# ttaoREtw/semi-tts

Measured on AMD Instinct MI355X. Metric: mel-frames/sec (decode+attn), higher is better.
Workload: dtype f32

## Files before the change

### include/semitts.h

```cpp
#ifndef SEMITTS_H
#define SEMITTS_H

#include <stddef.h>
#include <stdint.h>

#ifdef __cplusplus
extern "C" {
#endif

#define ST_ABI_VERSION 1

#define ST_ACT_NONE 0
#define ST_ACT_RELU 1
#define ST_ACT_TANH 2
#define ST_ACT_SIGMOID 3

const char* st_last_error(void);
int st_abi_version(void);
int st_device_info(int* n_cu, int* lds_bytes, char* name, int name_len);

int st_stream_create(void** stream_out);
int st_stream_destroy(void* stream);
int st_stream_sync(void* stream);
int st_graph_begin(void* stream);
// ... 225 lines not shown
    float* run_mean; float* run_var; long long* batches_tracked;
    float momentum, eps;
    float* mean; float* var;
    float* dx; int lddx;
    float* sums;
} st_bn_bank_seg;
size_t st_bn_bank_workspace_floats(int nseg, int max_rows, int N);
int st_bn_bank_fwd(const st_bn_bank_seg* segs, int nseg, int Bn, int N, float* Y, int ldy, int Tout, float* ws, void* stream);
int st_bn_bank_bwd(const st_bn_bank_seg* segs, int nseg, int Bn, int N, const float* dY, int lddy, int Tout, int relu_in, float* ws,
                   void* stream);
int st_bn_bank_stats_record(const st_bn_bank_seg* segs, int nseg, int Bn, int N, float* rec, float* ws, void* stream);
int st_bn_bank_sync_merge(const st_bn_bank_seg* segs, int nseg, int Bn, int N, const float* allrec, int world, float* inv_total, void* stream);
int st_bn_bank_norm(const st_bn_bank_seg* segs, int nseg, int Bn, int N, float* Y, int ldy, int Tout, void* stream);
int st_bn_bank_bwd_reduce(const st_bn_bank_seg* segs, int nseg, int Bn, int N, const float* dY, int lddy, int Tout, float* ws, void* stream);
int st_bn_bank_bwd_apply(const st_bn_bank_seg* segs, int nseg, int Bn, int N, const float* dY, int lddy, int Tout, int relu_in,
                         const float* inv_total, void* stream);
int st_highway_ht_fwd(const float* ht, const float* x, float* y, int M, int C, void* stream);
int st_highway_ht_bwd(const float* dy, const float* ht, const float* x, float* dht, float* dx_direct, int M, int C, void* stream);
int st_highway_bwd(const float* dy, const float* H, const float* x, const float* Tgate,
                   float* dH, float* dT, float* dx_direct, size_t total, void* stream);
int st_pool_prev_fwd(const float* x, float* y, int Bn, int T, int C, void* stream);
int st_pool_prev_bwd(const float* dy_pooled, const float* x, float* dx, int Bn, int T, int C, void* stream);
int st_copy3d(float* dst, long dst_sb, long dst_st, const float* src, long src_sb, long src_st,
              int Bn, int T, int C, int accumulate, void* stream);
int st_scatter_add_rows(const float* dout, const int64_t* idx, float* dtable, int n, int D, int V, void* stream);

int st_lstm_seq_fwd(const float* xproj, const float* w_hh, const float* b_hh, float* out, int ldo, int ocol,
                    float* ws, float* gates_tape, float* c_tape, int B, int T, int H, int reverse, void* stream);
int st_lstm_cell_bwd_pointwise(const float* dh0, int ld0, const float* dh1, int ld1, const float* dh2, int ld2,
                               const float* scale2, const float* mask, const float* gates, const float* c, int ldc,
                               const float* c_prev, int ldcp, float* dc, float* dgates, int ldg,
                               const st_t16_view* dgates_t16, int B, int H, void* stream);
int st_lstm_cell_pair_fwd(const st_seg* segs2, const float* const* b_hh2, const float* const* pre2, int ldpre,
                          const float* const* c_prev2, int ldc_prev, float* const* h_out2, int ldh,
                          float* const* c_out2, int ldc, float* const* gates_out2, int B, int H, void* stream);
int st_lstm_seq2_fwd(const float* const* xproj2, const float* const* w_hh2, const float* const* b_hh2, float* out, int ldo,
                     const int* ocol2, float* ws, float* const* gates_tape2, float* const* c_tape2,
                     int B, int T, int H, void* stream);
int st_lstm_seq2_persist_supported(int B, int T, int H, int ldo, int ocol0, int ocol1);
int st_lstm_seq2_persist_fwd(const float* const* xproj2, const float* const* w_hh2, const float* const* b_hh2, float* out, int ldo,
                             const int* ocol2, float* const* gates_tape2, float* const* c_tape2,
                             int B, int T, int H, unsigned* status, void* stream);
int st_lstm_seq2_bwd(const float* dout, int ldd, const int* dcol2, const float* const* gates_tape2, const float* const* c_tape2,
                     const float* const* w_hh_t2, float* const* dxproj2, float* ws, int B, int T, int H, void* stream);
int st_lstm_seq2_bwd_persist_supported(int B, int T, int H, int ldd, int dcol0, int dcol1);
int st_lstm_seq2_bwd_persist(const float* dout, int ldd, const int* dcol2, const float* const* gates_tape2, const float* const* c_tape2,
                             const float* const* w_hh2, float* const* dxproj2, int B, int T, int H, unsigned* status, void* stream);
int st_skinny_linear_pair_fwd(const st_seg* segs2, float* const* y2, int ldy, int B, int N, void* stream);
int st_lstm_seq2_bwd_packed(const float* dout, int ldd, const int* dcol2, const float* const* gates_tape2, const float* const* c_tape2,
                            const float* const* w_hh_t_p16_2, float* const* dxproj2, float* ws, float* dg_t16_ws,
                            int B, int T, int H, void* stream);
int st_lstm_seq_bwd(const float* dout, int ldd, int dcol, const float* gates_tape, const float* c_tape,
                    const float* w_hh_t, float* dxproj, float* ws, int B, int T, int H, int reverse, void* stream);
int st_gru_seq_fwd(const float* gi_fwd, const float* gi_bwd, const float* w_hh_fwd, const float* w_hh_bwd,
                   const float* b_hh_fwd, const float* b_hh_bwd, float* out, int ldo, float* tape,
                   int B, int T, int H, int ndir, void* stream);
int st_gru_seq_bwd(const float* dout, int ldd, const float* out, int ldo, const float* tape,
                   const float* w_hh_fwd, const float* w_hh_bwd, float* dgi_fwd, float* dgi_bwd,
                   float* dgh_fwd, float* dgh_bwd, int B, int T, int H, int ndir, void* stream);
#define ST_GRU_TRI 0
#define ST_GRU_QUAD 1
#define ST_GRU_REG32 2
#define ST_GRU_GENERAL 3
int st_gru_seq_variant(int H, int backward);

int st_vq_build_table(const float* learnable, int Dl, const float* attr, int n_attr,
                      const float* attr_w, const float* attr_b, int Da, float* table, int V, void* stream);
int st_gather_rows(const float* table, const int64_t* idx, float* out, int n, int D, int V, void* stream);
int st_vq_l2_fwd(const float* x, const float* table, const float* temp, float* p_code,
                 int64_t* idx, float* out, float* workspace, int n, int D, int V, void* stream);
int st_vq_pack_table(const float* table, float* packed, int D, int V, void* stream);
int st_vq_l2_packed_fwd(const float* x, const float* table, const float* packed, const float* temp, float* p_code,
                        int64_t* idx, float* out, int n, int D, int V, void* stream);
size_t st_vq_l2_workspace_floats(int D, int V);
int st_softmax_bwd(const float* p, const float* dp, const float* relu_scale, float scale, float* dz, float* rowsum,
                   int n, int V, void* stream);
int st_rowscale_combine(const float* a, float alpha, const float* x, const float* r, float beta, const float* c,
                        float* out, int M, int D, void* stream);
int st_vq_mean_fwd(const float* p_code, const float* latent, float* out, int* lens, int* frame_seg, float* frame_w,
                   int B, int T, int D, int V, int max_frames_per_phn, void* stream);
int st_vq_mean_bwd(const float* dout, int n_seg_rows, const int* frame_seg, const float* frame_w, float* dlatent,
                   int B, int T, int D, void* stream);
int st_softmax_argmax(const float* logits, float* p, int64_t* idx, int n, int V, void* stream);

typedef struct st_decoder_weights {
    const float* prenet_w0;
    const float* prenet_w1;
    const float* q_w_ih;
    const float* q_w_hh;
    const float* q_b_ih; const float* q_b_hh;
    const float* attn_query_w;
    const float* attn_v;
    const float* attn_loc_conv_w;
    const float* attn_loc_lin_w;
    const float* d_w_ih;
    const float* d_w_hh;
    const float* d_b_ih; const float* d_b_hh;
    const float* projgate_w;
    const float* projgate_b;
    const float* pre_norm_w[2]; const float* pre_norm_b[2];
    float* pre_norm_rm[2]; float* pre_norm_rv[2]; long long* pre_norm_nbt[2];
    float pre_norm_eps, pre_norm_momentum;
} st_decoder_weights;

typedef struct st_decoder_dims {
    int B, L, E, n_mels, r, P, Q, D, A, F, K;
    int fuse_pre0;
    int prenet_norm;
} st_decoder_dims;

typedef struct st_decoder_io {
    const float* memory;
    const float* pm;
    const float* ada_std;
    const float* ada_mean;
    const int* step_src;
    const float* teacher_pre;
    const float* teacher_mean;
    int Bt, Tt;
    const float* prenet_mask;
    const float* q_mask;
    const float* d_mask;
    int steps;
    float* mel_out;
    float* align_out;
    float* stop_out;
    const float* packed;
    float* xq_tape; float* xd_tape; float* xo_tape;
    float* cq_tape; float* cd_tape; float* wcum_tape;
    float* pq_buf;
    float* pre1_t16;
    float* mel_t16;
    float* zero_row;
    float* gates_q_tape;
    float* gates_d_tape;
    float* attn_s_buf;
    int attn_pre_parts;
    int attn_fin_parts;
    int defer_proj;
    int pre1_step_floats;
    int attn_s_step_floats;
    float* attn_loc_tape;
    float* attn_split_ws;
    int attn_split_parts;
    unsigned long long* pq_granules;
    const float* dec_in0;
    float* pre_nat;
    unsigned long long* attn_xchg;
    unsigned* handoff_status;
    int pair_cells;
    float* pre_nat_tape;
    float* gate_part;
    int gate_part_k;
} st_decoder_io;

int st_decoder_gate_split_k(const st_decoder_dims* d);
size_t st_decoder_packed_floats(const st_decoder_dims* d);
size_t st_decoder_tape_floats(const st_decoder_dims* d, int which);
int st_decoder_pack(const st_decoder_weights* w, const st_decoder_dims* d, float* packed, void* stream);
int st_decoder_forward(const st_decoder_weights* w, const st_decoder_dims* d, const st_decoder_io* io,
                       void* stream);
int st_decoder_fwd_forms(const st_decoder_dims* d, const st_decoder_io* io, int cus, int rng_capacity);

typedef struct st_attn_bwd_job {
    const float* pq; const float* pm; const float* memory;
    const float* w_prev; int ld_wprev; const float* w_cum_prev; const float* w; int ld_w;
    const float* loc_conv_w; const float* loc_lin_w; const float* v;
    const float* dctx[3]; int ld_dctx[3]; int n_dctx;
    const float* dw_direct[3]; int ld_dw[3]; int n_dw;
    float* dcum; const float* dcum_add; int ld_dcum_add;
    float* dpq; st_t16_view dpq_t16; float* dhist; float* ds_t; float* loc_t; float* dloc_t; float* hist_t;
    float* dctx_t; float* dv_t; const float* s_in;
    int B, L, A, E, F, K;
    int parts; float* dloc_part;
    const float* dctx_more[3]; int ld_dctx_more[3]; int n_dctx_more;
} st_attn_bwd_job;
int st_attn_step_bwd(const st_attn_bwd_job* job, void* stream);

int st_attn_dmem(const float* align, const float* dctx_tape, float* dmem, int B, int steps, int L, int E, void* stream);

typedef struct st_decoder_bwd_weights {
    const float* q_w_cat_t;
    const float* d_w_cat_t;
    const float* attn_query_w_t;
    const float* q_w_cat_t_p16;
    const float* d_w_cat_t_p16;
    const float* attn_query_w_t_p16;
    const float* attn_v; const float* attn_loc_conv_w; const float* attn_loc_lin_w;
} st_decoder_bwd_weights;

typedef struct st_decoder_bwd_io {
    const float* memory; const float* pm; const float* ada_std;
    const float* align;
    const float* wcum_tape;
    const float* cq_tape; const float* cd_tape;
    const float* gates_q_tape; const float* gates_d_tape;
    const float* q_mask; const float* d_mask;
    const float* pq_all;
    int steps; int Bp;
    const float* dxo;
    const float* dalign;
    float* dgq; float* dgd;
    float* dxq; float* dxd;
    float* dpq;
    float* ds_tape; float* loc_tape; float* dloc_tape;
    float* hist_tape; float* dctx_tape; float* dv_tape;
    float* dcq; float* dcd;
    float* dhist[2];
    float* dcum;
    float* dhq_attn;
    float* dgq_t16; float* dgd_t16;
    const int* step_src; int Bt;
    float* dY;
    float* dxo_rw;
    const float* wpg_t;
    const float* pre_w1_t; const float* pre_w0_t;
    const float* own_mask;
    const float* xq_nat;
    const float* pre1_nat;
    float* d2_tape; float* dp1_tape;
    float* tmp_p; float* tmp_in;
    int fuse_pw;
    float* dgd_t16_b;
    float* dpq_t16;
    int need_dxq0;
    const float* attn_s_tape;
    int overlap_attn;
    int prenet_norm;
    const float* pre_y_tape;
    const float* pre_norm_w[2]; const float* pre_norm_rm[2]; const float* pre_norm_rv[2];
    float pre_norm_eps;
    float* dpre_norm_w[2]; float* dpre_norm_b[2];
    int attn_parts; float* dloc_part;
    float* dxd_part; int dxd_splits;
    float* dxq_part; int dxq_splits;
} st_decoder_bwd_io;
int st_decoder_bwd_fuse_dims(const st_decoder_dims* d);
int st_decoder_bwd_forms(const st_decoder_dims* d, const st_decoder_bwd_io* io);
typedef struct st_attn_hist_job {
    const float* dloc_part; int parts;
    const float* loc_conv_w;
    const float* w_prev; int ld_wprev; const float* w_cum_prev;
    float* dloc_t; float* hist_t; float* dhist; float* dcum;
    int B, L, F, K;
} st_attn_hist_job;
int st_skinny_linear_packed_lstm_bwd_pair_fwd(const float* const* packed_w2, const st_t16_view* x2, int K, float* const* y2, int ldy,
                                              int B, int N, const st_lstm_pw_job* job2, void* stream);
int st_skinny_linear_packed_lstm_bwd_attn_bwd(const float* packed_w, const st_t16_view* x, int K, float* y, int ldy, int B, int N,
                                              const st_lstm_pw_job* job, const st_attn_bwd_job* ab, void* stream);
int st_attn_bwd_wide_fits(int L, int A, int E, int F, int K);
int st_attn_bwd_variant(int L, int A, int E, int F, int K, int has_s, int parts, int hosted, int B, int N, const float* loc_lin_w);
typedef struct st_partial_sum_job {
    const float* part; int S; int N;
    float* y; int ldy;
    const st_lstm_pw_job* pw;
} st_partial_sum_job;
int st_skinny_partial_attn_bwd(const float* packed_w, const st_t16_view* x, int K, float* part, int S, int B, int N,
                               const st_attn_bwd_job* ab, void* stream);
int st_skinny_partial_attn_hist(const float* packed_w, const st_t16_view* x, int K, float* part, int S, int B, int N,
                                const st_attn_hist_job* hist, void* stream);
int st_skinny_linear_packed_lstm_bwd_attn_hist_sum(const float* packed_w, const st_t16_view* x, int K, float* y, int ldy, int B, int N,
                                                   const st_lstm_pw_job* job, const st_attn_hist_job* hist,
                                                   const st_partial_sum_job* sum, void* stream);
int st_skinny_linear_packed_attn_hist(const float* packed_w, const st_t16_view* x, int K, float* y, int ldy, int B, int N,
                                      const st_attn_hist_job* hist, void* stream);
int st_decoder_backward(const st_decoder_bwd_weights* w, const st_decoder_dims* d, const st_decoder_bwd_io* io, void* stream);
void st_loop_graph_stats(long* fwd3, long* bwd3);
int st_loop_graphs_enable(int on);
int st_decoder_pack_dout(const float* dmel, const float* dstop, float* dY, int ld, int B, int Bp, int steps, int r, int n_mels,
                         void* stream);
int st_decoder_unpack_out(const float* Y, float* mel, float* stop, int B, int Bp, int steps, int r, int n_mels, int ld, void* stream);
int st_decoder_dteacher_sum(const float* dxq_part, float* dteacher, int S, int Bp, int XQw, int Bt, int Tt, int P, int steps, void* stream);
int st_adain_bwd(const float* dadapt, long da_step_stride, int da_ld, const float* hq, long hq_step_stride, int hq_ld,
                 const float* ada_std, const float* ada_mean, float* dstd, float* dmean, int B, int Q, int steps, void* stream);

size_t st_ctc_workspace_floats(int B, int T);
int st_ctc_loss(const float* prob, const int64_t* text, float eps, float* loss, float* dprob, float* ws,
                int B, int T, int V, int L, int log_input, void* stream);

int st_ctc_greedy_edit_distance(const float* prob, int B, int T, int V, const int64_t* text, int L,
                                const int32_t* ignore, int n_ignore,
                                int32_t* dist, int32_t* ref_len, int64_t* hyp , int32_t* hyp_len ,
                                void* stream);
int st_ids_edit_distance(const int64_t* pred, int B, int T, const int64_t* text, int L, const int32_t* ignore, int n_ignore,
                         int32_t* dist, int32_t* ref_len, int64_t* hyp, int32_t* hyp_len, void* stream);
int st_hyp_edit_distance(const int64_t* hyp, const int32_t* hyp_len, int B, int Lh, const int64_t* text, int L, const int32_t* ignore,
                         int n_ignore, int32_t* dist, int32_t* ref_len, void* stream);

size_t st_ctc_beam_workspace_bytes(int B, int T, int W);
int st_ctc_beam_search(const float* prob, int B, int T, int V, const int32_t* lengths , int W, int N, int blank,
                       int log_input, float eps, int64_t* hyp , int32_t* hyp_len ,
                       float* score , void* ws, void* stream);
int st_ctc_beam_search_lm(const float* prob, int B, int T, int V, const int32_t* lengths , int W, int N, int blank,
                          int log_input, float eps, const float* bonus , int order, int bos,
                          int64_t* hyp , int32_t* hyp_len , float* score , void* ws,
                          void* stream);

size_t st_ctc_align_workspace_bytes(int B, int T, int L);
int st_ctc_forced_align(const float* prob, int B, int T, int V, const int32_t* lengths ,
                        const int64_t* text , int L, const int32_t* text_lengths ,
                        int blank, int log_input, float eps,
                        float* score , int32_t* path ,
                        int32_t* tok_start , int32_t* tok_end , void* ws, void* stream);

#define ST_SCALAR_MAX 8
int st_scalar_combine(const float* const* xs, int n, const float* W, int m, float* const* outs, void* stream);
int st_scalar_fanout(const float* dout, const float* w, int n, float* out, void* stream);

size_t st_freq_loss_workspace_floats(void);
int st_freq_loss(const float* pred, const float* label, float* loss, float* dpred, float* ws,
                 int B, int T, int D, int n_low, float w_all, float w_low, float w_diff, int l1, void* stream);
typedef struct st_wgrad_job {
    const float* dC; int lddc, dcoff; const float* A; int lda; float* dW; float* db;
    int Bn, Tin, Tout, Cin, N, KT, pad;
} st_wgrad_job;
// ... 64 lines not shown
```

### semi_tts_amd/_lib.py

```python
import ctypes as C
import os

HERE = os.path.dirname(os.path.abspath(__file__))
LIB_PATH = os.environ.get('ST_LIB_PATH') or os.path.join(HERE, 'lib', 'libsemitts_hip.so')

c_float_p = C.c_void_p
c_void_p = C.c_void_p


class StSeg(C.Structure):
    _fields_ = [('x', C.c_void_p), ('w', C.c_void_p), ('ldx', C.c_int), ('ldw', C.c_int), ('k', C.c_int)]


class StT16View(C.Structure):
    _fields_ = [('base', C.c_void_p), ('kb_stride', C.c_int), ('kb0', C.c_int)]


class StGemmEpilogue(C.Structure):
    _fields_ = [('bias', C.c_void_p), ('act_pre', C.c_int),
                ('bn_mean', C.c_void_p), ('bn_var', C.c_void_p), ('bn_w', C.c_void_p), ('bn_b', C.c_void_p),
                ('bn_eps', C.c_float), ('act_post', C.c_int),
                ('res', C.c_void_p), ('ldres', C.c_int),
                ('highway_h', C.c_void_p), ('ldhw', C.c_int),
                ('mask', C.c_void_p), ('ldmask', C.c_int), ('w_tap_major', C.c_int),
                ('splitk_ws', C.c_void_p), ('splitk_slabs', C.c_int)]


class StGemmJob(C.Structure):
    _fields_ = [('A', C.c_void_p), ('lda', C.c_int), ('W', C.c_void_p), ('C', C.c_void_p), ('ldc', C.c_int), ('coff', C.c_int),
                ('Bn', C.c_int), ('Tin', C.c_int), ('Tout', C.c_int), ('Cin', C.c_int), ('N', C.c_int), ('KT', C.c_int),
                ('pad', C.c_int), ('stride', C.c_int), ('pool_prev', C.c_int), ('ep', StGemmEpilogue)]


class StRelayoutDesc(C.Structure):
    _fields_ = [('src', C.c_void_p), ('dst', C.c_void_p), ('N', C.c_int), ('Cin', C.c_int), ('KT', C.c_int), ('mode', C.c_int),
                ('blk0', C.c_int), ('ld_dst', C.c_int)]


class StBnBankSeg(C.Structure):
    _fields_ = [('x', C.c_void_p), ('ldx', C.c_int), ('T', C.c_int), ('w', C.c_void_p), ('b', C.c_void_p), ('run_mean', C.c_void_p),
                ('run_var', C.c_void_p), ('batches_tracked', C.c_void_p), ('momentum', C.c_float), ('eps', C.c_float),
                ('mean', C.c_void_p), ('var', C.c_void_p), ('dx', C.c_void_p), ('lddx', C.c_int), ('sums', C.c_void_p)]


class StDecoderWeights(C.Structure):
    _fields_ = [(n, C.c_void_p) for n in (
        'prenet_w0', 'prenet_w1', 'q_w_ih', 'q_w_hh', 'q_b_ih', 'q_b_hh',
        'attn_query_w', 'attn_v', 'attn_loc_conv_w', 'attn_loc_lin_w',
        'd_w_ih', 'd_w_hh', 'd_b_ih', 'd_b_hh', 'projgate_w', 'projgate_b')] + [
        ('pre_norm_w', C.c_void_p * 2), ('pre_norm_b', C.c_void_p * 2), ('pre_norm_rm', C.c_void_p * 2), ('pre_norm_rv', C.c_void_p * 2),
        ('pre_norm_nbt', C.c_void_p * 2), ('pre_norm_eps', C.c_float), ('pre_norm_momentum', C.c_float)]


class StDecoderDims(C.Structure):
    _fields_ = [(n, C.c_int) for n in ('B', 'L', 'E', 'n_mels', 'r', 'P', 'Q', 'D', 'A', 'F', 'K', 'fuse_pre0', 'prenet_norm')]


class StDecoderIO(C.Structure):
    _fields_ = [('memory', C.c_void_p), ('pm', C.c_void_p), ('ada_std', C.c_void_p), ('ada_mean', C.c_void_p),
                ('step_src', C.POINTER(C.c_int)), ('teacher_pre', C.c_void_p), ('teacher_mean', C.c_void_p),
                ('Bt', C.c_int), ('Tt', C.c_int),
                ('prenet_mask', C.c_void_p), ('q_mask', C.c_void_p), ('d_mask', C.c_void_p),
                ('steps', C.c_int),
                ('mel_out', C.c_void_p), ('align_out', C.c_void_p), ('stop_out', C.c_void_p),
                ('packed', C.c_void_p),
                ('xq_tape', C.c_void_p), ('xd_tape', C.c_void_p), ('xo_tape', C.c_void_p),
                ('cq_tape', C.c_void_p), ('cd_tape', C.c_void_p), ('wcum_tape', C.c_void_p),
                ('pq_buf', C.c_void_p), ('pre1_t16', C.c_void_p), ('mel_t16', C.c_void_p),
                ('zero_row', C.c_void_p),
                ('gates_q_tape', C.c_void_p), ('gates_d_tape', C.c_void_p), ('attn_s_buf', C.c_void_p), ('attn_pre_parts', C.c_int), ('attn_fin_parts', C.c_int), ('defer_proj', C.c_int),
                ('pre1_step_floats', C.c_int), ('attn_s_step_floats', C.c_int), ('attn_loc_tape', C.c_void_p),
                ('attn_split_ws', C.c_void_p), ('attn_split_parts', C.c_int), ('pq_granules', C.c_void_p),
                ('dec_in0', C.c_void_p), ('pre_nat', C.c_void_p), ('attn_xchg', C.c_void_p), ('handoff_status', C.c_void_p),
                ('pair_cells', C.c_int), ('pre_nat_tape', C.c_void_p), ('gate_part', C.c_void_p), ('gate_part_k', C.c_int)]


class StDecoderBwdWeights(C.Structure):
    _fields_ = [(n, C.c_void_p) for n in ('q_w_cat_t', 'd_w_cat_t', 'attn_query_w_t', 'q_w_cat_t_p16', 'd_w_cat_t_p16', 'attn_query_w_t_p16',
                                          'attn_v', 'attn_loc_conv_w', 'attn_loc_lin_w')]


class StDecoderBwdIO(C.Structure):
    _fields_ = ([(n, C.c_void_p) for n in ('memory', 'pm', 'ada_std', 'align', 'wcum_tape', 'cq_tape', 'cd_tape',
                                           'gates_q_tape', 'gates_d_tape', 'q_mask', 'd_mask', 'pq_all')] +
                [('steps', C.c_int), ('Bp', C.c_int)] +
                [(n, C.c_void_p) for n in ('dxo', 'dalign', 'dgq', 'dgd', 'dxq', 'dxd', 'dpq', 'ds_tape', 'loc_tape', 'dloc_tape',
                                           'hist_tape', 'dctx_tape', 'dv_tape', 'dcq', 'dcd')] +
                [('dhist', C.c_void_p * 2), ('dcum', C.c_void_p), ('dhq_attn', C.c_void_p), ('dgq_t16', C.c_void_p),
                 ('dgd_t16', C.c_void_p), ('step_src', C.POINTER(C.c_int)), ('Bt', C.c_int)] +
                [(n, C.c_void_p) for n in ('dY', 'dxo_rw', 'wpg_t', 'pre_w1_t', 'pre_w0_t', 'own_mask', 'xq_nat', 'pre1_nat',
                                           'd2_tape', 'dp1_tape', 'tmp_p', 'tmp_in')] +
                [('fuse_pw', C.c_int), ('dgd_t16_b', C.c_void_p), ('dpq_t16', C.c_void_p), ('need_dxq0', C.c_int), ('attn_s_tape', C.c_void_p),
                 ('overlap_attn', C.c_int), ('prenet_norm', C.c_int), ('pre_y_tape', C.c_void_p), ('pre_norm_w', C.c_void_p * 2),
                 ('pre_norm_rm', C.c_void_p * 2), ('pre_norm_rv', C.c_void_p * 2), ('pre_norm_eps', C.c_float),
                 ('dpre_norm_w', C.c_void_p * 2), ('dpre_norm_b', C.c_void_p * 2), ('attn_parts', C.c_int), ('dloc_part', C.c_void_p),
                 ('dxd_part', C.c_void_p), ('dxd_splits', C.c_int), ('dxq_part', C.c_void_p), ('dxq_splits', C.c_int)])



class StLstmPwJob(C.Structure):
    _fields_ = [('n0', C.c_int), ('H', C.c_int), ('dh1', C.c_void_p), ('ld1', C.c_int), ('dh2', C.c_void_p), ('ld2', C.c_int),
                ('scale2', C.c_void_p), ('mask', C.c_void_p), ('gates', C.c_void_p), ('c', C.c_void_p), ('ldc', C.c_int),
                ('c_prev', C.c_void_p), ('ldcp', C.c_int), ('dc', C.c_void_p), ('dgates', C.c_void_p), ('ldg', C.c_int),
                ('dgates_t16', StT16View), ('dh1_slabs', C.c_int), ('dh1_slab_stride', C.c_long)]


class StLstmCellPackedJob(C.Structure):
    _fields_ = [('packed_w', C.c_void_p), ('x', StT16View), ('K', C.c_int), ('b_ih', C.c_void_p), ('b_hh', C.c_void_p),
                ('c_prev', C.c_void_p), ('ldc_prev', C.c_int), ('mask', C.c_void_p), ('h_dst0', StT16View), ('h_dst1', StT16View),
                ('c_out', C.c_void_p), ('ldc', C.c_int), ('gates_out', C.c_void_p), ('ada_std', C.c_void_p), ('ada_mean', C.c_void_p),
                ('hadapt_dst', StT16View), ('B', C.c_int), ('H', C.c_int), ('part', C.c_void_p), ('w_kbs', C.c_int)]


class StAttnBwdJob(C.Structure):
    _fields_ = [('pq', C.c_void_p), ('pm', C.c_void_p), ('memory', C.c_void_p),
                ('w_prev', C.c_void_p), ('ld_wprev', C.c_int), ('w_cum_prev', C.c_void_p), ('w', C.c_void_p), ('ld_w', C.c_int),
                ('loc_conv_w', C.c_void_p), ('loc_lin_w', C.c_void_p), ('v', C.c_void_p),
                ('dctx', C.c_void_p * 3), ('ld_dctx', C.c_int * 3), ('n_dctx', C.c_int),
                ('dw_direct', C.c_void_p * 3), ('ld_dw', C.c_int * 3), ('n_dw', C.c_int),
                ('dcum', C.c_void_p), ('dcum_add', C.c_void_p), ('ld_dcum_add', C.c_int),
                ('dpq', C.c_void_p), ('dpq_t16', StT16View), ('dhist', C.c_void_p), ('ds_t', C.c_void_p), ('loc_t', C.c_void_p),
                ('dloc_t', C.c_void_p), ('hist_t', C.c_void_p), ('dctx_t', C.c_void_p), ('dv_t', C.c_void_p), ('s_in', C.c_void_p),
                ('B', C.c_int), ('L', C.c_int), ('A', C.c_int), ('E', C.c_int), ('F', C.c_int), ('K', C.c_int),
                ('parts', C.c_int), ('dloc_part', C.c_void_p),
                ('dctx_more', C.c_void_p * 3), ('ld_dctx_more', C.c_int * 3), ('n_dctx_more', C.c_int)]


class StAttnHistJob(C.Structure):
    _fields_ = [('dloc_part', C.c_void_p), ('parts', C.c_int), ('loc_conv_w', C.c_void_p),
                ('w_prev', C.c_void_p), ('ld_wprev', C.c_int), ('w_cum_prev', C.c_void_p),
                ('dloc_t', C.c_void_p), ('hist_t', C.c_void_p), ('dhist', C.c_void_p), ('dcum', C.c_void_p),
                ('B', C.c_int), ('L', C.c_int), ('F', C.c_int), ('K', C.c_int)]


class StWgradJob(C.Structure):
    _fields_ = [('dC', C.c_void_p), ('lddc', C.c_int), ('dcoff', C.c_int), ('A', C.c_void_p), ('lda', C.c_int), ('dW', C.c_void_p), ('db', C.c_void_p),
                ('Bn', C.c_int), ('Tin', C.c_int), ('Tout', C.c_int), ('Cin', C.c_int), ('N', C.c_int), ('KT', C.c_int), ('pad', C.c_int)]


class StPartialSumJob(C.Structure):
    _fields_ = [('part', C.c_void_p), ('S', C.c_int), ('N', C.c_int), ('y', C.c_void_p), ('ldy', C.c_int), ('pw', C.c_void_p)]


class StAttnPreJob(C.Structure):
    _fields_ = [('pm', C.c_void_p), ('w_prev', C.c_void_p), ('ld_wprev', C.c_int), ('w_cum_prev', C.c_void_p),
                ('loc_conv_w', C.c_void_p), ('loc_lin_w', C.c_void_p), ('s_buf', C.c_void_p),
                ('L', C.c_int), ('A', C.c_int), ('F', C.c_int), ('K', C.c_int), ('parts', C.c_int), ('cf_out', C.c_void_p),
                ('part', C.c_void_p)]


class StAttnFinJob(C.Structure):
    _fields_ = [('s_buf', C.c_void_p), ('memory', C.c_void_p), ('w_cum_prev', C.c_void_p),
                ('w_out', C.c_void_p), ('ld_wout', C.c_int), ('w_cum_out', C.c_void_p), ('v', C.c_void_p),
                ('ctx_dst', StT16View * 3), ('n_ctx_dst', C.c_int), ('parts', C.c_int),
                ('L', C.c_int), ('A', C.c_int), ('E', C.c_int), ('F', C.c_int), ('K', C.c_int), ('status', C.c_void_p),
                ('ctx', C.c_void_p), ('ld_ctx', C.c_int)]


class StAttnStepJob(C.Structure):
    _fields_ = [('pq', C.c_void_p), ('pm', C.c_void_p), ('memory', C.c_void_p),
                ('w_prev', C.c_void_p), ('ld_wprev', C.c_int), ('w_cum_prev', C.c_void_p),
                ('w_out', C.c_void_p), ('ld_wout', C.c_int), ('w_cum_out', C.c_void_p),
                ('loc_conv_w', C.c_void_p), ('loc_lin_w', C.c_void_p), ('v', C.c_void_p),
                ('ctx_dst', StT16View * 3), ('n_ctx_dst', C.c_int), ('ctx', C.c_void_p), ('ld_ctx', C.c_int),
                ('h_q', C.c_void_p), ('ld_hq', C.c_int), ('ada_std', C.c_void_p), ('ada_mean', C.c_void_p), ('h_adapt', C.c_void_p),
                ('Q', C.c_int), ('L', C.c_int), ('A', C.c_int), ('E', C.c_int), ('F', C.c_int), ('K', C.c_int)]


class StPartialProductJob(C.Structure):
    _fields_ = [('packed_w', C.c_void_p), ('w_kbs', C.c_int), ('kb0', C.c_int), ('KB', C.c_int), ('x', StT16View), ('N', C.c_int),
                ('part', C.c_void_p)]


P, I, F, Z = C.c_void_p, C.c_int, C.c_float, C.c_size_t

SIGNATURES = {
    'st_last_error': [],
    'st_abi_version': [],
    'st_device_info': [C.POINTER(I), C.POINTER(I), C.c_char_p, I],
    'st_stream_create': [C.POINTER(P)],
    'st_stream_destroy': [P],
    'st_stream_sync': [P],
    'st_graph_begin': [P],
    'st_graph_end': [P, C.POINTER(P)],
    'st_graph_launch': [P, P],
    'st_graph_destroy': [P],
    'st_event_create': [C.POINTER(P)],
    'st_event_record': [P, P],
    'st_event_elapsed_ms': [P, P, C.POINTER(F)],
    'st_event_destroy': [P],
    'st_lstm_cell_fwd': [C.POINTER(StSeg), I, P, P, P, I, P, I, P, P, I, P, I, P, I, I, P],
    'st_skinny_linear_fwd': [C.POINTER(StSeg), I, P, I, P, I, P, I, I, P, I, I, I, I, P],
    'st_attn_step_fwd': [C.POINTER(StAttnStepJob), I, P],
    'st_gemm_fwd': [P, I, P, P, I, I, I, I, I, I, I, I, I, I, I, C.POINTER(StGemmEpilogue), P],
    'st_gemm_fwd_batch': [C.POINTER(StGemmJob), I, P],
    'st_gemm_fwd_variant': [P, I, P, P, I, I, I, I, I, I, I, I, I, I, I, C.POINTER(StGemmEpilogue)],
    'st_gemm_fwd_batch_variant': [C.POINTER(StGemmJob), I],
    'st_highway_stack_supported': [I, I],
    'st_highway_stack_fwd': [P, I, C.POINTER(P), C.POINTER(P), C.POINTER(P), C.POINTER(P), I, P, I, I, I, P],
    'st_gemm_splitk_slabs': [I, I, I, I, I],
    'st_bn_stats': [P, I, I, I, I, P, P, P, P, F, P, P, P],
    'st_colreduce_workspace_floats': [I, I],
    'st_bn_apply': [P, I, I, I, I, P, P, P, P, F, I, P],
    'st_lstm_seq_fwd': [P, P, P, P, I, I, P, P, P, I, I, I, I, P],
    'st_lstm_cell_bwd_pointwise': [P, I, P, I, P, I, P, P, P, P, I, P, I, P, P, I, C.POINTER(StT16View), I, I, P],
    'st_lstm_seq_bwd': [P, I, I, P, P, P, P, P, I, I, I, I, P],
    'st_gru_seq_fwd': [P, P, P, P, P, P, P, I, P, I, I, I, I, P],
    'st_gru_seq_bwd': [P, I, P, I, P, P, P, P, P, P, P, I, I, I, I, P],
    'st_gru_seq_variant': [I, I],
    'st_vq_build_table': [P, I, P, I, P, P, I, P, I, P],
    'st_gather_rows': [P, P, P, I, I, I, P],
    'st_vq_l2_fwd': [P, P, P, P, P, P, P, I, I, I, P],
    'st_vq_pack_table': [P, P, I, I, P],
    'st_vq_l2_packed_fwd': [P, P, P, P, P, P, P, I, I, I, P],
    'st_vq_l2_workspace_floats': [I, I],
    'st_ctc_workspace_floats': [I, I],
    'st_ctc_loss': [P, P, C.c_float, P, P, P, I, I, I, I, I, P],
    'st_ctc_greedy_edit_distance': [P, I, I, I, P, I, P, I, P, P, P, P, P],
    'st_ids_edit_distance': [P, I, I, P, I, P, I, P, P, P, P, P],
    'st_hyp_edit_distance': [P, P, I, I, P, I, P, I, P, P, P],
    'st_ctc_beam_workspace_bytes': [I, I, I],
    'st_ctc_beam_search': [P, I, I, I, P, I, I, I, I, F, P, P, P, P, P],
    'st_ctc_beam_search_lm': [P, I, I, I, P, I, I, I, I, F, P, I, I, P, P, P, P, P],
    'st_ctc_align_workspace_bytes': [I, I, I],
    'st_ctc_forced_align': [P, I, I, I, P, P, I, P, I, I, F, P, P, P, P, P, P],
    'st_scalar_combine': [P, I, P, I, P, P],
    'st_scalar_fanout': [P, P, I, P, P],
    'st_softmax_bwd': [P, P, P, C.c_float, P, P, I, I, P],
    'st_rowscale_combine': [P, C.c_float, P, P, C.c_float, P, P, I, I, P],
    'st_vq_mean_fwd': [P, P, P, P, P, P, I, I, I, I, I, P],
    'st_vq_mean_bwd': [P, I, P, P, P, I, I, I, P],
    'st_softmax_argmax': [P, P, P, I, I, P],
    'st_packed_weight_floats': [C.POINTER(I), I, I, I],
    'st_t16_floats': [I, I],
    'st_pack_weight': [C.POINTER(P), C.POINTER(I), C.POINTER(I), I, I, I, P, P],
    'st_pack_weight_t': [C.POINTER(P), C.POINTER(I), C.POINTER(I), I, I, P, P],
    'st_relayout_blocks': [I, I, I],
    'st_relayout_batch': [P, I, I, P, P],
    'st_pack_weight_batch': [P, I, P],
    'st_tile_rows': [P, I, C.POINTER(StT16View), I, I, P],
    'st_untile_rows': [C.POINTER(StT16View), P, I, I, I, P],
    'st_lstm_cell_packed_fwd': [C.POINTER(StLstmCellPackedJob), P],
    'st_lstm_cell_packed_pair_fwd': [C.POINTER(StLstmCellPackedJob), C.POINTER(StLstmCellPackedJob), P],
    'st_skinny_linear_packed_fwd': [P, C.POINTER(StT16View), I, P, I, P, I, P, I, C.POINTER(StT16View), I, P, I, I,
                                    I, I, P, I, C.POINTER(StT16View), I, I, P],
    'st_skinny_linear_packed_attnpre_fwd': [P, C.POINTER(StT16View), I, P, I, P, I, P, I, C.POINTER(StT16View), I, P, I, I,
                                            I, I, P, I, C.POINTER(StT16View), I, I, C.POINTER(StAttnPreJob), P],
    'st_attn_pre_fwd': [C.POINTER(StAttnPreJob), I, P],
    'st_attn_fin_fwd': [P, C.POINTER(StAttnFinJob), I, P],
    'st_attn_fin_split_workspace_floats': [I, I, I],
    'st_attn_fin_split_fwd': [P, C.POINTER(StAttnFinJob), P, I, P],
    'st_query_attn_fin_fwd': [P, C.POINTER(StT16View), I, P, C.c_uint, C.POINTER(StAttnFinJob), I, P],
    'st_query_attn_fin_part_fwd': [P, C.POINTER(StT16View), I, P, C.c_uint, C.POINTER(StAttnFinJob), I, C.POINTER(StPartialProductJob), P],
    'st_partial_product_fwd': [C.POINTER(StPartialProductJob), I, P],
    'st_layer_norm_fwd': [P, I, P, P, F, P, I, P, P, I, I, P],
    'st_layer_norm_bwd': [P, I, P, I, P, P, P, P, I, P, I, I, P],
    'st_log_softmax_fwd': [P, P, I, I, P],
    'st_log_softmax_bwd': [P, P, P, I, I, P],
    'st_prenet_norm_fwd': [P, I, I, P, P, P, P, P, F, F, P, I, C.POINTER(StT16View), I, I, I, P],
    'st_prenet_norm_bwd': [P, I, P, I, I, P, P, P, F, P, P, I, I, P],
    'st_handoff_wait_selftest': [P, C.c_uint, I, P, P, I, P],
    'st_query_attn_rng_fits': [I, I, I],
    'st_attn_rng_xchg_words': [I, I, I],
    'st_query_attn_rng_fwd': [P, C.POINTER(StT16View), I, P, P, C.c_uint, C.POINTER(StAttnFinJob), I, P],
    'st_decoder_packed_floats': [C.POINTER(StDecoderDims)],
    'st_decoder_gate_split_k': [C.POINTER(StDecoderDims)],
    'st_decoder_tape_floats': [C.POINTER(StDecoderDims), I],
    'st_decoder_pack': [C.POINTER(StDecoderWeights), C.POINTER(StDecoderDims), P, P],
    'st_decoder_forward': [C.POINTER(StDecoderWeights), C.POINTER(StDecoderDims), C.POINTER(StDecoderIO), P],
    'st_decoder_fwd_forms': [C.POINTER(StDecoderDims), C.POINTER(StDecoderIO), I, I],
    'st_attn_step_bwd': [C.POINTER(StAttnBwdJob), P],
    'st_skinny_linear_packed_lstm_bwd_fwd': [P, C.POINTER(StT16View), I, P, I, I, I, C.POINTER(StLstmPwJob), P],
    'st_skinny_linear_packed_lstm_bwd_attn_bwd': [P, C.POINTER(StT16View), I, P, I, I, I, C.POINTER(StLstmPwJob), C.POINTER(StAttnBwdJob), P],
    'st_attn_bwd_wide_fits': [I, I, I, I, I],
    'st_attn_bwd_variant': [I, I, I, I, I, I, I, I, I, I, P],
    'st_skinny_linear_packed_attn_hist': [P, C.POINTER(StT16View), I, P, I, I, I, C.POINTER(StAttnHistJob), P],
    'st_skinny_partial_attn_hist': [P, C.POINTER(StT16View), I, P, I, I, I, C.POINTER(StAttnHistJob), P],
    'st_decoder_bwd_forms': [C.POINTER(StDecoderDims), C.POINTER(StDecoderBwdIO)],
    'st_decoder_bwd_fuse_dims': [C.POINTER(StDecoderDims)],
    'st_loop_graph_stats': [P, P],
    'st_loop_graphs_enable': [I],
    'st_skinny_partial_attn_bwd': [P, C.POINTER(StT16View), I, P, I, I, I, C.POINTER(StAttnBwdJob), P],
    'st_skinny_linear_packed_lstm_bwd_attn_hist_sum': [P, C.POINTER(StT16View), I, P, I, I, I, C.POINTER(StLstmPwJob), C.POINTER(StAttnHistJob),
                                                       C.POINTER(StPartialSumJob), P],
    'st_lstm_seq2_fwd': [C.POINTER(P), C.POINTER(P), C.POINTER(P), P, I, C.POINTER(I), P, C.POINTER(P), C.POINTER(P), I, I, I, P],
    'st_lstm_seq2_persist_supported': [I, I, I, I, I, I],
    'st_lstm_seq2_persist_fwd': [C.POINTER(P), C.POINTER(P), C.POINTER(P), P, I, C.POINTER(I), C.POINTER(P), C.POINTER(P), I, I, I, P, P],
    'st_lstm_seq2_bwd_persist_supported': [I, I, I, I, I, I],
    'st_lstm_seq2_bwd_persist': [P, I, C.POINTER(I), C.POINTER(P), C.POINTER(P), C.POINTER(P), C.POINTER(P), I, I, I, P, P],
    'st_lstm_seq2_bwd': [P, I, C.POINTER(I), C.POINTER(P), C.POINTER(P), C.POINTER(P), C.POINTER(P), P, I, I, I, P],
    'st_skinny_linear_pair_fwd': [P, C.POINTER(P), I, I, I, P],
    'st_lstm_seq2_bwd_packed': [P, I, C.POINTER(I), C.POINTER(P), C.POINTER(P), C.POINTER(P), C.POINTER(P), P, P, I, I, I, P],
    'st_skinny_linear_packed_lstm_bwd_pair_fwd': [C.POINTER(P), C.POINTER(StT16View), I, C.POINTER(P), I, I, I, C.POINTER(StLstmPwJob), P],
    'st_lstm_cell_pair_fwd': [P, C.POINTER(P), C.POINTER(P), I, C.POINTER(P), I, C.POINTER(P), I, C.POINTER(P), I, C.POINTER(P), I, I, P],
    'st_attn_dmem': [P, P, P, I, I, I, I, P],
    'st_decoder_backward': [C.POINTER(StDecoderBwdWeights), C.POINTER(StDecoderDims), C.POINTER(StDecoderBwdIO), P],
    'st_decoder_pack_dout': [P, P, P, I, I, I, I, I, I, P],
    'st_decoder_unpack_out': [P, P, P, I, I, I, I, I, I, P],
    'st_decoder_dteacher_sum': [P, P, I, I, I, I, I, I, I, P],
    'st_adain_bwd': [P, C.c_long, I, P, C.c_long, I, P, P, P, P, I, I, I, P],
    'st_mt_blocks': [P, I],
    'st_mt_table_misses': [],
    'st_mt_grad_norm': [P, P, I, P, P, P],
    'st_mt_clip_scale': [P, P, I, P, F, P],
    'st_mt_grad_norm_scaled': [P, P, I, P, P, F, P],
    'st_mt_clip_scale_pre': [P, P, I, P, F, F, P],
    'st_mt_copy': [P, P, P, I, P],
    'st_mt_adam': [P, P, P, P, P, I, F, F, F, F, F, P],
    'st_mt_adam_guarded': [P, P, P, P, P, I, F, F, F, F, F, P, P],
    'st_freq_loss': [P, P, P, P, P, I, I, I, I, F, F, F, I, P],
    'st_freq_loss_workspace_floats': [],
    'st_scale_by': [P, P, P, Z, P],
    'st_bn_norm_fwd': [P, I, I, P, I, I, I, I, P, P, P, P, F, I, P],
    'st_gemm_wgrad_workspace_floats': [I, I, I, I, I],
    'st_gemm_wgrad': [P, I, I, P, I, P, P, I, I, I, I, I, I, I, I, I, P],
    'st_gemm_wgrad_db': [P, I, I, P, I, P, P, P, I, I, I, I, I, I, I, I, I, P],
    'st_gemm_wgrad_batch_workspace_floats': [C.POINTER(StWgradJob), I],
    'st_gemm_wgrad_batch': [C.POINTER(StWgradJob), I, P, P],
    'st_gemm_wgrad_variant': [P, I, I, P, I, I, I, I, I, I, I, I, I, I, I, I],
    'st_gemm_wgrad_batch_variant': [C.POINTER(StWgradJob), I, C.POINTER(I)],
    'st_gemm_wgrad_split': [P, I, I, P, I, P, I, P, P, P, P, I, I, I, I, P],
    'st_colsum': [P, I, I, P, I, I, I, I, P, I, P, P],
    'st_act_bwd': [P, I, P, I, I, P, I, P, I, I, I, P],
    'st_bn_bwd': [P, I, I, P, I, I, I, P, I, I, P, P, P, F, I, I, P, I, I, P, P, I, P, P],
    'st_bn_bwd_reduce': [P, I, I, P, I, I, I, P, I, I, P, P, F, I, I, P, P, P],
    'st_bn_norm_res_mask_fwd': [P, P, P, I, I, P, P, P, P, F, I, P, P, P],
    'st_bn_bwd_reduce_masked': [P, I, P, I, P, I, I, P, I, P, P, F, I, I, P, P, P],
    'st_bn_bwd_apply_masked': [P, I, P, I, P, I, I, P, I, P, P, P, F, I, I, P, I, P, P, I, P, I, P],
    'st_bn_bwd_apply': [P, I, I, P, I, I, I, P, I, I, P, P, P, F, I, I, P, I, P, I, I, P],
    'st_bn_stats_record': [P, I, I, I, I, P, P, P, P],
    'st_bn_sync_merge': [P, I, I, P, P, P, P, F, P, P],
    'st_bn_bwd_apply_sync': [P, I, I, P, I, I, I, P, I, I, P, P, P, F, I, I, P, P, P, I, I, P],
    'st_highway_fwd': [P, P, P, P, Z, P],
    'st_bn_bank_workspace_floats': [I, I, I],
    'st_bn_bank_fwd': [C.POINTER(StBnBankSeg), I, I, I, P, I, I, P, P],
    'st_bn_bank_bwd': [C.POINTER(StBnBankSeg), I, I, I, P, I, I, I, P, P],
    'st_bn_bank_stats_record': [C.POINTER(StBnBankSeg), I, I, I, P, P, P],
    'st_bn_bank_sync_merge': [C.POINTER(StBnBankSeg), I, I, I, P, I, P, P],
    'st_bn_bank_norm': [C.POINTER(StBnBankSeg), I, I, I, P, I, I, P],
    'st_bn_bank_bwd_reduce': [C.POINTER(StBnBankSeg), I, I, I, P, I, I, P, P],
    'st_bn_bank_bwd_apply': [C.POINTER(StBnBankSeg), I, I, I, P, I, I, I, P, P],
    'st_highway_ht_fwd': [P, P, P, I, I, P],
    'st_highway_ht_bwd': [P, P, P, P, P, I, I, P],
    'st_highway_bwd': [P, P, P, P, P, P, P, Z, P],
    'st_pool_prev_fwd': [P, P, I, I, I, P],
    'st_pool_prev_bwd': [P, P, P, I, I, I, P],
    'st_copy3d': [P, C.c_long, C.c_long, P, C.c_long, C.c_long, I, I, I, I, P],
    'st_scatter_add_rows': [P, P, P, I, I, I, P],
    'st_fill': [P, F, Z, P],
    'st_copy2d': [P, I, P, I, I, I, P],
    'st_mean_rows': [P, P, I, I, I, P],
    'st_istft_workspace_floats': [I, I, I, I, I],
    'st_gl_workspace_floats': [I, I, I, I, I],
    'st_stft_fwd': [P, P, I, I, I, I, I, P],
    'st_istft': [P, P, I, I, I, I, I, P, P],
    'st_griffin_lim': [P, C.c_long, C.c_long, C.c_long, I, F, P, P, I, I, I, I, I, I, I, P, P],
    'st_mel_to_linear': [P, C.c_long, C.c_long, C.c_long, P, P, I, I, I, I, I, I, P],
    'st_gl_batch_workspace_floats': [I, I, I, I, I],
    'st_griffin_lim_batch': [P, C.c_long, C.c_long, C.c_long, I, P, I, F, P, P, P, I, I, I, I, I, I, I, P, P],
    'st_features_workspace_floats': [I],
    'st_audio_features': [P, C.c_long, P, C.c_ulonglong, P, P, P, P, P, I, I, I, I, I, F, P, P, P, P, I, P, P, I, P, I, P, P],
    'st_feature_noise': [P, C.c_long, I, C.c_ulonglong, P],
    'st_resample_batch': [P, I, C.c_long, P, P, I, I, I, I, I, I, P, P, P, C.c_long, P, P],
}
_RESTYPES = {'st_last_error': C.c_char_p, 'st_packed_weight_floats': C.c_size_t, 'st_t16_floats': C.c_size_t,
             'st_decoder_packed_floats': C.c_size_t, 'st_vq_l2_workspace_floats': C.c_size_t, 'st_ctc_workspace_floats': C.c_size_t, 'st_decoder_tape_floats': C.c_size_t,
             'st_gemm_wgrad_workspace_floats': C.c_size_t, 'st_gemm_wgrad_batch_workspace_floats': C.c_size_t, 'st_freq_loss_workspace_floats': C.c_size_t, 'st_attn_fin_split_workspace_floats': C.c_size_t, 'st_attn_rng_xchg_words': C.c_size_t, 'st_colreduce_workspace_floats': C.c_size_t, 'st_mt_blocks': C.c_size_t, 'st_mt_table_misses': C.c_long,
             'st_bn_bank_workspace_floats': C.c_size_t, 'st_istft_workspace_floats': C.c_size_t, 'st_gl_workspace_floats': C.c_size_t,
             'st_gl_batch_workspace_floats': C.c_size_t,
             'st_features_workspace_floats': C.c_size_t, 'st_ctc_beam_workspace_bytes': C.c_size_t, 'st_ctc_align_workspace_bytes': C.c_size_t}

_lib = None


def load():
    global _lib
    if _lib is not None:
        return _lib
    import torch
    if not os.path.exists(LIB_PATH):
        raise RuntimeError(
            'libsemitts_hip.so not found at %s -- build it with `python -m semi_tts_amd.build` '
            '(hipcc --offload-arch=gfx950).  There is no CPU fallback.' % LIB_PATH)
    lib = C.CDLL(LIB_PATH)
    for name, args in SIGNATURES.items():
        fn = getattr(lib, name)
        fn.argtypes = args
        fn.restype = _RESTYPES.get(name, C.c_int)
    if lib.st_abi_version() != 1:
        raise RuntimeError('libsemitts_hip.so ABI version mismatch')
    _lib = lib
    return lib


def check(rc, what):
    if rc != 0:
        msg = load().st_last_error()
        raise RuntimeError('%s failed (%d): %s' % (what, rc, msg.decode() if msg else '?'))


def check_header_symbols():
    import re
    hdr = open(os.path.join(os.path.dirname(HERE), 'include', 'semitts.h')).read()
    declared = sorted(set(re.findall(r'\b(st_[a-z0-9_]+)\s*\(', hdr)))
    lib = C.CDLL(LIB_PATH)
    missing = [s for s in declared if not hasattr(lib, s)]
    if missing:
        raise RuntimeError('declared in include/semitts.h but not exported by %s: %s' % (LIB_PATH, missing))
    if sorted(SIGNATURES) != declared:
        raise RuntimeError('ctypes table and include/semitts.h disagree: %s' % sorted(set(SIGNATURES) ^ set(declared)))
    return declared
```

### semi_tts_amd/csrc/decoder.hip

```cpp
#include "st_common.h"
#include "loop_graph.h"
#include <cstdlib>

namespace {

struct ZeroArgs { float* p[12]; size_t floats[12]; int n; };
__global__ __launch_bounds__(256) void zero_regions_kernel(const ZeroArgs a) {
    float* __restrict__ p = a.p[blockIdx.y];
    const size_t n = a.floats[blockIdx.y];
    const size_t n4 = (((uintptr_t)p & 15u) == 0) ? n / 4 : 0;
    const f32x4 z = {0.f, 0.f, 0.f, 0.f};
    for (size_t i = (size_t)blockIdx.x * blockDim.x + threadIdx.x; i < n4; i += (size_t)gridDim.x * blockDim.x) reinterpret_cast<f32x4*>(p)[i] = z;
    for (size_t i = n4 * 4 + (size_t)blockIdx.x * blockDim.x + threadIdx.x; i < n; i += (size_t)gridDim.x * blockDim.x) p[i] = 0.0f;
}

}

extern "C" size_t st_packed_weight_floats(const int* k, int nseg, int N, int lstm_H);
extern "C" size_t st_t16_floats(int B, int K);

namespace {

struct PackedLayout {
    size_t q, pq, d, pg, p0, p1, total;
};

PackedLayout packed_layout(const st_decoder_dims* d) {
    PackedLayout o;
    const int in_dim = d->r * d->n_mels;
    size_t p = 0;
    { int k[3] = {d->P, d->E, d->Q}; o.q = p; p += st_packed_weight_floats(k, 3, 4 * d->Q, d->Q); }
    { int k[1] = {d->Q}; o.pq = p; p += st_packed_weight_floats(k, 1, d->A, 0); }
    { int k[3] = {d->E, d->Q, d->D}; o.d = p; p += st_packed_weight_floats(k, 3, 4 * d->D, d->D); }
    { int k[2] = {d->D, d->E}; o.pg = p; p += st_packed_weight_floats(k, 2, in_dim + 1 + (d->fuse_pre0 ? d->P : 0), 0); }
    { int k[1] = {in_dim}; o.p0 = p; p += st_packed_weight_floats(k, 1, d->P, 0); }
    { int k[1] = {d->P}; o.p1 = p; p += st_packed_weight_floats(k, 1, d->P, 0); }
    o.total = p;
    return o;
}

inline int kb16(int k) { return (k + 15) >> 4; }

struct StepViews {
    int q_kbs, q_ctx, q_h;
    int d_kbs, d_ha, d_h;
    int o_kbs, o_ctx;
    size_t q_floats, d_floats, o_floats;
};

StepViews step_views(const st_decoder_dims* d) {
    StepViews v;
    const int bt = (d->B + 15) >> 4;
    v.q_ctx = kb16(d->P); v.q_h = v.q_ctx + kb16(d->E); v.q_kbs = v.q_h + kb16(d->Q);
    v.d_ha = kb16(d->E); v.d_h = v.d_ha + kb16(d->Q); v.d_kbs = v.d_h + kb16(d->D);
    v.o_ctx = kb16(d->D); v.o_kbs = v.o_ctx + kb16(d->E);
    v.q_floats = (size_t)bt * v.q_kbs * 256; v.d_floats = (size_t)bt * v.d_kbs * 256; v.o_floats = (size_t)bt * v.o_kbs * 256;
    return v;
}

__global__ __launch_bounds__(256) void tile_teacher_kernel(const float* teacher_pre, int Tt, float* xq_tape, size_t slot_floats,
                                                           int q_kbs, int steps, int Bt, int P) {
    const size_t total = (size_t)(steps - 1) * Bt * P;
    for (size_t i = (size_t)blockIdx.x * blockDim.x + threadIdx.x; i < total; i += (size_t)gridDim.x * blockDim.x) {
        const int k = (int)(i % P);
        const size_t sb = i / P;
        const int b = (int)(sb % Bt), s = (int)(sb / Bt) + 1;
        const int frame = s - 1 < Tt ? s - 1 : Tt - 1;
        const float v = teacher_pre[((size_t)b * Tt + frame) * P + k];
        xq_tape[(size_t)s * slot_floats + (((size_t)(b >> 4) * q_kbs + (k >> 4)) * 64 + ((k >> 2) & 3) * 16 + (b & 15)) * 4 + (k & 3)] = v;
    }
}

int prenet_own(const st_decoder_weights* w, const st_decoder_dims* d, const st_decoder_io* io, const PackedLayout& pl, const StepViews& sv,
               int t, bool layer1_done, void* stream) {
    const int in_dim = d->r * d->n_mels;
    const size_t BP = (size_t)d->B * d->P;
    const float* m1 = io->prenet_mask ? io->prenet_mask + ((size_t)t * 2 + 0) * BP : nullptr;
    const float* m2 = io->prenet_mask ? io->prenet_mask + ((size_t)t * 2 + 1) * BP : nullptr;
    st_t16_view mel = {io->mel_t16, kb16(in_dim), 0};
    st_t16_view pre1 = {io->pre1_t16 + (size_t)t * io->pre1_step_floats, kb16(d->P), 0};
    int rc = 0;
    if (d->prenet_norm) {
        st_t16_view next_n = {io->xq_tape + (size_t)(t + 1) * sv.q_floats, sv.q_kbs, 0};
        const st_t16_view* dsts[2] = {&pre1, &next_n};
        const st_t16_view* srcs[2] = {&mel, &pre1};
        const float* pw[2] = {io->packed + pl.p0, io->packed + pl.p1};
        const int Ks[2] = {16 * kb16(in_dim), 16 * kb16(d->P)};
        const float* ms[2] = {m1, m2};
        const int b0 = io->step_src[t] == -1 ? 0 : io->Bt;
        for (int l = 0; l < 2; ++l) {
            float* y = io->pre_nat_tape ? io->pre_nat_tape + ((size_t)t * 2 + l) * BP : io->pre_nat;
            rc = st_skinny_linear_packed_fwd(pw[l], srcs[l], Ks[l], nullptr, ST_ACT_NONE, nullptr, 0, y, d->P, nullptr, 0,
                                             nullptr, 0, 0, 0, 0, nullptr, 0, nullptr, d->B, d->P, stream);
            if (rc) return rc;
            rc = st_prenet_norm_fwd(y, d->P, d->prenet_norm, w->pre_norm_w[l], w->pre_norm_b[l], w->pre_norm_rm[l], w->pre_norm_rv[l],
                                    w->pre_norm_nbt[l], w->pre_norm_eps, w->pre_norm_momentum, ms[l], d->P, dsts[l], b0, d->B, d->P, stream);
            if (rc) return rc;
        }
        return 0;
    }
    if (!layer1_done)
        rc = st_skinny_linear_packed_fwd(io->packed + pl.p0, &mel, 16 * kb16(in_dim), nullptr, ST_ACT_RELU, m1, d->P,
                                         nullptr, 0, &pre1, 0, nullptr, 0, 0, 0, 0, nullptr, 0, nullptr, d->B, d->P, stream);
    if (rc) return rc;
    st_t16_view next = {io->xq_tape + (size_t)(t + 1) * sv.q_floats, sv.q_kbs, 0};
    return st_skinny_linear_packed_fwd(io->packed + pl.p1, &pre1, 16 * kb16(d->P), nullptr, ST_ACT_RELU, m2, d->P,
                                       nullptr, 0, &next, 0, nullptr, 0, 0, 0, 0, nullptr, 0, nullptr, d->B, d->P, stream);
}

}

extern "C" int st_decoder_gate_split_k(const st_decoder_dims* d) {
    if (!d) return 0;
    const StepViews sv = step_views(d);
    int hosted = (sv.d_kbs / 2) / 16 * 16;
    if (hosted < 16 || hosted > sv.d_kbs - sv.d_ha) hosted = sv.d_kbs - sv.d_ha;
    return 16 * (sv.d_kbs - hosted);
}

extern "C" size_t st_decoder_packed_floats(const st_decoder_dims* d) { return d ? packed_layout(d).total : 0; }

extern "C" int st_decoder_pack(const st_decoder_weights* w, const st_decoder_dims* d, float* packed, void* stream) {
    (void)hipGetLastError();
    ST_CHECK_ARG(w && d && packed, "st_decoder_pack: null pointer");
    const PackedLayout pl = packed_layout(d);
    const int in_dim = d->r * d->n_mels;
    st_pack_job j[6];
    memset(j, 0, sizeof(j));
    auto seg = [&](st_pack_job& q, int s, const float* wp, int ld, int k) { q.w[s] = wp; q.ldw[s] = ld; q.k[s] = k; q.nseg = s + 1; };
    seg(j[0], 0, w->q_w_ih, d->P + d->E, d->P); seg(j[0], 1, w->q_w_ih + d->P, d->P + d->E, d->E); seg(j[0], 2, w->q_w_hh, d->Q, d->Q);
    j[0].N = 4 * d->Q; j[0].lstm_H = d->Q; j[0].packed = packed + pl.q;
    seg(j[1], 0, w->attn_query_w, d->Q, d->Q); j[1].N = d->A; j[1].packed = packed + pl.pq;
    seg(j[2], 0, w->d_w_ih, d->E + d->Q, d->E); seg(j[2], 1, w->d_w_ih + d->E, d->E + d->Q, d->Q); seg(j[2], 2, w->d_w_hh, d->D, d->D);
    j[2].N = 4 * d->D; j[2].lstm_H = d->D; j[2].packed = packed + pl.d;
    seg(j[3], 0, w->projgate_w, d->D + d->E, d->D); seg(j[3], 1, w->projgate_w + d->D, d->D + d->E, d->E);
    j[3].N = in_dim + 1 + (d->fuse_pre0 ? d->P : 0); j[3].packed = packed + pl.pg;
    seg(j[4], 0, w->prenet_w0, in_dim, in_dim); j[4].N = d->P; j[4].packed = packed + pl.p0;
    seg(j[5], 0, w->prenet_w1, d->P, d->P); j[5].N = d->P; j[5].packed = packed + pl.p1;
    return st_pack_weight_batch(j, 6, stream);
}

extern "C" size_t st_decoder_tape_floats(const st_decoder_dims* d, int which) {
    if (!d) return 0;
    const StepViews sv = step_views(d);
    return which == 0 ? sv.q_floats : (which == 1 ? sv.d_floats : sv.o_floats);
}

namespace {

enum FwdAttn {
    ATTN_WHOLE,
    ATTN_PRE_FIN,
    ATTN_FIN_SPLIT,
    ATTN_PQ_FIN,
    ATTN_PQ_RNG
};
enum FwdProd {
    PROD_NONE,
    PROD_OWN,
    PROD_PQ_FIN,
    PROD_PQ_PRE
};
struct FwdForms {
    bool pure_tf;
    bool defer;
    bool pre_in_pq;
    bool pair_cells;
    FwdAttn attn;
    FwdProd prod;
    int fin_parts;
    int pq_pre_parts;
    int d_k0;
};

FwdForms fwd_forms(const st_decoder_dims* d, const st_decoder_io* io, int cus, int rng_capacity) {
    FwdForms f;
    const int B = d->B, L = d->L, E = d->E, Q = d->Q, D = d->D, A = d->A, BT = (B + 15) / 16;
    f.pure_tf = io->teacher_pre && io->Bt == B && io->Tt > 0;
    for (int t = 0; t + 1 < io->steps && f.pure_tf; ++t) f.pure_tf = io->step_src[t] == (t < io->Tt ? t : io->Tt - 1);
    f.defer = io->defer_proj != 0;
    f.pair_cells = f.defer && f.pure_tf && io->pair_cells;
    const bool split_attn = io->attn_s_buf != nullptr;
    f.pre_in_pq = split_attn && f.defer;
    const int fp_req = io->attn_fin_parts;
    f.fin_parts = (fp_req == 2 || fp_req == 4 || fp_req == 8) && E % (4 * fp_req) == 0 ? fp_req : 1;
    const int sp = io->attn_split_parts;
    const bool fin_split = split_attn && io->attn_split_ws && sp >= 2 && sp <= 64 && A % 4 == 0 && A <= 256 && E % 4 == 0 &&
                           E / 4 <= 512 && 512 % (E / 4) == 0 && (L + sp - 1) / sp <= 512;
    const bool fin_rng = fin_split && !f.pre_in_pq && io->pq_granules && io->attn_xchg && sp <= 8 && A % 16 == 0 && E % (4 * sp) == 0 &&
                         E / sp <= 256 && (sp - 1) * ((L + sp - 1) / sp) < L && (A / 16) * BT + B * sp <= rng_capacity;
    const bool fuse_pq_fin = !fin_split && split_attn && !f.pre_in_pq && io->pq_granules && A % 16 == 0 && A <= 256 && E % 4 == 0 &&
                             (A / 16) * BT + B * f.fin_parts <= cus;
    f.attn = !split_attn ? ATTN_WHOLE : fin_rng ? ATTN_PQ_RNG : fin_split ? ATTN_FIN_SPLIT : fuse_pq_fin ? ATTN_PQ_FIN : ATTN_PRE_FIN;
    const bool split_d = io->gate_part && (!f.defer || f.pre_in_pq) && B > 16 && B <= 32 && D % 16 == 0 && (D / 4) % 2 == 0 &&
                         E % 16 == 0 && Q % 16 == 0 && st_aligned16(io->gate_part);
    const int pre_parts_split = io->attn_pre_parts > 2 ? 2 : io->attn_pre_parts;
    const bool split_pre = split_d && f.pre_in_pq && A <= 16 * 128 &&
                           ((A + 15) / 16) * BT + B * (pre_parts_split > 1 ? pre_parts_split : 1) + (4 * D) / 32 <= cus;
    f.pq_pre_parts = split_pre ? pre_parts_split : io->attn_pre_parts;
    if (!split_d) f.prod = PROD_NONE;
    else if (split_pre) f.prod = PROD_PQ_PRE;
    else if (fuse_pq_fin && (A / 16) * BT + B * f.fin_parts + (4 * D) / 32 <= cus) f.prod = PROD_PQ_FIN;
    else f.prod = PROD_OWN;
    f.d_k0 = (io->gate_part_k ? io->gate_part_k : st_decoder_gate_split_k(d)) / 16;
    return f;
}

}

int pk_attnrng_capacity();

extern "C" int st_decoder_fwd_forms(const st_decoder_dims* d, const st_decoder_io* io, int cus, int rng_capacity) {
    if (!d || !io || (io->steps > 1 && !io->step_src)) return -1;
    const FwdForms f = fwd_forms(d, io, cus > 0 ? cus : st_device_cus(), rng_capacity > 0 ? rng_capacity : pk_attnrng_capacity());
    return (int)f.attn | ((int)f.prod << 4) | (f.pure_tf ? 1 << 8 : 0) | (f.defer ? 1 << 9 : 0) | (f.pre_in_pq ? 1 << 10 : 0) |
           (f.pair_cells ? 1 << 11 : 0) | (f.fin_parts << 12) | ((f.prod != PROD_NONE ? f.d_k0 & 0xfff : 0) << 16);
}

static int decoder_forward_issue(const st_decoder_weights* w, const st_decoder_dims* d, const st_decoder_io* io, void* stream);

static stlg::Cache g_fwd_graphs;
extern "C" void st_loop_graph_stats(long* fwd3, long* bwd3);
extern "C" void stx_fwd_loop_graph_stats(long* out3) {
    std::lock_guard<std::mutex> lock(g_fwd_graphs.mu);
    out3[0] = g_fwd_graphs.replays; out3[1] = g_fwd_graphs.captures; out3[2] = g_fwd_graphs.eager;
}

extern "C" int st_decoder_forward(const st_decoder_weights* w, const st_decoder_dims* d, const st_decoder_io* io,
                                  void* stream) {
    (void)hipGetLastError();
    ST_CHECK_ARG(w && d && io, "st_decoder_forward: null struct pointer");
    if (io->defer_proj && io->steps > 0 && io->step_src && stlg::enabled(d->B)) {
        st_decoder_io key_io = *io;
        key_io.step_src = nullptr;
        uint64_t key = stlg::fnv(stlg::FNV0, w, sizeof(*w));
        key = stlg::fnv(key, d, sizeof(*d));
        key = stlg::fnv(key, &key_io, sizeof(key_io));
        key = stlg::fnv(key, io->step_src, sizeof(int) * (size_t)io->steps);
        stlg::Entry* e = nullptr;
        hipStream_t issue_on = (hipStream_t)stream;
        const int mode = stlg::begin(g_fwd_graphs, key, (hipStream_t)stream, &e, &issue_on);
        if (mode == 1) return 0;
        int rc = decoder_forward_issue(w, d, io, (void*)issue_on);
        if (mode == 2) {
            rc = stlg::end(g_fwd_graphs, e, (hipStream_t)stream, rc);
            if (rc == -5) st_set_error("st_decoder_forward: capturing the loop into a hipGraph failed");
        }
        return rc;
    }
    return decoder_forward_issue(w, d, io, stream);
}

static int decoder_forward_issue(const st_decoder_weights* w, const st_decoder_dims* d, const st_decoder_io* io, void* stream) {
    ST_CHECK_ARG(w && d && io, "st_decoder_forward: null struct pointer");
    const int B = d->B, L = d->L, E = d->E, P = d->P, Q = d->Q, D = d->D, A = d->A;
    const int steps = io->steps;
    const int in_dim = d->r * d->n_mels;
    ST_CHECK_ARG(B > 0 && L > 0 && steps > 0 && in_dim > 0, "st_decoder_forward: B=%d L=%d steps=%d", B, L, steps);
    ST_CHECK_ARG(io->memory && io->pm && io->ada_std && io->ada_mean && io->step_src && io->packed,
                 "st_decoder_forward: null input");
    ST_CHECK_ARG(io->mel_out && io->align_out && io->stop_out, "st_decoder_forward: null output");
    ST_CHECK_ARG(io->xq_tape && io->xd_tape && io->xo_tape && io->cq_tape && io->cd_tape && io->wcum_tape &&
                 io->pq_buf && io->pre1_t16 && io->mel_t16 && io->zero_row, "st_decoder_forward: null tape/scratch");
    ST_CHECK_ARG(d->prenet_norm >= 0 && d->prenet_norm <= 3 && (!d->prenet_norm || (!d->fuse_pre0 && io->pre_nat && w->pre_norm_w[0] &&
                 w->pre_norm_w[1] && w->pre_norm_b[0] && w->pre_norm_b[1])), "st_decoder_forward: normalised prenet needs pre_nat, the norm weights and fuse_pre0 = 0");
    for (int t = 0; t + 1 < steps; ++t) {
        const int src = io->step_src[t];
        ST_CHECK_ARG(!d->fuse_pre0 || src == -1, "st_decoder_forward: fuse_pre0 needs every next input to be the own output");
        ST_CHECK_ARG(src >= -2 && (src < 0 || (io->teacher_pre && src < io->Tt)), "st_decoder_forward: step_src[%d]=%d invalid", t, src);
        ST_CHECK_ARG(src != -2 || io->teacher_mean, "st_decoder_forward: step_src[%d]=-2 without teacher_mean", t);
        ST_CHECK_ARG(src == -1 || (io->Bt > 0 && io->Bt <= B), "st_decoder_forward: Bt=%d invalid", io->Bt);
    }
    const StepViews sv = step_views(d);
    ST_CHECK_ARG(io->gate_part_k == 0 || !io->gate_part || (io->gate_part_k % 16 == 0 && io->gate_part_k >= 16 * sv.d_ha && io->gate_part_k < 16 * sv.d_kbs),
                 "st_decoder_forward: gate_part_k = %d must be a multiple of 16 in [%d, %d)", io->gate_part_k, 16 * sv.d_ha, 16 * sv.d_kbs);
    FwdForms f = fwd_forms(d, io, st_device_cus(), pk_attnrng_capacity());
    ST_CHECK_ARG(!f.defer || (f.pure_tf && !d->fuse_pre0), "st_decoder_forward: defer_proj needs pure teacher forcing");
#ifdef ST_ABLATE
    const int skip = getenv("ST_SKIP") ? atoi(getenv("ST_SKIP")) : 0;
    if ((skip & 8) || (f.prod == PROD_PQ_FIN && (skip & 6)) || (f.prod == PROD_PQ_PRE && (skip & 2))) f.prod = PROD_NONE;
#define ST_SKIPPED(bit) (skip & (1 << (bit)))
#else
#define ST_SKIPPED(bit) 0
#endif
    hipStream_t st = (hipStream_t)stream;
    const PackedLayout pl = packed_layout(d);
    const size_t BQ = (size_t)B * Q, BD = (size_t)B * D, BL = (size_t)B * L;
    ZeroArgs za;
    memset(&za, 0, sizeof(za));
    auto zero = [&](void* p, size_t bytes) { za.p[za.n] = (float*)p; za.floats[za.n] = bytes / sizeof(float); ++za.n; };
    zero(io->cq_tape, BQ * sizeof(float));
    zero(io->cd_tape, BD * sizeof(float));
    zero(io->wcum_tape, BL * sizeof(float));
    zero(io->zero_row, BL * sizeof(float));
    zero(io->xq_tape, sv.q_floats * sizeof(float));
    zero(io->xd_tape, sv.d_floats * sizeof(float));
    if (io->attn_loc_tape) zero(io->attn_loc_tape, BL * d->F * sizeof(float));
    const int sp_parts = io->attn_split_parts;
    if (f.attn == ATTN_PQ_FIN || f.attn == ATTN_PQ_RNG) zero(io->pq_granules, (size_t)B * A * sizeof(unsigned long long));
    if (f.attn == ATTN_PQ_RNG) zero(io->attn_xchg, st_attn_rng_xchg_words(B, E, sp_parts) * sizeof(unsigned long long));
    {
        size_t most = 0;
        for (int i = 0; i < za.n; ++i) most = za.floats[i] > most ? za.floats[i] : most;
        size_t blocks = (most / 4 + 255) / 256 + 1;
        if (blocks > 256) blocks = 256;
        hipLaunchKernelGGL(zero_regions_kernel, dim3((unsigned)blocks, za.n), dim3(256), 0, st, za);
        ST_LAUNCH_CHECK();
    }
    if (io->dec_in0) {
        st_t16_view xq0 = {io->xq_tape, sv.q_kbs, 0};
        int rc0 = st_tile_rows(io->dec_in0, P, &xq0, B, P, stream);
        if (rc0) return rc0;
    }
    if (f.pure_tf && steps > 1) {
        const size_t total = (size_t)(steps - 1) * B * P;
        size_t blocks = (total + 255) / 256;
        if (blocks > 4096) blocks = 4096;
        hipLaunchKernelGGL(tile_teacher_kernel, dim3((unsigned)blocks), dim3(256), 0, st, io->teacher_pre, io->Tt, io->xq_tape,
                           sv.q_floats, sv.q_kbs, steps, B, P);
        ST_LAUNCH_CHECK();
    }

    const size_t ldmel = (size_t)steps * in_dim;
    const int ldal = steps * L;
    const int Kq = 16 * sv.q_kbs, Kd = 16 * sv.d_kbs, Ko = 16 * sv.o_kbs;
    st_partial_product_job pj_d;
    memset(&pj_d, 0, sizeof(pj_d));
    pj_d.packed_w = io->packed + pl.d; pj_d.w_kbs = sv.d_kbs; pj_d.kb0 = f.d_k0; pj_d.KB = sv.d_kbs - f.d_k0; pj_d.N = 4 * D; pj_d.part = io->gate_part;
    const bool part = f.prod != PROD_NONE;
    auto cell_q = [&](int t) {
        st_lstm_cell_packed_job j;
        memset(&j, 0, sizeof(j));
        j.packed_w = io->packed + pl.q; j.x = st_t16_view{io->xq_tape + (size_t)t * sv.q_floats, sv.q_kbs, 0}; j.K = Kq;
        j.b_ih = w->q_b_ih; j.b_hh = w->q_b_hh;
        j.c_prev = io->cq_tape + (size_t)t * BQ; j.ldc_prev = Q; j.mask = io->q_mask ? io->q_mask + (size_t)t * BQ : nullptr;
        j.h_dst0 = st_t16_view{io->xq_tape + (size_t)(t + 1) * sv.q_floats, sv.q_kbs, sv.q_h};
        j.c_out = io->cq_tape + (size_t)(t + 1) * BQ; j.ldc = Q;
        j.gates_out = io->gates_q_tape ? io->gates_q_tape + (size_t)t * 4 * BQ : nullptr;
        j.ada_std = io->ada_std; j.ada_mean = io->ada_mean; j.hadapt_dst = st_t16_view{io->xd_tape + (size_t)t * sv.d_floats, sv.d_kbs, sv.d_ha};
        j.B = B; j.H = Q;
        return j;
    };
    auto cell_d = [&](int t) {
        st_lstm_cell_packed_job j;
        memset(&j, 0, sizeof(j));
        j.packed_w = io->packed + pl.d; j.x = st_t16_view{io->xd_tape + (size_t)t * sv.d_floats, sv.d_kbs, 0}; j.K = Kd;
        j.b_ih = w->d_b_ih; j.b_hh = w->d_b_hh;
        if (part) { j.K = 16 * f.d_k0; j.part = io->gate_part; j.w_kbs = sv.d_kbs; }
        j.c_prev = io->cd_tape + (size_t)t * BD; j.ldc_prev = D; j.mask = io->d_mask ? io->d_mask + (size_t)t * BD : nullptr;
        j.h_dst0 = st_t16_view{io->xd_tape + (size_t)(t + 1) * sv.d_floats, sv.d_kbs, sv.d_h};
        j.h_dst1 = st_t16_view{io->xo_tape + (size_t)t * sv.o_floats, sv.o_kbs, 0};
        j.c_out = io->cd_tape + (size_t)(t + 1) * BD; j.ldc = D;
        j.gates_out = io->gates_d_tape ? io->gates_d_tape + (size_t)t * 4 * BD : nullptr;
        j.B = B; j.H = D;
        return j;
    };
    auto pre_job = [&](int t, int parts) {
        return st_attn_pre_job{io->pm, io->align_out + (size_t)(t - 1) * L, ldal, io->wcum_tape + (size_t)t * BL,
                               w->attn_loc_conv_w, w->attn_loc_lin_w,
                               f.attn != ATTN_WHOLE ? io->attn_s_buf + (size_t)t * io->attn_s_step_floats : nullptr, L, A, d->F, d->K,
                               parts, io->attn_loc_tape ? io->attn_loc_tape + (size_t)t * BL * d->F : nullptr, nullptr};
    };
    int rc = 0;
    for (int t = 0; t < steps; ++t) {
        float* xq_next = io->xq_tape + (size_t)(t + 1) * sv.q_floats;
        float* xd = io->xd_tape + (size_t)t * sv.d_floats;
        float* xo = io->xo_tape + (size_t)t * sv.o_floats;
        pj_d.x = st_t16_view{xd, sv.d_kbs, f.d_k0};

        st_t16_view hq_dst = {xq_next, sv.q_kbs, sv.q_h};
        if (!(f.pair_cells && t > 0) && !ST_SKIPPED(0)) {
            const st_lstm_cell_packed_job jq = cell_q(t);
            rc = st_lstm_cell_packed_fwd(&jq, stream);
            if (rc) return rc;
        }

        if (f.attn != ATTN_PQ_FIN && f.attn != ATTN_PQ_RNG && !ST_SKIPPED(1)) {
            if (f.pre_in_pq && t > 0) {
                st_attn_pre_job job = pre_job(t, f.pq_pre_parts);
                if (f.prod == PROD_PQ_PRE) job.part = &pj_d;
                rc = st_skinny_linear_packed_attnpre_fwd(io->packed + pl.pq, &hq_dst, 16 * kb16(Q), nullptr, ST_ACT_NONE, nullptr, 0,
                                                         io->pq_buf, A, nullptr, 0, nullptr, 0, 0, 0, 0, nullptr, 0, nullptr, B, A,
                                                         &job, stream);
            } else
                rc = st_skinny_linear_packed_fwd(io->packed + pl.pq, &hq_dst, 16 * kb16(Q), nullptr, ST_ACT_NONE, nullptr, 0,
                                                 io->pq_buf, A, nullptr, 0, nullptr, 0, 0, 0, 0, nullptr, 0, nullptr, B, A, stream);
            if (rc) return rc;
        }

        st_t16_view ctx_dst[3] = {{xq_next, sv.q_kbs, sv.q_ctx}, {xd, sv.d_kbs, 0}, {xo, sv.o_kbs, sv.o_ctx}};
        const float* s_t = t == 0 || f.attn == ATTN_WHOLE ? io->pm : io->attn_s_buf + (size_t)t * io->attn_s_step_floats;
        auto fin_job = [&](int parts) {
            st_attn_fin_job fj;
            memset(&fj, 0, sizeof(fj));
            fj.s_buf = s_t; fj.memory = io->memory; fj.w_cum_prev = io->wcum_tape + (size_t)t * BL;
            fj.w_out = io->align_out + (size_t)t * L; fj.ld_wout = ldal; fj.w_cum_out = io->wcum_tape + (size_t)(t + 1) * BL; fj.v = w->attn_v;
            for (int c = 0; c < 3; ++c) fj.ctx_dst[c] = ctx_dst[c];
            fj.status = io->handoff_status;
            fj.n_ctx_dst = 3; fj.parts = parts; fj.L = L; fj.A = A; fj.E = E; fj.F = d->F; fj.K = d->K;
            return fj;
        };
        switch (f.attn) {
        case ATTN_WHOLE:
            if (!ST_SKIPPED(2)) {
                st_attn_step_job sj;
                memset(&sj, 0, sizeof(sj));
                sj.pq = io->pq_buf; sj.pm = io->pm; sj.memory = io->memory;
                sj.w_prev = t == 0 ? io->zero_row : io->align_out + (size_t)(t - 1) * L; sj.ld_wprev = t == 0 ? L : ldal;
                sj.w_cum_prev = io->wcum_tape + (size_t)t * BL;
                sj.w_out = io->align_out + (size_t)t * L; sj.ld_wout = ldal; sj.w_cum_out = io->wcum_tape + (size_t)(t + 1) * BL;
                sj.loc_conv_w = w->attn_loc_conv_w; sj.loc_lin_w = w->attn_loc_lin_w; sj.v = w->attn_v;
                for (int c = 0; c < 3; ++c) sj.ctx_dst[c] = ctx_dst[c];
                sj.n_ctx_dst = 3; sj.L = L; sj.A = A; sj.E = E; sj.F = d->F; sj.K = d->K;
                rc = st_attn_step_fwd(&sj, B, stream);
            }
            break;
        case ATTN_PRE_FIN:
            if (!ST_SKIPPED(2)) {
                const st_attn_fin_job fj = fin_job(f.fin_parts);
                rc = st_attn_fin_fwd(io->pq_buf, &fj, B, stream);
            }
            break;
        case ATTN_FIN_SPLIT:
            if (!ST_SKIPPED(2)) {
                const st_attn_fin_job fj = fin_job(sp_parts);
                rc = st_attn_fin_split_fwd(io->pq_buf, &fj, io->attn_split_ws, B, stream);
            }
            break;
        case ATTN_PQ_FIN:
            if (!(ST_SKIPPED(1) || ST_SKIPPED(2))) {
                const st_attn_fin_job fj = fin_job(f.fin_parts);
                rc = f.prod == PROD_PQ_FIN
                         ? st_query_attn_fin_part_fwd(io->packed + pl.pq, &hq_dst, 16 * kb16(Q), io->pq_granules, (unsigned)(t + 1), &fj, B, &pj_d, stream)
                         : st_query_attn_fin_fwd(io->packed + pl.pq, &hq_dst, 16 * kb16(Q), io->pq_granules, (unsigned)(t + 1), &fj, B, stream);
            }
            break;
        case ATTN_PQ_RNG:
            if (!(ST_SKIPPED(1) || ST_SKIPPED(2))) {
                const st_attn_fin_job fj = fin_job(sp_parts);
                rc = st_query_attn_rng_fwd(io->packed + pl.pq, &hq_dst, 16 * kb16(Q), io->pq_granules, io->attn_xchg, (unsigned)(t + 1), &fj, B, stream);
            }
            break;
        }
        if (rc) return rc;

        if (f.prod == PROD_OWN || (f.prod == PROD_PQ_PRE && t == 0)) {
            rc = st_partial_product_fwd(&pj_d, B, stream);
            if (rc) return rc;
        }
        if (!ST_SKIPPED(3)) {
            const st_lstm_cell_packed_job jd = cell_d(t);
            if (f.pair_cells && t + 1 < steps) {
                const st_lstm_cell_packed_job jq = cell_q(t + 1);
                rc = st_lstm_cell_packed_pair_fwd(&jd, &jq, stream);
            } else
                rc = st_lstm_cell_packed_fwd(&jd, stream);
            if (rc) return rc;
        }

        st_t16_view xo_v = {xo, sv.o_kbs, 0};
        st_t16_view mel_dst = {io->mel_t16, kb16(in_dim), 0};
        st_t16_view pre1_dst = {io->pre1_t16 + (size_t)t * io->pre1_step_floats, kb16(P), 0};
        const bool fuse = d->fuse_pre0 != 0;
        if (f.defer) continue;
        const bool split_attn = f.attn != ATTN_WHOLE;
        const st_attn_pre_job job = pre_job(t + 1, io->attn_pre_parts);
        if (!ST_SKIPPED(4)) {
            rc = st_skinny_linear_packed_attnpre_fwd(io->packed + pl.pg, &xo_v, ST_SKIPPED(7) ? Ko / 4 : Ko, w->projgate_b, ST_ACT_NONE, nullptr, 0,
                                                     io->mel_out + (size_t)t * in_dim, (int)ldmel, fuse ? nullptr : &mel_dst, in_dim,
                                                     io->stop_out + (size_t)t * d->r, steps * d->r, d->r,
                                                     fuse ? in_dim + 1 : 0, ST_ACT_RELU,
                                                     io->prenet_mask ? io->prenet_mask + (size_t)t * 2 * B * P : nullptr, P,
                                                     fuse ? &pre1_dst : nullptr, B, in_dim + 1 + (fuse ? P : 0),
                                                     split_attn && t + 1 < steps && !ST_SKIPPED(6) ? &job : nullptr, stream);
            if (rc) return rc;
        }

        if (t + 1 < steps) {
            const int src = io->step_src[t];
            st_t16_view next = {xq_next, sv.q_kbs, 0};
            if ((src == -1 || io->Bt < B) && !ST_SKIPPED(5)) {
                rc = prenet_own(w, d, io, pl, sv, t, fuse, stream);
                if (rc) return rc;
            }
            if (!f.pure_tf && src >= 0) rc = st_tile_rows(io->teacher_pre + (size_t)src * P, io->Tt * P, &next, io->Bt, P, stream);
            else if (!f.pure_tf && src == -2) rc = st_tile_rows(io->teacher_mean, P, &next, io->Bt, P, stream);
            if (rc) return rc;
        } else if (d->prenet_norm == 3 && (io->step_src[t] == -1 || io->Bt < B)) {
            rc = prenet_own(w, d, io, pl, sv, t, false, stream);
            if (rc) return rc;
        }
    }
    return 0;
}
```

### semi_tts_amd/csrc/skinny.hip

```cpp
#include "st_common.h"

namespace {

constexpr int SK_MAXSEG = 3;

struct SkArgs {
    st_seg seg[SK_MAXSEG];
    int nseg;
    int B, N, H;
    const float* b_ih; const float* b_hh; const float* pre; int ldpre;
    const float* c_prev; int ldc_prev; const float* mask;
    float* h_out; int ldh; float* c_out; int ldc; float* gates_out;
    const float* bias; int act; const float* lmask; int ldmask;
    float* y; int ldy; int n_split; float* y2; int ldy2; int rep;
};

template <bool VEC>
__device__ __forceinline__ f32x4 sk_load(const float* p, int k0, int klim) {
    if (VEC) {
        if (k0 + 4 <= klim) return st_ld4(p + k0);
        f32x4 z = {0.f, 0.f, 0.f, 0.f};
        return z;
    } else {
        return st_ld4_guard(p + k0, klim - k0);
    }
}

template <int MODE, int NB, int KW, bool VEC>
__device__ __forceinline__ void sk_body(const SkArgs& a, f32x4* red) {
    const int tid = threadIdx.x;
    const int lane = tid & 63;
    const int wave = tid >> 6;
    const int i = lane & 15;
    const int kq = lane >> 4;
    const int tile = blockIdx.x;
    const int bbase = blockIdx.y * (NB * 16);

    int wrow;
    if (MODE == 0) wrow = (i & 3) * a.H + tile * 4 + (i >> 2);
    else { wrow = tile * 16 + i; if (wrow >= a.N) wrow = a.N - 1; }

    int brow[NB];
#pragma unroll
    for (int bt = 0; bt < NB; ++bt) {
        int b = bbase + bt * 16 + i;
        brow[bt] = b < a.B ? b : a.B - 1;
    }

    f32x4 acc[NB];
#pragma unroll
    for (int bt = 0; bt < NB; ++bt) acc[bt] = f32x4{0.f, 0.f, 0.f, 0.f};

    const int eb_ = bbase + (tid >> 6) * 16 + (lane & 15);
    const bool e_on = tid < NB * 64 && eb_ < a.B;
    float e_bi[4] = {0.f, 0.f, 0.f, 0.f}, e_bh[4] = {0.f, 0.f, 0.f, 0.f}, e_pr[4] = {0.f, 0.f, 0.f, 0.f};
    float e_c = 0.f, e_m = 1.f, l_bias[4] = {0.f, 0.f, 0.f, 0.f}, l_m1[4] = {1.f, 1.f, 1.f, 1.f};
    if (e_on) {
        const float* dummy = a.seg[0].w;
        if (MODE == 0) {
            const int u = tile * 4 + (lane >> 4);
            const float* pbi = a.b_ih ? a.b_ih + u : dummy;
            const float* pbh = a.b_hh ? a.b_hh + u : dummy;
            const float* ppr = a.pre ? a.pre + (size_t)eb_ * a.ldpre + u : dummy;
#pragma unroll
            for (int r = 0; r < 4; ++r) {
                e_bi[r] = pbi[a.b_ih ? r * a.H : 0];
                e_bh[r] = pbh[a.b_hh ? r * a.H : 0];
                e_pr[r] = ppr[a.pre ? r * a.H : 0];
            }
            e_c = (a.c_prev ? a.c_prev + (size_t)eb_ * a.ldc_prev + u : dummy)[0];
            e_m = (a.mask ? a.mask + (size_t)eb_ * a.H + u : dummy)[0];
        } else {
            const int nb = tile * 16 + 4 * (lane >> 4);
#pragma unroll
            for (int r = 0; r < 4; ++r) {
                const int n = nb + r < a.N ? nb + r : a.N - 1;
                l_bias[r] = (a.bias ? a.bias + n : dummy)[0];
                l_m1[r] = (a.lmask ? a.lmask + (size_t)eb_ * a.ldmask + n : dummy)[0];
            }
        }
    }

    int cstart = wave;
    for (int s = 0; s < a.nseg; ++s) {
        const float* __restrict__ wp = a.seg[s].w + (size_t)wrow * a.seg[s].ldw;
        const float* xp[NB];
#pragma unroll
        for (int bt = 0; bt < NB; ++bt) xp[bt] = a.seg[s].x + (size_t)brow[bt] * a.seg[s].ldx;
        const int K = a.seg[s].k;
        const int nchunk = (K + 31) >> 5;
        int c = cstart;
        for (; c < nchunk; c += 2 * KW) {
            const int k0 = c * 32 + kq * 4;
            const int k1 = (c + KW) * 32 + kq * 4;
            f32x4 w00 = sk_load<VEC>(wp, k0, K), w01 = sk_load<VEC>(wp, k0 + 16, K);
            f32x4 w10 = sk_load<VEC>(wp, k1, K), w11 = sk_load<VEC>(wp, k1 + 16, K);
            f32x4 x00[NB], x01[NB], x10[NB], x11[NB];
#pragma unroll
            for (int bt = 0; bt < NB; ++bt) {
                x00[bt] = sk_load<VEC>(xp[bt], k0, K);
                x01[bt] = sk_load<VEC>(xp[bt], k0 + 16, K);
                x10[bt] = sk_load<VEC>(xp[bt], k1, K);
                x11[bt] = sk_load<VEC>(xp[bt], k1 + 16, K);
            }
#pragma unroll
            for (int cc = 0; cc < 4; ++cc) {
#pragma unroll
                for (int bt = 0; bt < NB; ++bt) {
                    acc[bt] = __builtin_amdgcn_mfma_f32_16x16x4f32(w00[cc], x00[bt][cc], acc[bt], 0, 0, 0);
                    acc[bt] = __builtin_amdgcn_mfma_f32_16x16x4f32(w01[cc], x01[bt][cc], acc[bt], 0, 0, 0);
                    acc[bt] = __builtin_amdgcn_mfma_f32_16x16x4f32(w10[cc], x10[bt][cc], acc[bt], 0, 0, 0);
                    acc[bt] = __builtin_amdgcn_mfma_f32_16x16x4f32(w11[cc], x11[bt][cc], acc[bt], 0, 0, 0);
                }
            }
        }
        cstart = (cstart + KW - (nchunk % KW)) % KW;
    }

#pragma unroll
    for (int bt = 0; bt < NB; ++bt) red[(wave * NB + bt) * 64 + lane] = acc[bt];
    __syncthreads();
    if (tid >= NB * 64) return;

    const int bt = tid >> 6;
    f32x4 s = red[bt * 64 + lane];
#pragma unroll
    for (int w = 1; w < KW; ++w) {
        f32x4 t = red[(w * NB + bt) * 64 + lane];
        s[0] += t[0]; s[1] += t[1]; s[2] += t[2]; s[3] += t[3];
    }
    const int b = bbase + bt * 16 + (lane & 15);
    if (b >= a.B) return;

    if (MODE == 0) {
        const int H = a.H;
        const int u = tile * 4 + (lane >> 4);
        float g[4];
#pragma unroll
        for (int r = 0; r < 4; ++r) {
            g[r] = s[r] + (((a.b_ih ? e_bi[r] : 0.0f) + (a.b_hh ? e_bh[r] : 0.0f)) + (a.pre ? e_pr[r] : 0.0f));
        }
        const float gi = st_sigmoid_fast(g[0]), gf = st_sigmoid_fast(g[1]), gg = st_tanh_fast(g[2]), go = st_sigmoid_fast(g[3]);
        const float cp = a.c_prev ? e_c : 0.0f;
        const float c2 = gf * cp + gi * gg;
        float h2 = go * st_tanh_fast(c2);
        if (a.mask) h2 *= e_m;
        a.c_out[(size_t)b * a.ldc + u] = c2;
        a.h_out[(size_t)b * a.ldh + u] = h2;
        if (a.gates_out) {
            float* gp = a.gates_out + (size_t)b * 4 * H + u;
            gp[0] = gi; gp[H] = gf; gp[2 * H] = gg; gp[3 * H] = go;
        }
    } else {
#pragma unroll
        for (int r = 0; r < 4; ++r) {
            const int n = tile * 16 + 4 * (lane >> 4) + r;
            if (n >= a.N) continue;
            float v = s[r] + (a.bias ? l_bias[r] : 0.0f);
            v = st_act(v, a.act);
            if (a.lmask) v *= l_m1[r];
            if (a.n_split > 0 && n >= a.n_split) {
                float* p = a.y2 + (size_t)b * a.ldy2 + (size_t)(n - a.n_split) * a.rep;
                for (int j = 0; j < a.rep; ++j) p[j] = v;
            } else {
                a.y[(size_t)b * a.ldy + n] = v;
            }
        }
    }
}

template <int MODE, int NB, int KW, bool VEC>
__global__ __launch_bounds__(KW * 64) void sk_kernel(const SkArgs a) {
    __shared__ f32x4 red[KW * NB * 64];
    sk_body<MODE, NB, KW, VEC>(a, red);
}

template <int MODE, int NB, int KW, bool VEC>
__global__ __launch_bounds__(KW * 64) void sk_pair_kernel(const SkArgs a0, const SkArgs a1) {
    __shared__ f32x4 red[KW * NB * 64];
    if (blockIdx.z == 0) sk_body<MODE, NB, KW, VEC>(a0, red);
    else sk_body<MODE, NB, KW, VEC>(a1, red);
}

template <int MODE, int NB, bool VEC>
int sk_launch_pair(const SkArgs& a0, const SkArgs& a1, int tiles, hipStream_t st) {
    constexpr int KW = 8;
    dim3 grid(tiles, (a0.B + NB * 16 - 1) / (NB * 16), 2);
    hipLaunchKernelGGL((sk_pair_kernel<MODE, NB, KW, VEC>), grid, dim3(KW * 64), 0, st, a0, a1);
    ST_LAUNCH_CHECK();
    return 0;
}

template <int MODE>
int sk_dispatch_pair(const SkArgs (&a)[2], int tiles, hipStream_t st) {
    bool vec = true;
    for (int j = 0; j < 2; ++j) {
        const st_seg& g = a[j].seg[0];
        vec = vec && st_aligned16(g.x) && st_aligned16(g.w) && (g.ldx % 4 == 0) && (g.ldw % 4 == 0) && (g.k % 4 == 0);
    }
    const int nb = a[0].B <= 16 ? 1 : (a[0].B <= 32 ? 2 : 4);
    if (vec) {
        if (nb == 1) return sk_launch_pair<MODE, 1, true>(a[0], a[1], tiles, st);
        if (nb == 2) return sk_launch_pair<MODE, 2, true>(a[0], a[1], tiles, st);
        return sk_launch_pair<MODE, 4, true>(a[0], a[1], tiles, st);
    }
    if (nb == 1) return sk_launch_pair<MODE, 1, false>(a[0], a[1], tiles, st);
    if (nb == 2) return sk_launch_pair<MODE, 2, false>(a[0], a[1], tiles, st);
    return sk_launch_pair<MODE, 4, false>(a[0], a[1], tiles, st);
}

template <int MODE, int NB, bool VEC>
int sk_launch(const SkArgs& a, int tiles, hipStream_t st) {
    constexpr int KW = 8;
    dim3 grid(tiles, (a.B + NB * 16 - 1) / (NB * 16));
    hipLaunchKernelGGL((sk_kernel<MODE, NB, KW, VEC>), grid, dim3(KW * 64), 0, st, a);
    ST_LAUNCH_CHECK();
    return 0;
}

template <int MODE>
int sk_dispatch(const SkArgs& a, int tiles, hipStream_t st) {
    bool vec = true;
    for (int s = 0; s < a.nseg; ++s) {
        const st_seg& g = a.seg[s];
        vec = vec && st_aligned16(g.x) && st_aligned16(g.w) && (g.ldx % 4 == 0) && (g.ldw % 4 == 0) && (g.k % 4 == 0);
    }
    const int nb = a.B <= 16 ? 1 : (a.B <= 32 ? 2 : 4);
    if (vec) {
        if (nb == 1) return sk_launch<MODE, 1, true>(a, tiles, st);
        if (nb == 2) return sk_launch<MODE, 2, true>(a, tiles, st);
        return sk_launch<MODE, 4, true>(a, tiles, st);
    }
    if (nb == 1) return sk_launch<MODE, 1, false>(a, tiles, st);
    if (nb == 2) return sk_launch<MODE, 2, false>(a, tiles, st);
    return sk_launch<MODE, 4, false>(a, tiles, st);
}

int sk_fill_segs(SkArgs& a, const st_seg* segs, int nseg) {
    ST_CHECK_ARG(nseg >= 1 && nseg <= SK_MAXSEG, "skinny op: nseg=%d not in [1,%d]", nseg, SK_MAXSEG);
    a.nseg = nseg;
    for (int s = 0; s < nseg; ++s) {
        ST_CHECK_ARG(segs[s].x && segs[s].w && segs[s].k > 0, "skinny op: segment %d has null pointer or k<=0", s);
        ST_CHECK_ARG(segs[s].ldx >= segs[s].k && segs[s].ldw >= segs[s].k, "skinny op: segment %d stride < k", s);
        a.seg[s] = segs[s];
    }
    return 0;
}

}

extern "C" int st_lstm_cell_fwd(const st_seg* segs, int nseg, const float* b_ih, const float* b_hh,
                                const float* pre, int ldpre, const float* c_prev, int ldc_prev,
                                const float* mask, float* h_out, int ldh, float* c_out, int ldc,
                                float* gates_out, int B, int H, void* stream) {
    (void)hipGetLastError();
    ST_CHECK_ARG(B > 0 && H > 0, "st_lstm_cell_fwd: B=%d H=%d", B, H);
    ST_CHECK_ARG(H % 4 == 0, "st_lstm_cell_fwd: H=%d must be a multiple of 4", H);
    ST_CHECK_ARG(h_out && c_out, "st_lstm_cell_fwd: null output");
    SkArgs a;
    memset(&a, 0, sizeof(a));
    int rc = sk_fill_segs(a, segs, nseg);
    if (rc) return rc;
    a.B = B; a.N = 4 * H; a.H = H;
    a.b_ih = b_ih; a.b_hh = b_hh; a.pre = pre; a.ldpre = ldpre;
    a.c_prev = c_prev; a.ldc_prev = ldc_prev; a.mask = mask;
    a.h_out = h_out; a.ldh = ldh; a.c_out = c_out; a.ldc = ldc; a.gates_out = gates_out;
    return sk_dispatch<0>(a, H / 4, (hipStream_t)stream);
}

extern "C" int st_lstm_cell_pair_fwd(const st_seg* segs2, const float* const* b_hh2, const float* const* pre2, int ldpre,
                                     const float* const* c_prev2, int ldc_prev, float* const* h_out2, int ldh,
                                     float* const* c_out2, int ldc, float* const* gates_out2, int B, int H, void* stream) {
    (void)hipGetLastError();
    ST_CHECK_ARG(B > 0 && H > 0 && H % 4 == 0 && segs2 && h_out2 && c_out2, "st_lstm_cell_pair_fwd: bad arguments");
    SkArgs a[2];
    bool vec = true;
    for (int j = 0; j < 2; ++j) {
        memset(&a[j], 0, sizeof(SkArgs));
        int rc = sk_fill_segs(a[j], segs2 + j, 1);
        if (rc) return rc;
        ST_CHECK_ARG(h_out2[j] && c_out2[j], "st_lstm_cell_pair_fwd: null output");
        a[j].B = B; a[j].N = 4 * H; a[j].H = H;
        a[j].b_hh = b_hh2 ? b_hh2[j] : nullptr; a[j].pre = pre2 ? pre2[j] : nullptr; a[j].ldpre = ldpre;
        a[j].c_prev = c_prev2 ? c_prev2[j] : nullptr; a[j].ldc_prev = ldc_prev;
        a[j].h_out = h_out2[j]; a[j].ldh = ldh; a[j].c_out = c_out2[j]; a[j].ldc = ldc;
        a[j].gates_out = gates_out2 ? gates_out2[j] : nullptr;
        const st_seg& g = a[j].seg[0];
        vec = vec && st_aligned16(g.x) && st_aligned16(g.w) && (g.ldx % 4 == 0) && (g.ldw % 4 == 0) && (g.k % 4 == 0);
    }
    (void)vec;
    return sk_dispatch_pair<0>(a, H / 4, (hipStream_t)stream);
}

extern "C" int st_skinny_linear_pair_fwd(const st_seg* segs2, float* const* y2, int ldy, int B, int N, void* stream) {
    (void)hipGetLastError();
    ST_CHECK_ARG(B > 0 && N > 0 && segs2 && y2 && y2[0] && y2[1], "st_skinny_linear_pair_fwd: bad arguments");
    SkArgs a[2];
    for (int j = 0; j < 2; ++j) {
        memset(&a[j], 0, sizeof(SkArgs));
        int rc = sk_fill_segs(a[j], segs2 + j, 1);
        if (rc) return rc;
        a[j].B = B; a[j].N = N; a[j].H = 0; a[j].act = ST_ACT_NONE; a[j].y = y2[j]; a[j].ldy = ldy;
    }
    return sk_dispatch_pair<1>(a, (N + 15) / 16, (hipStream_t)stream);
}

extern "C" int st_skinny_linear_fwd(const st_seg* segs, int nseg, const float* bias, int act,
                                    const float* mask, int ldmask, float* y, int ldy,
                                    int n_split, float* y2, int ldy2, int rep,
                                    int B, int N, void* stream) {
    (void)hipGetLastError();
    ST_CHECK_ARG(B > 0 && N > 0 && y, "st_skinny_linear_fwd: B=%d N=%d y=%p", B, N, (void*)y);
    ST_CHECK_ARG(n_split <= 0 || (y2 && rep >= 1), "st_skinny_linear_fwd: n_split without y2/rep");
    SkArgs a;
    memset(&a, 0, sizeof(a));
    int rc = sk_fill_segs(a, segs, nseg);
    if (rc) return rc;
    a.B = B; a.N = N; a.H = 0;
    a.bias = bias; a.act = act; a.lmask = mask; a.ldmask = ldmask;
    a.y = y; a.ldy = ldy; a.n_split = n_split; a.y2 = y2; a.ldy2 = ldy2; a.rep = rep;
    return sk_dispatch<1>(a, (N + 15) / 16, (hipStream_t)stream);
}
```

### semi_tts_amd/csrc/skinny_packed.hip

```cpp
#include "st_common.h"
#include "attention_body.h"
#include "attention_bwd_body.h"
#include <cstdlib>

#ifndef PK_PROF
#define PK_PROF(n)
#endif
#ifndef RT2_PROF
#define RT2_PROF(n)
#endif

namespace {

constexpr int PK_MAXSEG = 3;

__host__ __device__ inline int pk_kb(int k) { return (k + 15) >> 4; }

struct PackArgs {
    const float* w[PK_MAXSEG]; int ldw[PK_MAXSEG]; int k[PK_MAXSEG]; int kb0[PK_MAXSEG];
    int nseg; int N; int H; int KB; int tiles; float* out;
};

__device__ __forceinline__ void pack_weight_body(const PackArgs& a);
__global__ __launch_bounds__(256) void pack_weight_kernel(const PackArgs a) { pack_weight_body(a); }

constexpr int PACK_BATCH_MAX = 8;
struct PackBatch { PackArgs j[PACK_BATCH_MAX]; };
__global__ __launch_bounds__(256) void pack_weight_batch_kernel(const PackBatch b) { pack_weight_body(b.j[blockIdx.y]); }

__device__ __forceinline__ void pack_weight_body(const PackArgs& a) {
    const size_t total = (size_t)a.tiles * a.KB * 64;
    for (size_t idx = (size_t)blockIdx.x * blockDim.x + threadIdx.x; idx < total; idx += (size_t)gridDim.x * blockDim.x) {
        const int lane = (int)(idx & 63);
        const size_t blk = idx >> 6;
        const int kb = (int)(blk % a.KB), tile = (int)(blk / a.KB);
        const int i = lane & 15, kq = lane >> 4;
        int row;
        if (a.H > 0) row = (i & 3) * a.H + tile * 4 + (i >> 2);
        else row = tile * 16 + i;
        int s = 0;
        while (s + 1 < a.nseg && kb >= a.kb0[s + 1]) ++s;
        const int k = (kb - a.kb0[s]) * 16 + kq * 4;
        f32x4 v = {0.f, 0.f, 0.f, 0.f};
        if (row < a.N) {
            const float* p = a.w[s] + (size_t)row * a.ldw[s] + k;
            const int rem = a.k[s] - k;
            if (rem >= 4 && st_aligned16(p)) v = st_ld4(p);
            else {
                if (rem > 0) v[0] = p[0];
                if (rem > 1) v[1] = p[1];
                if (rem > 2) v[2] = p[2];
                if (rem > 3) v[3] = p[3];
            }
        }
        reinterpret_cast<f32x4*>(a.out)[idx] = v;
    }
}

struct PackTArgs {
    const float* w[PK_MAXSEG]; int ldw[PK_MAXSEG]; int r0[PK_MAXSEG + 1];
    int nseg; int N; int K; int KB; int tiles; int vec; float* out;
};

__global__ __launch_bounds__(256) void pack_weight_t_kernel(const PackTArgs a) {
    const size_t total = (size_t)a.tiles * a.KB * 16;
    for (size_t idx = (size_t)blockIdx.x * blockDim.x + threadIdx.x; idx < total; idx += (size_t)gridDim.x * blockDim.x) {
        const int ig = (int)(idx & 3), kq = (int)((idx >> 2) & 3);
        const size_t blk = idx >> 4;
        const int kb = (int)(blk % a.KB), tile = (int)(blk / a.KB);
        const int row = tile * 16 + ig * 4, k = kb * 16 + kq * 4;
        f32x4 in[4];
#pragma unroll
        for (int j = 0; j < 4; ++j) in[j] = f32x4{0.f, 0.f, 0.f, 0.f};
        if (row < a.N) {
            int s = 0;
            while (s + 1 < a.nseg && row >= a.r0[s + 1]) ++s;
            const bool whole = a.vec && row + 4 <= a.r0[s + 1];
            if (whole && k + 4 <= a.K) {
                const float* p0 = a.w[s] + (size_t)k * a.ldw[s] + (row - a.r0[s]);
#pragma unroll
                for (int j = 0; j < 4; ++j) in[j] = st_ld4(p0 + (size_t)j * a.ldw[s]);
            } else
#pragma unroll
            for (int j = 0; j < 4; ++j) {
                if (k + j >= a.K) continue;
                if (whole) {
                    in[j] = st_ld4(a.w[s] + (size_t)(k + j) * a.ldw[s] + (row - a.r0[s]));
                } else {
#pragma unroll
                    for (int c = 0; c < 4; ++c) {
                        const int r = row + c;
                        if (r >= a.N) continue;
                        int sc = s;
                        while (sc + 1 < a.nseg && r >= a.r0[sc + 1]) ++sc;
                        in[j][c] = a.w[sc][(size_t)(k + j) * a.ldw[sc] + (r - a.r0[sc])];
                    }
                }
            }
        }
        f32x4* o = reinterpret_cast<f32x4*>(a.out) + blk * 64 + kq * 16 + ig * 4;
#pragma unroll
        for (int c = 0; c < 4; ++c) o[c] = f32x4{in[0][c], in[1][c], in[2][c], in[3][c]};
    }
}

__global__ __launch_bounds__(256) void tile_rows_kernel(const float* src, int ld, float* dst, int kbs, int kb0, int B, int K) {
    const int KB = pk_kb(K), BT = (B + 15) >> 4;
    const size_t total = (size_t)BT * KB * 64;
    for (size_t idx = (size_t)blockIdx.x * blockDim.x + threadIdx.x; idx < total; idx += (size_t)gridDim.x * blockDim.x) {
        const int lane = (int)(idx & 63);
        const size_t blk = idx >> 6;
        const int kb = (int)(blk % KB), bt = (int)(blk / KB);
        const int b = bt * 16 + (lane & 15), k = kb * 16 + (lane >> 4) * 4;
        if (b >= B) continue;
        f32x4 v = {0.f, 0.f, 0.f, 0.f};
        const float* p = src + (size_t)b * ld + k;
        const int rem = K - k;
        if (rem > 0) v[0] = p[0];
        if (rem > 1) v[1] = p[1];
        if (rem > 2) v[2] = p[2];
        if (rem > 3) v[3] = p[3];
        reinterpret_cast<f32x4*>(dst)[((size_t)bt * kbs + kb0 + kb) * 64 + lane] = v;
    }
}

__global__ __launch_bounds__(256) void untile_rows_vec_kernel(const float* src, int kbs, int kb0, float* dst, int ld, int B, int K) {
    const int KB = pk_kb(K), BT = (B + 15) >> 4;
    const size_t total = (size_t)BT * KB * 64;
    for (size_t idx = (size_t)blockIdx.x * blockDim.x + threadIdx.x; idx < total; idx += (size_t)gridDim.x * blockDim.x) {
        const int lane = (int)(idx & 63);
        const size_t blk = idx >> 6;
        const int kb = (int)(blk % KB), bt = (int)(blk / KB);
        const int b = bt * 16 + (lane & 15), k = kb * 16 + (lane >> 4) * 4;
        if (b >= B || k >= K) continue;
        const f32x4 v = reinterpret_cast<const f32x4*>(src)[((size_t)bt * kbs + kb0 + kb) * 64 + lane];
        float* o = dst + (size_t)b * ld + k;
        if (k + 4 <= K) *reinterpret_cast<f32x4*>(o) = v;
        else { o[0] = v[0]; if (k + 1 < K) o[1] = v[1]; if (k + 2 < K) o[2] = v[2]; }
    }
}

__global__ __launch_bounds__(256) void untile_rows_kernel(const float* src, int kbs, int kb0, float* dst, int ld, int B, int K) {
    const size_t total = (size_t)B * K;
    for (size_t idx = (size_t)blockIdx.x * blockDim.x + threadIdx.x; idx < total; idx += (size_t)gridDim.x * blockDim.x) {
        const int b = (int)(idx / K), k = (int)(idx - (size_t)b * K);
        const size_t off = (((size_t)(b >> 4) * kbs + kb0 + (k >> 4)) * 64 + ((k >> 2) & 3) * 16 + (b & 15)) * 4 + (k & 3);
        dst[(size_t)b * ld + k] = src[off];
    }
}

__device__ __forceinline__ size_t t16_off(int b, int k, int KB) {
    return (((size_t)(b >> 4) * KB + (k >> 4)) * 64 + ((k >> 2) & 3) * 16 + (b & 15)) * 4 + (k & 3);
}

struct PkOut { float* base; int kb_stride; int kb0; };

struct PkArgs {
    const f32x4* w; int w_kbs;
    const f32x4* x; int x_kbs;
    int KB;
    int B, N, H;
    const float* b_ih; const float* b_hh;
    const float* c_prev; int ldc_prev; const float* mask;
    float* c_out; int ldc; float* gates_out;
    PkOut h_dst[2];
    const float* ada_std; const float* ada_mean; PkOut ha_dst;
    const float* bias; int act; const float* lmask; int ldmask;
    float* y; int ldy; PkOut y_dst; int n_split; float* y2; int ldy2; int rep;
    int n_split2; int act2; const float* mask2; int ldmask2; PkOut y3_dst;
    unsigned long long* gran; unsigned epoch;
    const float* part;
};

struct PkPw {
    int n0, H;
    const float* dh1; int ld1;
    int dh1_slabs; long dh1_slab_stride;
    const float* dh2; int ld2; const float* scale2;
    const float* mask;
    const float* gates;
    const float* c; int ldc; const float* c_prev; int ldcp;
    float* dc;
    float* dgates; int ldg;
    PkOut dg_t16;
};

__device__ __forceinline__ void pk_store(const PkOut& d, int b, int k, float v) {
    if (d.base) d.base[t16_off(b, d.kb0 * 16 + k, d.kb_stride)] = v;
}

template <int NB, int TRIP>
struct PkRegs { f32x4 w[TRIP]; f32x4 x[TRIP][NB]; };

typedef __attribute__((ext_vector_type(4))) unsigned int pk_u32x4;

#ifndef PK_W_AUX
#define PK_W_AUX 0
#endif
struct PkSrc {
    __amdgpu_buffer_rsrc_t w, x;
    unsigned voff;
    int x_kbs;
};

template <int NB, int KW, int TRIP>
__device__ __forceinline__ void pk_load(PkRegs<NB, TRIP>& r, const PkSrc& src, int kb, int KB) {
    (void)KB;
#pragma unroll
    for (int t = 0; t < TRIP; ++t) {
        const unsigned vo = src.voff + (unsigned)(kb + t * KW) * 1024u;
        r.w[t] = __builtin_bit_cast(f32x4, __builtin_amdgcn_raw_buffer_load_b128(src.w, vo, 0, PK_W_AUX));
#pragma unroll
        for (int bt = 0; bt < NB; ++bt)
            r.x[t][bt] = __builtin_bit_cast(f32x4, __builtin_amdgcn_raw_buffer_load_b128(src.x, vo, bt * src.x_kbs * 1024, 0));
    }
}

template <int NB, int TRIP>
__device__ __forceinline__ void pk_mma(const PkRegs<NB, TRIP>& r, f32x4 (&acc)[NB]) {
#pragma unroll
    for (int t = 0; t < TRIP; ++t) {
        const f32x4 w = r.w[t];
#pragma unroll
        for (int cc = 0; cc < 4; ++cc)
#pragma unroll
            for (int bt = 0; bt < NB; ++bt)
                acc[bt] = __builtin_amdgcn_mfma_f32_16x16x4f32(w[cc], r.x[t][bt][cc], acc[bt], 0, 0, 0);
    }
}

template <int MODE, int NB, int KW, int TRIP>
__device__ __forceinline__ void pk_body(const PkArgs& a, const int tile, const int by, f32x4* red, const PkPw* pw = nullptr, const int tid0 = 0) {
    const int tid = (int)threadIdx.x - tid0, lane = tid & 63, wave = __builtin_amdgcn_readfirstlane(tid >> 6);
    const int bt0 = by * NB;
    const int BT = (a.B + 15) >> 4;

    PK_PROF(0);
#define PK_TOUCH(x) asm volatile("" :: "s"(x))
    PK_TOUCH(a.w); PK_TOUCH(a.x); PK_TOUCH(a.w_kbs); PK_TOUCH(a.x_kbs); PK_TOUCH(a.KB); PK_TOUCH(a.B); PK_TOUCH(a.N); PK_TOUCH(a.H);
    if (MODE == 0) {
        PK_TOUCH(a.b_ih); PK_TOUCH(a.b_hh); PK_TOUCH(a.c_prev); PK_TOUCH(a.ldc_prev);
        PK_TOUCH(a.mask); PK_TOUCH(a.ada_std); PK_TOUCH(a.ada_mean); PK_TOUCH(a.ha_dst.base);
    }
    if (MODE >= 1) {
        PK_TOUCH(a.bias); PK_TOUCH(a.lmask); PK_TOUCH(a.ldmask); PK_TOUCH(a.mask2); PK_TOUCH(a.ldmask2); PK_TOUCH(a.n_split2);
    }
#undef PK_TOUCH
    f32x4 acc[NB];
#pragma unroll
    for (int bt = 0; bt < NB; ++bt) acc[bt] = f32x4{0.f, 0.f, 0.f, 0.f};

    const int bt_base = bt0 + NB <= BT ? bt0 : (BT >= NB ? BT - NB : 0);
    const int KB = a.KB;
    PkSrc src;
    src.w = __builtin_amdgcn_make_buffer_rsrc((void*)(a.w + (size_t)tile * a.w_kbs * 64), 0, KB * 1024, 0x00020000);
    src.x = __builtin_amdgcn_make_buffer_rsrc((void*)(a.x + (size_t)bt_base * a.x_kbs * 64), 0, ((NB - 1) * a.x_kbs + KB) * 1024, 0x00020000);
    src.voff = (unsigned)lane * 16u;
    src.x_kbs = a.x_kbs;
    constexpr int STEP = KW * TRIP;
    PK_PROF(6);
    const int G = (KB + STEP - 1) / STEP;
#ifdef PK_NO_ROTATE
    const int rot = 0;
#else
    const int rot = (int)((((unsigned)tile & 255u) * (unsigned)G) >> 8);
#endif
    auto kb_of = [&](int gq) { int q = gq + rot; if (q >= G) q -= G; return q * STEP + wave; };
    PkRegs<NB, TRIP> ra, rb;
    if (G > 0) pk_load<NB, KW, TRIP>(ra, src, kb_of(0), KB);
    if (G > 1) pk_load<NB, KW, TRIP>(rb, src, kb_of(1), KB);
    const int eb = (bt_base + (tid >> 6)) * 16 + (lane & 15);
    const bool e_on = tid < NB * 64 && eb < a.B && bt_base + (tid >> 6) >= bt0;
    float e_bi[4] = {0.f, 0.f, 0.f, 0.f}, e_bh[4] = {0.f, 0.f, 0.f, 0.f};
    float e_c = 0.f, e_m = 1.f, e_s = 0.f, e_mu = 0.f;
    float l_bias[4] = {0.f, 0.f, 0.f, 0.f}, l_m1[4] = {1.f, 1.f, 1.f, 1.f}, l_m2[4] = {1.f, 1.f, 1.f, 1.f};
    const float* dummy = reinterpret_cast<const float*>(a.w);
    auto epi_prefetch = [&]() __attribute__((always_inline)) {
    if (MODE == 0 && e_on) {
        const int u = tile * 4 + (lane >> 4);
        const float* pbi = a.b_ih ? a.b_ih + u : dummy;
        const float* pbh = a.b_hh ? a.b_hh + u : dummy;
        const int sH = a.H;
#pragma unroll
        for (int r = 0; r < 4; ++r) {
            e_bi[r] = pbi[a.b_ih ? r * sH : 0];
            e_bh[r] = pbh[a.b_hh ? r * sH : 0];
        }
        e_c = (a.c_prev ? a.c_prev + (size_t)eb * a.ldc_prev + u : dummy)[0];
        e_m = (a.mask ? a.mask + (size_t)eb * a.H + u : dummy)[0];
        e_s = (a.ha_dst.base ? a.ada_std + (size_t)eb * a.H + u : dummy)[0];
        e_mu = (a.ha_dst.base ? a.ada_mean + (size_t)eb * a.H + u : dummy)[0];
    }
    if (MODE >= 1 && e_on) {
        const int nb = tile * 16 + 4 * (lane >> 4);
        const bool has_m2 = a.mask2 && a.n_split2 > 0;
#pragma unroll
        for (int r = 0; r < 4; ++r) {
            const int n = nb + r < a.N ? nb + r : a.N - 1;
            l_bias[r] = (a.bias ? a.bias + n : dummy)[0];
            l_m1[r] = (a.lmask ? a.lmask + (size_t)eb * a.ldmask + n : dummy)[0];
            l_m2[r] = (has_m2 && n >= a.n_split2 ? a.mask2 + (size_t)eb * a.ldmask2 + (n - a.n_split2) : dummy)[0];
        }
    }
    };
    const bool epi_late = G >= 3;
    if (!epi_late) epi_prefetch();
    PK_PROF(7);
    {
        int g = 0;
        PK_PROF(1);
        bool first = true;
        while (g < G) {
            pk_mma<NB, TRIP>(ra, acc);
            if (first) { PK_PROF(2); first = false; }
            if (g + 2 < G) pk_load<NB, KW, TRIP>(ra, src, kb_of(g + 2), KB);
            if (g == 0 && epi_late) epi_prefetch();
            ++g;
            if (g >= G) break;
            pk_mma<NB, TRIP>(rb, acc);
            if (g + 2 < G) pk_load<NB, KW, TRIP>(rb, src, kb_of(g + 2), KB);
            ++g;
        }
    }

    PK_PROF(3);
#pragma unroll
    for (int bt = 0; bt < NB; ++bt) red[(wave * NB + bt) * 64 + lane] = acc[bt];
    __syncthreads();
    PK_PROF(4);
    if (tid >= NB * 64) return;
    const int btl = tid >> 6;
    f32x4 s = red[btl * 64 + lane];
#pragma unroll
    for (int w = 1; w < KW; ++w) {
        const f32x4 t = red[(w * NB + btl) * 64 + lane];
        s[0] += t[0]; s[1] += t[1]; s[2] += t[2]; s[3] += t[3];
    }
    const int b = (bt_base + btl) * 16 + (lane & 15);
    if (b >= a.B || bt_base + btl < bt0) return;

    if (MODE == 0) {
        const int H = a.H;
        const int u = tile * 4 + (lane >> 4);
        float e_b[4];
#pragma unroll
        for (int r = 0; r < 4; ++r) e_b[r] = (a.b_ih ? e_bi[r] : 0.0f) + (a.b_hh ? e_bh[r] : 0.0f);
        e_c = a.c_prev ? e_c : 0.0f;
        e_m = a.mask ? e_m : 1.0f;
        const float gi = st_sigmoid_fast(s[0] + e_b[0]), gf = st_sigmoid_fast(s[1] + e_b[1]);
        const float gg = st_tanh_fast(s[2] + e_b[2]), go = st_sigmoid_fast(s[3] + e_b[3]);
        const float c2 = gf * e_c + gi * gg;
        const float h2 = go * st_tanh_fast(c2) * e_m;
        a.c_out[(size_t)b * a.ldc + u] = c2;
        pk_store(a.h_dst[0], b, u, h2);
        pk_store(a.h_dst[1], b, u, h2);
        if (a.ha_dst.base) pk_store(a.ha_dst, b, u, e_s * (h2 - e_mu));
        if (a.gates_out) {
            float* gp = a.gates_out + (size_t)b * 4 * H + u;
            gp[0] = gi; gp[H] = gf; gp[2 * H] = gg; gp[3 * H] = go;
        }
        PK_PROF(5);
    } else {
        const int n0 = tile * 16 + 4 * (lane >> 4);
        const int lim = a.n_split > 0 ? a.n_split : (a.n_split2 > 0 ? a.n_split2 : a.N);
        if (n0 + 3 < min(lim, a.N)) {
            f32x4 v4;
#pragma unroll
            for (int r = 0; r < 4; ++r) {
                float v = st_act(s[r] + (a.bias ? l_bias[r] : 0.0f), a.act);
                v4[r] = a.lmask ? v * l_m1[r] : v;
            }
            if (a.gran) {
                typedef __attribute__((address_space(1))) unsigned long long gu64;
                gu64* gp = (gu64*)(a.gran + (size_t)b * a.N + n0);
#pragma unroll
                for (int r = 0; r < 4; ++r)
                    __hip_atomic_store(gp + r, ((unsigned long long)a.epoch << 32) | (unsigned long long)__float_as_uint(v4[r]),
                                       __ATOMIC_RELAXED, __HIP_MEMORY_SCOPE_AGENT);
            }
            if (a.y) {
                float* py = a.y + (size_t)b * a.ldy + n0;
                if ((a.ldy & 3) == 0 && st_aligned16(a.y)) *reinterpret_cast<f32x4*>(py) = v4;
                else { py[0] = v4[0]; py[1] = v4[1]; py[2] = v4[2]; py[3] = v4[3]; }
            }
            if (a.y_dst.base) *reinterpret_cast<f32x4*>(a.y_dst.base + t16_off(b, a.y_dst.kb0 * 16 + n0, a.y_dst.kb_stride)) = v4;
            if (MODE == 2 && n0 >= pw->n0 && n0 + 3 < pw->n0 + pw->H) {
                const PkPw& q = *pw;
                const int H = q.H, u = n0 - q.n0;
                const size_t bu = (size_t)b * H + u;
                const float* gp = q.gates + (size_t)b * 4 * H + u;
                const f32x4 gi = st_ld4(gp), gf = st_ld4(gp + H), gg = st_ld4(gp + 2 * H), go = st_ld4(gp + 3 * H);
                const f32x4 cr = st_ld4(q.c + (size_t)b * q.ldc + u);
                const f32x4 dci = st_ld4(q.dc + bu);
                const float* dummy = q.gates;
                const f32x4 l1 = st_ld4(q.dh1 ? q.dh1 + (size_t)b * q.ld1 + u : dummy);
                f32x4 l1s[3];
#pragma unroll
                for (int sl = 0; sl < 3; ++sl) l1s[sl] = st_ld4(q.dh1 && sl + 1 < q.dh1_slabs ? q.dh1 + (size_t)(sl + 1) * q.dh1_slab_stride + (size_t)b * q.ld1 + u : dummy);
                const f32x4 l2 = st_ld4(q.dh2 ? q.dh2 + (size_t)b * q.ld2 + u : dummy);
                const f32x4 sc = st_ld4(q.scale2 ? q.scale2 + bu : dummy);
                const f32x4 mk = st_ld4(q.mask ? q.mask + bu : dummy);
                const f32x4 cp = st_ld4(q.c_prev ? q.c_prev + (size_t)b * q.ldcp + u : dummy);
                f32x4 d0, d1, d2, d3, dco;
#pragma unroll
                for (int r = 0; r < 4; ++r) {
                    float dh = v4[r];
                    if (q.dh1) {
                        float a1 = l1[r];
#pragma unroll
                        for (int sl = 0; sl < 3; ++sl) a1 += sl + 1 < q.dh1_slabs ? l1s[sl][r] : 0.0f;
                        dh += a1;
                    }
                    if (q.dh2) dh += l2[r] * (q.scale2 ? sc[r] : 1.0f);
                    if (q.mask) dh *= mk[r];
                    const float tc = tanhf(cr[r]);
                    const float cpv = q.c_prev ? cp[r] : 0.0f;
                    const float dc = dci[r] + dh * go[r] * (1.0f - tc * tc);
                    d0[r] = dc * gg[r] * gi[r] * (1.0f - gi[r]); d1[r] = dc * cpv * gf[r] * (1.0f - gf[r]);
                    d2[r] = dc * gi[r] * (1.0f - gg[r] * gg[r]); d3[r] = dh * tc * go[r] * (1.0f - go[r]);
                    dco[r] = dc * gf[r];
                }
                float* dg = q.dgates + (size_t)b * q.ldg + u;
                *reinterpret_cast<f32x4*>(dg) = d0; *reinterpret_cast<f32x4*>(dg + H) = d1;
                *reinterpret_cast<f32x4*>(dg + 2 * H) = d2; *reinterpret_cast<f32x4*>(dg + 3 * H) = d3;
                if (q.dg_t16.base) {
                    const int k0 = q.dg_t16.kb0 * 16 + u;
                    *reinterpret_cast<f32x4*>(q.dg_t16.base + t16_off(b, k0, q.dg_t16.kb_stride)) = d0;
                    *reinterpret_cast<f32x4*>(q.dg_t16.base + t16_off(b, k0 + H, q.dg_t16.kb_stride)) = d1;
                    *reinterpret_cast<f32x4*>(q.dg_t16.base + t16_off(b, k0 + 2 * H, q.dg_t16.kb_stride)) = d2;
                    *reinterpret_cast<f32x4*>(q.dg_t16.base + t16_off(b, k0 + 3 * H, q.dg_t16.kb_stride)) = d3;
                }
                *reinterpret_cast<f32x4*>(q.dc + bu) = dco;
            }
            PK_PROF(5);
            return;
        }
#pragma unroll
        for (int r = 0; r < 4; ++r) {
            const int n = n0 + r;
            if (n >= a.N) continue;
            float v = s[r] + (a.bias ? l_bias[r] : 0.0f);
            v = st_act(v, a.act);
            if (a.lmask) v *= l_m1[r];
            if (a.n_split2 > 0 && n >= a.n_split2) {
                v = st_act(v, a.act2);
                if (a.mask2) v *= l_m2[r];
                pk_store(a.y3_dst, b, n - a.n_split2, v);
            } else if (a.n_split > 0 && n >= a.n_split) {
                float* p = a.y2 + (size_t)b * a.ldy2 + (size_t)(n - a.n_split) * a.rep;
                for (int j = 0; j < a.rep; ++j) p[j] = v;
            } else {
                if (a.y) a.y[(size_t)b * a.ldy + n] = v;
                pk_store(a.y_dst, b, n, v);
            }
        }
        PK_PROF(5);
    }
}

template <int KW, int TRIP, int NB, int AUX0 = 0, int AUX1 = 0>
__device__ __forceinline__ void pk_lstm_rt2_body(const f32x4* wp, const f32x4* xp, const int w_kbs, const int x_kbs, const int KB,
                                                 const int B, const int H, const PkArgs& a, const int bx, const int by, f32x4* red) {
    constexpr int RT = 2;
    RT2_PROF(0);
    const int tid = threadIdx.x, lane = tid & 63, wave = __builtin_amdgcn_readfirstlane(tid >> 6);
    const int tile0 = bx * RT, bt_base = by * NB;
    __amdgpu_buffer_rsrc_t rw[RT];
#pragma unroll
    for (int rt = 0; rt < RT; ++rt)
        rw[rt] = __builtin_amdgcn_make_buffer_rsrc((void*)(wp + (size_t)(tile0 + rt) * w_kbs * 64), 0, KB * 1024, 0x00020000);
    const __amdgpu_buffer_rsrc_t rx = __builtin_amdgcn_make_buffer_rsrc((void*)(xp + (size_t)bt_base * x_kbs * 64), 0, ((NB - 1) * x_kbs + KB) * 1024, 0x00020000);
    const unsigned voff = (unsigned)lane * 16u;
    constexpr int STEP = KW * TRIP;
    const int G = (KB + STEP - 1) / STEP;
    const int rot = (int)((((unsigned)bx & 255u) * (unsigned)G) >> 8);
    auto kb_of = [&](int gq) { int q = gq + rot; if (q >= G) q -= G; return q * STEP + wave; };
    struct Regs { f32x4 w[TRIP][RT]; f32x4 x[TRIP][NB]; };
    auto load = [&](Regs& r, int kb) __attribute__((always_inline)) {
#pragma unroll
        for (int t = 0; t < TRIP; ++t) {
            const unsigned vo = voff + (unsigned)(kb + t * KW) * 1024u;
#pragma unroll
            for (int rt = 0; rt < RT; ++rt)
                r.w[t][rt] = rt == 0 ? __builtin_bit_cast(f32x4, __builtin_amdgcn_raw_buffer_load_b128(rw[0], vo, 0, AUX0))
                                     : __builtin_bit_cast(f32x4, __builtin_amdgcn_raw_buffer_load_b128(rw[rt], vo, 0, AUX1));
#pragma unroll
            for (int bt = 0; bt < NB; ++bt) r.x[t][bt] = __builtin_bit_cast(f32x4, __builtin_amdgcn_raw_buffer_load_b128(rx, vo, bt * x_kbs * 1024, 0));
        }
    };
    f32x4 acc[RT][NB];
#pragma unroll
    for (int rt = 0; rt < RT; ++rt)
#pragma unroll
        for (int bt = 0; bt < NB; ++bt) acc[rt][bt] = f32x4{0.f, 0.f, 0.f, 0.f};
    auto mma = [&](const Regs& r) __attribute__((always_inline)) {
#pragma unroll
        for (int t = 0; t < TRIP; ++t)
#pragma unroll
            for (int cc = 0; cc < 4; ++cc)
#pragma unroll
                for (int rt = 0; rt < RT; ++rt)
#pragma unroll
                    for (int bt = 0; bt < NB; ++bt)
                        acc[rt][bt] = __builtin_amdgcn_mfma_f32_16x16x4f32(r.w[t][rt][cc], r.x[t][bt][cc], acc[rt][bt], 0, 0, 0);
    };
    Regs ra, rb;
    if (G > 0) load(ra, kb_of(0));
    if (G > 1) load(rb, kb_of(1));
    RT2_PROF(1);
    const int e_rt = (tid >> 6) / NB, e_bt = (tid >> 6) % NB;
    const int eb = (bt_base + e_bt) * 16 + (lane & 15);
    const int u = (tile0 + e_rt) * 4 + (lane >> 4);
    const bool e_on = tid < RT * NB * 64 && eb < B;
    float e_bi[4] = {0.f, 0.f, 0.f, 0.f}, e_bh[4] = {0.f, 0.f, 0.f, 0.f};
    float e_c = 0.f, e_m = 1.f, e_s = 0.f, e_mu = 0.f;
    f32x4 e_p = {0.f, 0.f, 0.f, 0.f};
    const float* dummy = reinterpret_cast<const float*>(wp);
    auto epi_prefetch = [&]() __attribute__((always_inline)) {
        if (e_on) {
            if (a.part) e_p = st_ld4(a.part + (size_t)eb * (4 * H) + (size_t)(tile0 + e_rt) * 16 + 4 * (lane >> 4));
            const float* pbi = a.b_ih ? a.b_ih + u : dummy;
            const float* pbh = a.b_hh ? a.b_hh + u : dummy;
#pragma unroll
            for (int r = 0; r < 4; ++r) {
                e_bi[r] = pbi[a.b_ih ? r * H : 0];
                e_bh[r] = pbh[a.b_hh ? r * H : 0];
            }
            e_c = (a.c_prev ? a.c_prev + (size_t)eb * a.ldc_prev + u : dummy)[0];
            e_m = (a.mask ? a.mask + (size_t)eb * H + u : dummy)[0];
            e_s = (a.ha_dst.base ? a.ada_std + (size_t)eb * H + u : dummy)[0];
            e_mu = (a.ha_dst.base ? a.ada_mean + (size_t)eb * H + u : dummy)[0];
        }
    };
    {
        int g = 0;
        while (g < G) {
            mma(ra);
            if (g == 0) RT2_PROF(2);
            if (g + 2 < G) load(ra, kb_of(g + 2));
            if (g == 0) epi_prefetch();
            ++g;
            if (g >= G) break;
            mma(rb);
            if (g + 2 < G) load(rb, kb_of(g + 2));
            ++g;
        }
    }
    RT2_PROF(3);
#pragma unroll
    for (int rt = 0; rt < RT; ++rt)
#pragma unroll
        for (int bt = 0; bt < NB; ++bt) red[((wave * RT + rt) * NB + bt) * 64 + lane] = acc[rt][bt];
    __syncthreads();
    RT2_PROF(4);
    if (tid >= RT * NB * 64) return;
    f32x4 s = red[(e_rt * NB + e_bt) * 64 + lane];
#pragma unroll
    for (int w = 1; w < KW; ++w) {
        const f32x4 t = red[((w * RT + e_rt) * NB + e_bt) * 64 + lane];
        s[0] += t[0]; s[1] += t[1]; s[2] += t[2]; s[3] += t[3];
    }
    if (eb >= B) return;
    if (a.part) { s[0] += e_p[0]; s[1] += e_p[1]; s[2] += e_p[2]; s[3] += e_p[3]; }
    float e_b[4];
#pragma unroll
    for (int r = 0; r < 4; ++r) e_b[r] = (a.b_ih ? e_bi[r] : 0.0f) + (a.b_hh ? e_bh[r] : 0.0f);
    e_c = a.c_prev ? e_c : 0.0f;
    e_m = a.mask ? e_m : 1.0f;
    const float gi = st_sigmoid_fast(s[0] + e_b[0]), gf = st_sigmoid_fast(s[1] + e_b[1]);
    const float gg = st_tanh_fast(s[2] + e_b[2]), go = st_sigmoid_fast(s[3] + e_b[3]);
    const float c2 = gf * e_c + gi * gg;
    const float h2 = go * st_tanh_fast(c2) * e_m;
    a.c_out[(size_t)eb * a.ldc + u] = c2;
    pk_store(a.h_dst[0], eb, u, h2);
    pk_store(a.h_dst[1], eb, u, h2);
    if (a.ha_dst.base) pk_store(a.ha_dst, eb, u, e_s * (h2 - e_mu));
    if (a.gates_out) {
        float* gp = a.gates_out + (size_t)eb * 4 * H + u;
        gp[0] = gi; gp[H] = gf; gp[2 * H] = gg; gp[3 * H] = go;
    }
    RT2_PROF(5);
}

template <int KW, int TRIP, int NB, int AUX0 = 0, int AUX1 = 0>
__global__ __launch_bounds__(KW * 64) void pk_lstm_rt2_kernel(const f32x4* wp, const f32x4* xp, const int w_kbs, const int x_kbs, const int KB,
                                                          const int B, const int H, const PkArgs rest) {
    __shared__ f32x4 red[KW * 2 * NB * 64];
    pk_lstm_rt2_body<KW, TRIP, NB, AUX0, AUX1>(wp, xp, w_kbs, x_kbs, KB, B, H, rest, blockIdx.x, blockIdx.y, red);
}

template <int KW, int TRIP>
__global__ __launch_bounds__(KW * 64) void pk_lstm_rt2_pair_kernel(const int n0, const PkArgs a0, const PkArgs a1) {
    __shared__ f32x4 red[KW * 2 * 1 * 64];
    const bool second = (int)blockIdx.x >= n0;
    const PkArgs& a = second ? a1 : a0;
    const int i = second ? (int)blockIdx.x - n0 : (int)blockIdx.x;
    const int half = a.H >> 3;
    const int by = i >= half ? 1 : 0;
    pk_lstm_rt2_body<KW, TRIP, 1>(a.w, a.x, a.w_kbs, a.x_kbs, a.KB, a.B, a.H, a, i - by * half, by, red);
}

template <int MODE, int NB, int KW, int TRIP>
__global__ __launch_bounds__(KW * 64) void pk_kernel(const f32x4* w, const f32x4* x, const int w_kbs, const int x_kbs, const int KB,
                                                     const int B, const int N, const int H, const PkArgs rest) {
    __shared__ f32x4 red[KW * NB * 64];
    PkArgs a = rest;
    a.w = w; a.x = x; a.w_kbs = w_kbs; a.x_kbs = x_kbs; a.KB = KB; a.B = B; a.N = N; a.H = H;
    pk_body<MODE, NB, KW, TRIP>(a, blockIdx.x, blockIdx.y, red);
}

template <int NB, int KW, int TRIP>
__global__ __launch_bounds__(KW * 64) void pk_pw_kernel(const f32x4* w, const f32x4* x, const int w_kbs, const int x_kbs, const int KB,
                                                        const int B, const int N, const PkArgs rest, const PkPw pw) {
    __shared__ f32x4 red[KW * NB * 64];
    PkArgs a = rest;
    a.w = w; a.x = x; a.w_kbs = w_kbs; a.x_kbs = x_kbs; a.KB = KB; a.B = B; a.N = N; a.H = 0;
    pk_body<2, NB, KW, TRIP>(a, blockIdx.x, blockIdx.y, red, &pw);
}

template <int NB, int KW, int TRIP>
__global__ __launch_bounds__(KW * 64) void pk_pw_pair_kernel(const int n0, const int tiles, const PkArgs a0, const PkPw pw0, const PkArgs a1,
                                                             const PkPw pw1) {
    __shared__ f32x4 red[KW * NB * 64];
    const bool second = (int)blockIdx.x >= n0;
    const PkArgs& a = second ? a1 : a0;
    const PkPw& pw = second ? pw1 : pw0;
    const int i = second ? (int)blockIdx.x - n0 : (int)blockIdx.x;
    const int by = i / tiles;
    pk_body<2, NB, KW, TRIP>(a, i - by * tiles, by, red, &pw);
}

template <int NB, int KW, int TRIP, int LBLK, int NS>
__global__ __launch_bounds__(KW * 64) __attribute__((amdgpu_waves_per_eu((NS > 1 && NB == 1) ? 4 : 1, (NS > 1 && NB == 1) ? 4 : 8))) void pk_pw_ab_kernel(const f32x4* w, const f32x4* x, const int w_kbs, const int x_kbs, const int KB,
                                                           const int B, const int N, const int tiles_a, const int n_ab,
                                                           const PkArgs rest, const PkPw pw, const AbArgs ab) {
    extern __shared__ __attribute__((aligned(16))) float pk_dyn_lds[];
    __shared__ f32x4 red[KW * NB * 64];
    static_assert(KW * 64 == AB_THREADS, "both parts use 512-thread workgroups");
    const int i = blockIdx.x;
    if (i < n_ab) {
        if (NS == 1) ab_body<true, LBLK, 1>(ab, i, pk_dyn_lds);
        else { const int part = i / ab.B; ab_body<true, LBLK, NS>(ab, i - part * ab.B, pk_dyn_lds, part); }
        return;
    }
    PkArgs a = rest;
    a.w = w; a.x = x; a.w_kbs = w_kbs; a.x_kbs = x_kbs; a.KB = KB; a.B = B; a.N = N; a.H = 0;
    const int j = i - n_ab;
    const int by = j / tiles_a;
    pk_body<2, NB, KW, TRIP>(a, j - by * tiles_a, by, red, &pw);
}

#ifdef ST_ABLATE
static int st_exp_flag() { static int v = -1; if (v < 0) { const char* e = getenv("ST_EXP"); v = e ? atoi(e) : 0; } return v; }
#else
static inline int st_exp_flag() { return 0; }
#endif

struct PkPartArgs {
    const f32x4* w; int w_kbs;
    const f32x4* x; int x_kbs;
    int KB, S;
    int B, N;
    float* part;
};

template <int KW, int TRIP>
__device__ __forceinline__ void pk_part_body(const PkPartArgs& p, const int j, f32x4* red) {
    constexpr int RT = 2, NB = 2;
    const int tid = threadIdx.x, lane = tid & 63, wave = __builtin_amdgcn_readfirstlane(tid >> 6);
    const int n_tp = p.N >> 5;
    const int sp = j / n_tp, tp = j - sp * n_tp;
    const int KBs = p.KB / p.S, kb_lo = sp * KBs;
    __amdgpu_buffer_rsrc_t rw[RT];
#pragma unroll
    for (int rt = 0; rt < RT; ++rt)
        rw[rt] = __builtin_amdgcn_make_buffer_rsrc((void*)(p.w + ((size_t)(tp * RT + rt) * p.w_kbs + kb_lo) * 64), 0, KBs * 1024, 0x00020000);
    __amdgpu_buffer_rsrc_t rx[NB];
#pragma unroll
    for (int bt = 0; bt < NB; ++bt)
        rx[bt] = __builtin_amdgcn_make_buffer_rsrc((void*)(p.x + ((size_t)bt * p.x_kbs + kb_lo) * 64), 0, KBs * 1024, 0x00020000);
    const unsigned voff = (unsigned)lane * 16u;
    constexpr int STEP = KW * TRIP;
    const int G = (KBs + STEP - 1) / STEP;
    const int rot = (int)((((unsigned)tp & 255u) * (unsigned)G) >> 8);
    auto kb_of = [&](int gq) { int q = gq + rot; if (q >= G) q -= G; return q * STEP + wave; };
    struct Regs { f32x4 w[TRIP][RT]; f32x4 x[TRIP][NB]; };
    auto load = [&](Regs& r, int kb) __attribute__((always_inline)) {
#pragma unroll
        for (int t = 0; t < TRIP; ++t) {
            const unsigned vo = voff + (unsigned)(kb + t * KW) * 1024u;
#pragma unroll
            for (int rt = 0; rt < RT; ++rt) r.w[t][rt] = __builtin_bit_cast(f32x4, __builtin_amdgcn_raw_buffer_load_b128(rw[rt], vo, 0, 0));
#pragma unroll
            for (int bt = 0; bt < NB; ++bt) r.x[t][bt] = __builtin_bit_cast(f32x4, __builtin_amdgcn_raw_buffer_load_b128(rx[bt], vo, 0, 0));
        }
    };
    f32x4 acc[RT][NB];
#pragma unroll
    for (int rt = 0; rt < RT; ++rt)
#pragma unroll
        for (int bt = 0; bt < NB; ++bt) acc[rt][bt] = f32x4{0.f, 0.f, 0.f, 0.f};
    auto mma = [&](const Regs& r) __attribute__((always_inline)) {
#pragma unroll
        for (int t = 0; t < TRIP; ++t)
#pragma unroll
            for (int cc = 0; cc < 4; ++cc)
#pragma unroll
                for (int rt = 0; rt < RT; ++rt)
#pragma unroll
                    for (int bt = 0; bt < NB; ++bt)
                        acc[rt][bt] = __builtin_amdgcn_mfma_f32_16x16x4f32(r.w[t][rt][cc], r.x[t][bt][cc], acc[rt][bt], 0, 0, 0);
    };
    Regs ra, rb;
    if (G > 0) load(ra, kb_of(0));
    if (G > 1) load(rb, kb_of(1));
    {
        int g = 0;
        while (g < G) {
            mma(ra);
            if (g + 2 < G) load(ra, kb_of(g + 2));
            ++g;
            if (g >= G) break;
            mma(rb);
            if (g + 2 < G) load(rb, kb_of(g + 2));
            ++g;
        }
    }
#pragma unroll
    for (int rt = 0; rt < RT; ++rt)
#pragma unroll
        for (int bt = 0; bt < NB; ++bt) red[((wave * RT + rt) * NB + bt) * 64 + lane] = acc[rt][bt];
    __syncthreads();
    if (tid >= RT * NB * 64) return;
// ... 1017 lines not shown
```

### semi_tts_amd/module.py

```python
import ctypes as C

import numpy as np
import os
import torch
import torch.nn as nn

from . import ops
from . import _lib
from . import autograd as AG
from ._lib import StDecoderWeights, StDecoderDims, StDecoderIO, check


_ONES = {}


def _scaled_mask(shape, p, device):
    n = int(torch.Size(shape).numel())
    key = (str(device), n)
    ones = _ONES.get(key)
    if ones is None:
        if len(_ONES) > 64:
            _ONES.clear()
        ones = _ONES[key] = torch.ones(n, device=device, dtype=torch.float32)
    return torch.nn.functional.dropout(ones, p, training=True).view(shape)
# ... 153 lines not shown
        hidden_dim = list(hidden_dim)
        dims = [in_dim] + hidden_dim[:-1]
        self.layers = nn.ModuleList([Linear(din, dout, bias=False, norm_type=norm_type)
                                     for din, dout in zip(dims, hidden_dim)])
        self.apply_dropout = apply_dropout

    def forward(self, x, masks=None):
        if masks is None and self.apply_dropout > 0:
            masks = _scaled_masks([x.shape[:-1] + (layer.linear.out_features,) for layer in self.layers], self.apply_dropout, x.device)
        for i, layer in enumerate(self.layers):
            x = layer(x, act='relu', mask=masks[i] if masks is not None else None)
        return x


class Attention(nn.Module):

    def __init__(self, query_dim, memory_dim, hidden_dim, n_location_filters, location_kernel_size,
                 loc_aware, use_summed_weights):
        super().__init__()
        self.query_layer = Linear(query_dim, hidden_dim, bias=False, w_init_gain='tanh')
        self.memory_layer = Linear(memory_dim, hidden_dim, bias=False, w_init_gain='tanh')
        self.v = Linear(hidden_dim, 1, bias=False)
        self.loc_aware = loc_aware
        self.use_summed_weights = use_summed_weights
        self._dims = (hidden_dim, n_location_filters, location_kernel_size)
        if loc_aware:
            self.loc_conv = Conv1d(in_channels=2 if use_summed_weights else 1, out_channels=n_location_filters,
                                   kernel_size=location_kernel_size, bias=False, stride=1, dilation=1)
            self.loc_linear = Linear(n_location_filters, hidden_dim, bias=False, w_init_gain='tanh')

    def location_weights(self):
        A, F_, K = self._dims
        if not self.loc_aware:
            dev = self.v.linear.weight.device
            return torch.zeros(F_, 2, K, device=dev), torch.zeros(A, F_, device=dev)
        wc = self.loc_conv.conv.weight
        if not self.use_summed_weights:
            wc = torch.cat([wc, torch.zeros_like(wc)], dim=1)
        return wc, self.loc_linear.linear.weight

    def process_memory(self, memory):
        return ops.gemm(memory, self.memory_layer.linear.weight)

    def forward(self, query, memory, processed_memory, attn_history, mask=None):
        assert mask is None, 'the reference never passes a mask (module.py:163)'
        B, L, E = memory.shape
        pq = ops.linear_small(query, self.query_layer.linear.weight)
        hist = attn_history.contiguous()
        w_prev = hist[:, 0].contiguous()
        w_cum = hist[:, 1].contiguous() if hist.shape[1] > 1 else torch.zeros_like(w_prev)
        w = torch.empty(B, L, device=memory.device, dtype=torch.float32)
        w_cum_new = torch.empty_like(w)
        ctx = torch.empty(B, E, device=memory.device, dtype=torch.float32)
        wc, wl = self.location_weights()
        ops.attn_step(pq, processed_memory, memory, w_prev, w_cum, w, w_cum_new, wc.detach().contiguous(), wl.detach().contiguous(),
                      self.v.linear.weight, ctx)
        return ctx, w


def plan_decode(teacher_is_int, teacher_frames, teacher_bs, B, r, tf_rate, drop_dec_in, unpair_max_frame,
                coin=None):
    coin = coin or np.random.rand
    inference = tf_rate == 0.0
    partial = (not teacher_is_int) and B != teacher_bs
    if inference:
        steps = teacher_frames // r if teacher_is_int else teacher_frames
        t_groups = None
    else:
        assert not teacher_is_int, 'teacher forcing needs a teacher tensor'
        t_groups = teacher_frames // r
        if partial:
            assert unpair_max_frame is not None
            steps = max(t_groups, unpair_max_frame // r)
        else:
            steps = t_groups
    src = []
    for t in range(steps):
        if inference or (coin() > tf_rate):
            src.append(-1)
        elif coin() < drop_dec_in:
            src.append(-2)
        else:
            src.append(min(t, t_groups - 1))
    return steps, src


class Decoder(nn.Module):

    def __init__(self, n_mels, n_frames_per_step, enc_embed_dim, spkr_embed_dim, prenet_dim, prenet_dropout,
                 query_rnn_dim, dec_rnn_dim, query_dropout, dec_dropout, attn_dim, n_location_filters,
                 location_kernel_size, loc_aware, use_summed_weights, drop_dec_in, prenet_norm_type=None,
                 pretrain=False, spkr_embed_mode='adaIN'):
        super().__init__()
        self.n_mels = n_mels
        self.n_frames_per_step = n_frames_per_step
        self.enc_embed_dim = enc_embed_dim
        self.spkr_embed_dim = spkr_embed_dim
        self.query_rnn_dim = query_rnn_dim
        self.dec_rnn_dim = dec_rnn_dim
        self.prenet_dropout = prenet_dropout
        self.prenet_dim = prenet_dim
        self.query_dropout = nn.Dropout(query_dropout)
        self.dec_dropout = nn.Dropout(dec_dropout)
        self.attn_dim = attn_dim
        self.n_location_filters = n_location_filters
        self.location_kernel_size = location_kernel_size
        self.pretrain = pretrain
        self.loc_aware = loc_aware
        self.use_summed_weights = use_summed_weights
        self.drop_dec_in = drop_dec_in
        self.prenet_norm_type = prenet_norm_type
        self.spkr_embed_mode = spkr_embed_mode.lower()
        if self.spkr_embed_mode == 'adain':
            self.pseudo_latent_mean = nn.Linear(spkr_embed_dim, query_rnn_dim)
            self.pseudo_latent_std = nn.Sequential(nn.Linear(spkr_embed_dim, query_rnn_dim), nn.ReLU())
        elif self.spkr_embed_mode == 'concat':
            self.spkr_mem_proj = nn.Linear(spkr_embed_dim + enc_embed_dim, enc_embed_dim)
        elif self.spkr_embed_mode == 'add':
            self.spkr_proj = nn.Linear(spkr_embed_dim, enc_embed_dim)
            self.spkr_mem_proj = nn.Linear(enc_embed_dim, enc_embed_dim)
        else:
            raise NotImplementedError
        self.prenet = Prenet(n_mels * n_frames_per_step, [prenet_dim, prenet_dim], apply_dropout=prenet_dropout,
                             norm_type=prenet_norm_type)
        self.query_rnn = nn.LSTMCell(prenet_dim + enc_embed_dim, query_rnn_dim)
        self.attn = Attention(query_rnn_dim, enc_embed_dim, attn_dim, n_location_filters, location_kernel_size,
                              loc_aware, use_summed_weights)
        self.dec_rnn = nn.LSTMCell(query_rnn_dim + enc_embed_dim, dec_rnn_dim)
        self.proj = Linear(dec_rnn_dim + enc_embed_dim, n_mels * n_frames_per_step)
        self.gate_layer = Linear(dec_rnn_dim + enc_embed_dim, 1, bias=True, w_init_gain='sigmoid')
        self.last_tapes = None
        self.fuse_prenet = True
        self.cache_packed = False
        self.attn_split = True
        self.attn_pre_parts = 4
        self.attn_fin_parts = 2
        self.attn_pq_in_fin = True
        self.split_gates = os.environ.get('ST_SPLIT_GATES', '1') != '0'
        self.split_cell_k = int(os.environ.get('ST_SPLIT_CELL_K', '0'))
        self.split_gates_train = os.environ.get('ST_SPLIT_GATES_TRAIN', '1') != '0'
        self.check_handoff = True
        self.handoff_status = None
        self.attn_split_min_len = 128
        self.attn_split_positions = 43
        self.bwd_fuse_pointwise = True
        self.bwd_overlap_attn = True
        self.bwd_dxq_splits = int(os.environ.get('ST_DXQ_SPLITS', '4'))
        self.bwd_dxd_splits = int(os.environ.get('ST_DXD_SPLITS', '2'))
        self.bwd_attn_parts = int(os.environ.get('ST_ATTN_PARTS', '2'))
        self._last_fwd_forms = None
        self._last_bwd_forms = None
        self.fwd_pair_cells = True
        self.attn_rng_one_launch = True

    def gate_split_k(self):
        if self.split_cell_k:
            return int(self.split_cell_k)
        import ctypes as C
        from . import _lib
        d = StDecoderDims(B=32, L=1, E=self.enc_embed_dim, n_mels=self.n_mels, r=self.n_frames_per_step, P=self.prenet_dim,
                          Q=self.query_rnn_dim, D=self.dec_rnn_dim, A=1)
        return int(_lib.load().st_decoder_gate_split_k(C.byref(d)))

    def _weights_struct(self, keep, fuse_pre0=False):
        w = StDecoderWeights()
        pw, gw = self.proj.linear.weight, self.gate_layer.linear.weight
        in_dim, KO = pw.shape
        n_rows = in_dim + 1 + (self.prenet_dim if fuse_pre0 else 0)
        if not fuse_pre0 and not ops.capturing():
            pg_w = ops.cat_params([pw.detach(), gw.detach()])
            pg_b = ops.cat_params([self.proj.linear.bias.detach(), self.gate_layer.linear.bias.detach()])
        else:
            pg_w = torch.empty(n_rows, KO, device=pw.device, dtype=torch.float32)
            pg_b = torch.empty(n_rows, device=pw.device, dtype=torch.float32)
            ops.copy2d(pg_w, pw, in_dim, KO)
            ops.copy2d(pg_w[in_dim:], gw, 1, KO)
            ops.copy2d(pg_b.view(1, -1), self.proj.linear.bias.view(1, -1), 1, in_dim)
            ops.copy2d(pg_b.view(1, -1)[:, in_dim:], self.gate_layer.linear.bias.view(1, -1), 1, 1)
        if fuse_pre0:
            w0 = self.prenet.layers[0].linear.weight
            pwT = pw.detach().t().contiguous()
            ops.gemm(w0, pwT, out=pg_w[in_dim + 1:])
            ops.gemm(w0, self.proj.linear.bias.view(1, -1), out=pg_b[in_dim + 1:].view(-1, 1))
            keep.append(pwT)
        loc_wc, loc_wl = (t.detach().contiguous() for t in self.attn.location_weights())
        keep += [loc_wc, loc_wl]
        keep += [pg_w, pg_b]
        tensors = dict(
            prenet_w0=self.prenet.layers[0].linear.weight, prenet_w1=self.prenet.layers[1].linear.weight,
            q_w_ih=self.query_rnn.weight_ih, q_w_hh=self.query_rnn.weight_hh,
            q_b_ih=self.query_rnn.bias_ih, q_b_hh=self.query_rnn.bias_hh,
            attn_query_w=self.attn.query_layer.linear.weight, attn_v=self.attn.v.linear.weight,
            attn_loc_conv_w=loc_wc, attn_loc_lin_w=loc_wl,
            d_w_ih=self.dec_rnn.weight_ih, d_w_hh=self.dec_rnn.weight_hh,
            d_b_ih=self.dec_rnn.bias_ih, d_b_hh=self.dec_rnn.bias_hh, projgate_w=pg_w, projgate_b=pg_b)
        for k, t in tensors.items():
            setattr(w, k, ops._p(t))
        if self.prenet_norm_type is not None:
            for l, layer in enumerate(self.prenet.layers):
                nm = layer.norm
                w.pre_norm_w[l], w.pre_norm_b[l] = ops._p(nm.weight), ops._p(nm.bias)
                if self.prenet_norm_type == 'BatchNorm1d':
                    w.pre_norm_rm[l], w.pre_norm_rv[l] = ops._p(nm.running_mean), ops._p(nm.running_var)
                    w.pre_norm_nbt[l] = ops._p(nm.num_batches_tracked, torch.int64)
                    w.pre_norm_momentum = float(nm.momentum)
                w.pre_norm_eps = float(nm.eps)
        return w

    def forward(self, memory, memory_lengths, teacher, spkr_embed, tf_rate=0.0, unpair_max_frame=None, _masks=None):
        assert len(self.prenet.layers) == 2
        dev = memory.device
        memory = memory.contiguous()
        spkr_embed = spkr_embed.contiguous()
        B, L, E = memory.shape
        r, n_mels, P = self.n_frames_per_step, self.n_mels, self.prenet_dim
        Q, D, A = self.query_rnn_dim, self.dec_rnn_dim, self.attn_dim
        _masks = _masks or {}
        is_int = isinstance(teacher, int)
        Bt = B if is_int else teacher.shape[0]
        steps, step_src = plan_decode(is_int, teacher if is_int else teacher.shape[1], Bt, B, r, tf_rate,
                                      self.drop_dec_in, unpair_max_frame)
        differentiable = self.training and torch.is_grad_enabled()
        lin = (lambda x, m, act=None: AG.linear(x, m.weight, m.bias, act)) if differentiable else \
              (lambda x, m, act=None: (ops.linear_small(x, m.weight, m.bias, act) if x.dim() == 2 and x.shape[0] <= 64
                                       else ops.gemm(x, m.weight, bias=m.bias, act_pre=act)))
        pm = AG.conv(memory, self.attn.memory_layer.linear.weight) if differentiable else self.attn.process_memory(memory)
        ctx_memory = memory
        if self.spkr_embed_mode == 'adain':
            ada_std = lin(spkr_embed, self.pseudo_latent_std[0], 'relu')
            ada_mean = lin(spkr_embed, self.pseudo_latent_mean)
        else:
            ada_std = torch.ones(B, Q, device=dev, dtype=torch.float32)
            ada_mean = torch.zeros(B, Q, device=dev, dtype=torch.float32)
            if self.spkr_embed_mode == 'concat':
                w = self.spkr_mem_proj.weight
                sp = (AG.linear(spkr_embed, w[:, E:].contiguous(), self.spkr_mem_proj.bias) if differentiable
                      else ops.linear_small(spkr_embed, w[:, E:].contiguous(), self.spkr_mem_proj.bias))
                res = sp.unsqueeze(1).expand(B, L, E).contiguous()
                ctx_memory = (AG.conv(memory, w[:, :E].contiguous(), res=res) if differentiable
                              else ops.gemm(memory, w[:, :E].contiguous(), res=res))
            else:
                sp = lin(spkr_embed, self.spkr_proj)
                ctx_memory = lin(memory + sp.unsqueeze(1), self.spkr_mem_proj)
        if self.pretrain:
            ctx_memory = torch.zeros_like(memory)
        teacher_pre = teacher_mean = None
        Tt = 0
        if tf_rate != 0.0:
            tch = teacher.contiguous().view(Bt, -1, n_mels * r)
            Tt = tch.shape[1]
            teacher_pre = self.prenet(tch, _masks.get('teacher'))
            if any(s == -2 for s in step_src):
                teacher_mean = ops.mean_rows(teacher_pre.detach())
        dec_in0 = None
        if self.prenet_norm_type is not None:
            dec_in0 = self.prenet(torch.zeros(B, n_mels * r, device=dev, dtype=torch.float32), _masks.get('go')).contiguous()
        uses_own = any(s == -1 for s in step_src[:-1]) or Bt < B
        own_mask = _masks.get('own')
        if own_mask is None and uses_own and self.prenet_dropout > 0:
            own_mask = _scaled_mask((steps, 2, B, P), self.prenet_dropout, dev)
        q_mask, d_mask = _masks.get('q'), _masks.get('d')
        if self.training:
            if q_mask is None and d_mask is None and self.query_dropout.p == self.dec_dropout.p and self.query_dropout.p > 0:
                q_mask, d_mask = _scaled_masks([(steps, B, Q), (steps, B, D)], self.query_dropout.p, dev)
            if q_mask is None and self.query_dropout.p > 0:
                q_mask = _scaled_mask((steps, B, Q), self.query_dropout.p, dev)
            if d_mask is None and self.dec_dropout.p > 0:
                d_mask = _scaled_mask((steps, B, D), self.dec_dropout.p, dev)
        plan = dict(steps=steps, step_src=step_src, Bt=Bt, Tt=Tt, masks=(own_mask, q_mask, d_mask),
                    teacher_mean=teacher_mean, dec_in0=dec_in0.detach() if dec_in0 is not None else None)
        if differentiable:
            mel, align, stop = AG.decoder_loop(self, plan, ctx_memory.contiguous(), pm, ada_std, ada_mean, teacher_pre, dec_in0)
            return mel, (align * 0.0 if self.pretrain else align), stop
        mel, align, stop, tapes = self._run_loop(plan, ctx_memory.contiguous(), pm, ada_std, ada_mean, teacher_pre, keep_tapes=False)
        self.last_tapes = tapes
        if self.pretrain:
            ops.fill_(align, 0.0)
        return mel, align, stop

    def _run_loop(self, plan, memory, pm, ada_std, ada_mean, teacher_pre, keep_tapes):
        dev = memory.device
        B, L, E = memory.shape
        r, n_mels, P = self.n_frames_per_step, self.n_mels, self.prenet_dim
        Q, D, A = self.query_rnn_dim, self.dec_rnn_dim, self.attn_dim
        steps, step_src, Bt, Tt = plan['steps'], plan['step_src'], plan['Bt'], plan['Tt']
        own_mask, q_mask, d_mask = plan['masks']
        teacher_mean = plan['teacher_mean']
        keep = []
        f32 = dict(device=dev, dtype=torch.float32)
        mel = torch.empty(B, steps * r, n_mels, **f32)
        align = torch.empty(B, steps, L, **f32)
        stop = torch.empty(B, steps * r, **f32)
        lib = _lib.load()
        fuse_pre0 = ((not self.training) and self.fuse_prenet and Bt == B and all(s_ == -1 for s_ in step_src)
                     and self.prenet_norm_type is None)
        pn_mode = {None: 0, 'LayerNorm': 1, 'BatchNorm1d': 3 if self.training else 2}[self.prenet_norm_type]
        dims = StDecoderDims(B=B, L=L, E=E, n_mels=n_mels, r=r, P=P, Q=Q, D=D, A=A,
                             F=self.n_location_filters, K=self.location_kernel_size, fuse_pre0=1 if fuse_pre0 else 0,
                             prenet_norm=pn_mode)
        t16 = lambda k: int(lib.st_t16_floats(B, k))
        slot = [int(lib.st_decoder_tape_floats(C.byref(dims), i)) for i in range(3)]
        in_dim = r * n_mels
        n_pre1 = steps if keep_tapes else 1
        sizes = dict(xq=(steps + 1) * slot[0], xd=(steps + 1) * slot[1], xo=steps * slot[2], pre1=n_pre1 * t16(P), melt=t16(in_dim))
        no_pads = B % 16 == 0 and all(k % 16 == 0 for k in (P, E, Q, D, in_dim))
        tf_all = teacher_pre is not None and Bt == B and all(step_src[t] == min(t, Tt - 1) for t in range(steps - 1))
        tiled = (ops.uninit if (keep_tapes and no_pads and tf_all and self.prenet_norm_type is None) else ops.zeros)(sum(sizes.values()), **f32)
        tapes, off = {}, 0
        for k, n in sizes.items():
            tapes[k] = tiled[off:off + n]
            off += n
        tapes.update(cq=torch.empty(steps + 1, B, Q, **f32), cd=torch.empty(steps + 1, B, D, **f32),
                     wcum=torch.empty(steps + 1, B, L, **f32), pq=torch.empty(B, A, **f32),
                     zero=torch.empty(B, L, **f32), tiled=tiled)
        if keep_tapes:
            tapes['gates_q'] = torch.empty(steps, B, 4, Q, **f32)
            tapes['gates_d'] = torch.empty(steps, B, 4, D, **f32)

        cache = self.__dict__.setdefault('_packed_cache', {}) if (self.cache_packed and not self.training) else None
        ckey = (bool(fuse_pre0), str(dev), tuple(p._version for p in self.parameters())) if cache is not None else None
        if cache is not None and ckey not in cache:
            cache.clear()
        if cache is not None and ckey in cache:
            w, keep_w, packed = cache[ckey]
            keep.append(keep_w)
        else:
            w = self._weights_struct(keep, fuse_pre0)
            packed = torch.empty(int(lib.st_decoder_packed_floats(C.byref(dims))), **f32)
            check(lib.st_decoder_pack(C.byref(w), C.byref(dims), ops._p(packed), ops.stream_handle()), 'st_decoder_pack')
            if cache is not None:
                cache[ckey] = (w, list(keep), packed)
        io = StDecoderIO()
        src_arr = (C.c_int * max(steps, 1))(*step_src)
        io.memory, io.pm, io.ada_std, io.ada_mean = ops._p(memory), ops._p(pm), ops._p(ada_std), ops._p(ada_mean)
        io.step_src = C.cast(src_arr, C.POINTER(C.c_int))
        io.teacher_pre, io.teacher_mean = ops._p(teacher_pre), ops._p(teacher_mean)
        io.Bt, io.Tt = Bt, Tt
        io.prenet_mask, io.q_mask, io.d_mask = ops._p(own_mask), ops._p(q_mask), ops._p(d_mask)
        io.steps = steps
        io.mel_out, io.align_out, io.stop_out = ops._p(mel), ops._p(align), ops._p(stop)
        io.packed = ops._p(packed)
        io.xq_tape, io.xd_tape, io.xo_tape = (ops._p(tapes[k]) for k in ('xq', 'xd', 'xo'))
        io.cq_tape, io.cd_tape, io.wcum_tape = (ops._p(tapes[k]) for k in ('cq', 'cd', 'wcum'))
        io.pq_buf, io.pre1_t16, io.mel_t16 = (ops._p(tapes[k]) for k in ('pq', 'pre1', 'melt'))
        io.zero_row = ops._p(tapes['zero'])
        if pn_mode:
            tapes['pre_nat'] = torch.empty(B, P, **f32)
            io.pre_nat = ops._p(tapes['pre_nat'])
            tapes['pn_mode'] = pn_mode
            if keep_tapes:
                tapes['pre_y'] = torch.empty(steps, 2, B, P, **f32)
                io.pre_nat_tape = ops._p(tapes['pre_y'])
        if plan.get('dec_in0') is not None:
            io.dec_in0 = ops._p(plan['dec_in0'])
        io.gates_q_tape, io.gates_d_tape = ops._p(tapes.get('gates_q')), ops._p(tapes.get('gates_d'))
        io.pre1_step_floats = t16(P) if keep_tapes else 0
        pure_tf = teacher_pre is not None and Bt == B and all(step_src[t] == min(t, Tt - 1) for t in range(steps - 1))
        defer = bool(keep_tapes and pure_tf)
        io.defer_proj = 1 if defer else 0
        io.pair_cells = 1 if (defer and self.fwd_pair_cells) else 0
        if self.attn_split and (not self.training or defer):
            if keep_tapes:
                tapes['attn_s'] = ops.uninit(steps, B, L, A, **f32)
                tapes['attn_loc'] = ops.uninit(steps, B, L, self.n_location_filters, **f32)
                io.attn_s_step_floats = B * L * A
                io.attn_loc_tape = ops._p(tapes['attn_loc'])
            else:
                tapes['attn_s'] = torch.empty(B, L, A, **f32)
            io.attn_s_buf = ops._p(tapes['attn_s'])
            parts = int(self.attn_pre_parts)
            while parts < 64 and (L + parts - 1) // parts > 512:
                parts *= 2
            io.attn_pre_parts = parts
            io.attn_fin_parts = int(self.attn_fin_parts)
            if L >= self.attn_split_min_len and not keep_tapes:
                sp = max(2, min(64, (L + self.attn_split_positions - 1) // self.attn_split_positions))
                tapes['attn_split_ws'] = torch.empty(int(lib.st_attn_fin_split_workspace_floats(B, E, sp)), **f32)
                io.attn_split_ws, io.attn_split_parts = ops._p(tapes['attn_split_ws']), sp
                if self.attn_pq_in_fin and sp <= 8 and self.attn_rng_one_launch:
                    tapes['attn_xchg'] = torch.empty(2 * int(lib.st_attn_rng_xchg_words(B, E, sp)), **f32)
                    io.attn_xchg = ops._p(tapes['attn_xchg'])
            if self.split_gates and 16 < B <= 32 and ((not keep_tapes and L < self.attn_split_min_len) or (defer and self.split_gates_train)):
                tapes['gate_part'] = torch.empty(B, 4 * D, **f32)
                io.gate_part = ops._p(tapes['gate_part'])
                io.gate_part_k = int(self.split_cell_k)
            if self.attn_pq_in_fin and not keep_tapes:
                tapes['pq_gran'] = torch.empty(B, 2 * A, **f32)
                io.pq_granules = ops._p(tapes['pq_gran'])
                if self.handoff_status is None or self.handoff_status.device != dev:
                    self.handoff_status = torch.zeros(1, device=dev, dtype=torch.int32)
                io.handoff_status = ops._p(self.handoff_status, torch.int32)
        self._last_fwd_forms = int(lib.st_decoder_fwd_forms(C.byref(dims), C.byref(io), 0, 0))
        check(lib.st_decoder_forward(C.byref(w), C.byref(dims), C.byref(io), ops.stream_handle()),
              'st_decoder_forward')
        if io.handoff_status and self.check_handoff and not ops.capturing():
            if ops.handoff_starved(self.handoff_status):
                ops.degrade('decode loop (query projection -> attention hand-off)', 'one launch each (attn_pq_in_fin = False)')
                self.attn_pq_in_fin = False
                io.pq_granules, io.handoff_status, io.attn_xchg = None, None, None
                self._last_fwd_forms = int(lib.st_decoder_fwd_forms(C.byref(dims), C.byref(io), 0, 0))
                check(lib.st_decoder_forward(C.byref(w), C.byref(dims), C.byref(io), ops.stream_handle()), 'st_decoder_forward')
        if not keep_tapes and self.check_handoff and not ops.capturing():
            ops.check_persist_status(dev)
        if defer:
            kb = ops.kb16
            Bp = ((B + 15) // 16) * 16
            xo_nat = ops.untile_tape(tapes['xo'], steps, Bp, kb(D) + kb(E), [(0, D), (kb(D), E)])
            y = ops.gemm(xo_nat.view(-1, D + E), keep[-2], bias=keep[-1]).view(steps, Bp, in_dim + 1)
            check(lib.st_decoder_unpack_out(ops._p(y), ops._p(mel), ops._p(stop), B, Bp, steps, r, n_mels, in_dim + 1, ops.stream_handle()),
                  'st_decoder_unpack_out')
            tapes['xo_nat'] = xo_nat
        tapes['packed'] = packed
        tapes.update(pm=pm, ada_std=ada_std, ada_mean=ada_mean, teacher_pre=teacher_pre, masks=(own_mask, q_mask, d_mask),
                     keep=keep, step_src=step_src, slot=slot)
        return mel, align, stop, tapes


class BatchNormConv1d(nn.Module):

    def __init__(self, in_size, out_size, kernel_size, stride, padding, activation=None):
        super().__init__()
        assert stride == 1
        self.conv1d = nn.Conv1d(in_size, out_size, kernel_size=kernel_size, stride=stride, padding=padding, bias=False)
        self.bn = nn.BatchNorm1d(out_size, momentum=0.99, eps=1e-3)
        self.activation = activation
        self.padding = padding

    def forward(self, x_cl, training=None, Tout=None, out=None, coff=0, pool_prev=False, stats_Tout=None, collect=None):
        order = 'relu_bn' if self.activation is not None else 'bn'
        return _conv_bn_act(x_cl, self.conv1d.weight, None, self.bn, self.padding, self.bn.eps, self.bn.momentum,
                            order, self.training if training is None else training, Tout, out, coff, pool_prev,
                            stats_Tout, collect)


class Highway(nn.Module):

    def __init__(self, in_size, out_size):
        super().__init__()
        self.H = nn.Linear(in_size, out_size)
        self.H.bias.data.zero_()
        self.T = nn.Linear(in_size, out_size)
        self.T.bias.data.fill_(-1)

    def forward(self, x):
        if self.training:
            return AG.highway_layer(x, self.H.weight, self.H.bias, self.T.weight, self.T.bias)
        h = ops.gemm(x, self.H.weight, bias=self.H.bias, act_pre='relu')
        return ops.gemm(x, self.T.weight, bias=self.T.bias, act_pre='sigmoid', highway_h=h, res=x)


class CBHG(nn.Module):

    def __init__(self, in_dim, K=16, hidden_sizes=(128, 128)):
        super().__init__()
        hidden_sizes = list(hidden_sizes)
        self.in_dim = in_dim
        relu = nn.ReLU()
        self.conv1d_banks = nn.ModuleList([BatchNormConv1d(in_dim, in_dim, kernel_size=k, stride=1, padding=k // 2,
                                                           activation=relu) for k in range(1, K + 1)])
        in_sizes = [K * in_dim] + hidden_sizes[:-1]
        acts = [relu] * (len(hidden_sizes) - 1) + [None]
        self.conv1d_projs = nn.ModuleList([BatchNormConv1d(i, o, kernel_size=3, stride=1, padding=1, activation=a)
                                           for i, o, a in zip(in_sizes, hidden_sizes, acts)])
        self.pre_highway_proj = nn.Linear(hidden_sizes[-1], in_dim, bias=False)
        self.highways = nn.ModuleList([Highway(in_dim, in_dim) for _ in range(4)])
        self.gru = nn.GRU(in_dim, in_dim, num_layers=1, batch_first=True, bidirectional=True)

    def forward(self, inputs, input_lengths=None):
        assert input_lengths is None, 'the reference never passes lengths to the postnet CBHG'
        x = inputs.contiguous()
        B, T, Cn = x.shape
        assert Cn == self.in_dim
        K = len(self.conv1d_banks)
        if self.training:
            return self._forward_train(x)
        bank = torch.empty(B, T, K * Cn, device=x.device, dtype=torch.float32)
        jobs = []
        for i, blk in enumerate(self.conv1d_banks):
            k = i + 1
            blk(x, Tout=T, out=bank, coff=i * Cn, stats_Tout=T + 1 if k % 2 == 0 else T, collect=jobs)
        ops.gemm_flush(jobs)
        y = self.conv1d_projs[0](bank, pool_prev=True)
        for blk in self.conv1d_projs[1:]:
            y = blk(y)
        y = ops.gemm(y, self.pre_highway_proj.weight, res=x)
        ys = ops.highway_stack(y, [(hw.H.weight, hw.H.bias, hw.T.weight, hw.T.bias) for hw in self.highways])
        if ys is None:
            for hw in self.highways:
                y = hw(y)
        else:
            y = ys
        H = self.gru.hidden_size
        jobs = []
        gi_f = ops.gemm(y, self.gru.weight_ih_l0, bias=self.gru.bias_ih_l0, collect=jobs)
        gi_b = ops.gemm(y, self.gru.weight_ih_l0_reverse, bias=self.gru.bias_ih_l0_reverse, collect=jobs)
        ops.gemm_flush(jobs)
        out = torch.empty(B, T, 2 * H, device=x.device, dtype=torch.float32)
        ops.gru_seq(gi_f, gi_b, self.gru.weight_hh_l0, self.gru.weight_hh_l0_reverse,
                    self.gru.bias_hh_l0, self.gru.bias_hh_l0_reverse, out)
        return out


def _cbhg_forward_train(self, x):
    B, T, Cn = x.shape
    acts = set(blk.activation is not None for blk in self.conv1d_banks)
    assert len(acts) == 1
    relu = acts.pop()
    bank_launches = len(self.conv1d_banks) <= 16
    pre = AG.conv_group(x, [blk.conv1d.weight for blk in self.conv1d_banks], [blk.padding for blk in self.conv1d_banks],
                        [T + 1 if (i + 1) % 2 == 0 else T for i in range(len(self.conv1d_banks))], act='relu' if relu else None,
                        act_grad_done=bank_launches and relu)
    if bank_launches:
        bank = AG.batch_norm_bank(pre, [blk.bn for blk in self.conv1d_banks], T, relu_in=relu)
    else:
        bank = torch.cat([y[:, :T] for y in AG.batch_norm_train_group(pre, [blk.bn for blk in self.conv1d_banks])], dim=-1)
    y = self.conv1d_projs[0](bank, pool_prev=True)
    for blk in self.conv1d_projs[1:]:
        y = blk(y)
    y = AG.conv(y, self.pre_highway_proj.weight, res=x)
    for hw in self.highways:
        y = hw(y)
    g = self.gru
    gi_f, gi_b = AG.conv_group(y, [g.weight_ih_l0, g.weight_ih_l0_reverse], [0, 0], [None, None],
                               biases=[g.bias_ih_l0, g.bias_ih_l0_reverse])
    return AG.bigru(gi_f, gi_b, g.weight_hh_l0, g.bias_hh_l0, g.weight_hh_l0_reverse, g.bias_hh_l0_reverse)


CBHG._forward_train = _cbhg_forward_train


class Postnet(nn.Module):

    def __init__(self, n_mels, postnet_embed_dim, postnet_kernel_size, postnet_n_conv, postnet_dropout):
        super().__init__()
        in_size = [n_mels] + [postnet_embed_dim] * (postnet_n_conv - 1)
        out_size = [postnet_embed_dim] * (postnet_n_conv - 1) + [n_mels]
        act_fn = ['tanh'] * (postnet_n_conv - 1) + ['linear']
        self.postnet_dropout = postnet_dropout
        self.convs = nn.ModuleList([
            nn.Sequential(Conv1d(din, dout, kernel_size=postnet_kernel_size, stride=1,
                                 padding=(postnet_kernel_size - 1) // 2, dilation=1, w_init_gain=fn),
                          nn.BatchNorm1d(dout), nn.Tanh() if fn == 'tanh' else nn.Identity(), nn.Dropout(postnet_dropout))
            for din, dout, fn in zip(in_size, out_size, act_fn)])

    def forward(self, x, _masks=None):
        x = x.contiguous()
        for i, blk in enumerate(self.convs):
            conv, bn = blk[0], blk[1]
            order = 'bn_tanh' if isinstance(blk[2], nn.Tanh) else 'bn'
            x = _conv_bn_act(x, conv.conv.weight, conv.conv.bias, bn, conv.padding, bn.eps, bn.momentum, order,
                             self.training)
            if self.training and self.postnet_dropout > 0:
                x = x * (_masks[i] if _masks is not None else _scaled_mask(x.shape, self.postnet_dropout, x.device))
        return x
```

Measured before the change: 2.895 million.

## Fuse decode setup: AdaIN linears, tape zeroing and first query cell in one kernel

Adds a single decode-setup kernel that computes the AdaIN std/mean speaker projections, zeroes the working tape buffers, and evaluates the first query LSTM cell (zero state) in the same launch. The separate linear launches, the zero-fill kernel and the step-0 cell launch are skipped, and the host-side zeros allocation of the tiled tapes becomes uninitialised when the setup kernel covers it. This removes several small launches and a redundant fill before the decode loop. The cost is a more complex setup path with skip ranges for the xd tape and a dependence on correct coverage of every buffer the setup kernel zeroes.

```diff
diff --git a/include/semitts.h b/include/semitts.h
--- a/include/semitts.h
+++ b/include/semitts.h
@@ -401,6 +401,14 @@
     float* pre_nat_tape;
     float* gate_part;
     int gate_part_k;
+    const float* setup_spkr;
+    int setup_S;
+    const float* setup_std_w;
+    const float* setup_std_b;
+    const float* setup_mean_w;
+    const float* setup_mean_b;
+    float* setup_ada_std;
+    float* setup_ada_mean;
 } st_decoder_io;
 
 int st_decoder_gate_split_k(const st_decoder_dims* d);
@@ -410,6 +418,7 @@
 int st_decoder_forward(const st_decoder_weights* w, const st_decoder_dims* d, const st_decoder_io* io,
                        void* stream);
 int st_decoder_fwd_forms(const st_decoder_dims* d, const st_decoder_io* io, int cus, int rng_capacity);
+int st_decoder_setup_forms(const st_decoder_dims* d, const st_decoder_io* io);
 
 typedef struct st_attn_bwd_job {
     const float* pq; const float* pm; const float* memory;
diff --git a/semi_tts_amd/_lib.py b/semi_tts_amd/_lib.py
--- a/semi_tts_amd/_lib.py
+++ b/semi_tts_amd/_lib.py
@@ -72,7 +72,9 @@
                 ('pre1_step_floats', C.c_int), ('attn_s_step_floats', C.c_int), ('attn_loc_tape', C.c_void_p),
                 ('attn_split_ws', C.c_void_p), ('attn_split_parts', C.c_int), ('pq_granules', C.c_void_p),
                 ('dec_in0', C.c_void_p), ('pre_nat', C.c_void_p), ('attn_xchg', C.c_void_p), ('handoff_status', C.c_void_p),
-                ('pair_cells', C.c_int), ('pre_nat_tape', C.c_void_p), ('gate_part', C.c_void_p), ('gate_part_k', C.c_int)]
+                ('pair_cells', C.c_int), ('pre_nat_tape', C.c_void_p), ('gate_part', C.c_void_p), ('gate_part_k', C.c_int),
+                ('setup_spkr', C.c_void_p), ('setup_S', C.c_int), ('setup_std_w', C.c_void_p), ('setup_std_b', C.c_void_p),
+                ('setup_mean_w', C.c_void_p), ('setup_mean_b', C.c_void_p), ('setup_ada_std', C.c_void_p), ('setup_ada_mean', C.c_void_p)]
 
 
 class StDecoderBwdWeights(C.Structure):
@@ -269,6 +271,7 @@
     'st_decoder_pack': [C.POINTER(StDecoderWeights), C.POINTER(StDecoderDims), P, P],
     'st_decoder_forward': [C.POINTER(StDecoderWeights), C.POINTER(StDecoderDims), C.POINTER(StDecoderIO), P],
     'st_decoder_fwd_forms': [C.POINTER(StDecoderDims), C.POINTER(StDecoderIO), I, I],
+    'st_decoder_setup_forms': [C.POINTER(StDecoderDims), C.POINTER(StDecoderIO)],
     'st_attn_step_bwd': [C.POINTER(StAttnBwdJob), P],
     'st_skinny_linear_packed_lstm_bwd_fwd': [P, C.POINTER(StT16View), I, P, I, I, I, C.POINTER(StLstmPwJob), P],
     'st_skinny_linear_packed_lstm_bwd_attn_bwd': [P, C.POINTER(StT16View), I, P, I, I, I, C.POINTER(StLstmPwJob), C.POINTER(StAttnBwdJob), P],
diff --git a/semi_tts_amd/csrc/decode_setup.h b/semi_tts_amd/csrc/decode_setup.h
--- /dev/null
+++ b/semi_tts_amd/csrc/decode_setup.h
@@ -0,0 +1,57 @@
+#pragma once
+#include "st_common.h"
+
+namespace {
+
+struct PkOut { float* base; int kb_stride; int kb0; };
+
+__device__ __forceinline__ size_t t16_off(int b, int k, int KB) {
+    return (((size_t)(b >> 4) * KB + (k >> 4)) * 64 + ((k >> 2) & 3) * 16 + (b & 15)) * 4 + (k & 3);
+}
+
+__device__ __forceinline__ void pk_store(const PkOut& d, int b, int k, float v) {
+    if (d.base) d.base[t16_off(b, d.kb0 * 16 + k, d.kb_stride)] = v;
+}
+
+struct PkCellOut {
+    float* c_out; int ldc; float* gates_out;
+    PkOut h_dst[2];
+    PkOut ha_dst;
+};
+
+__device__ __forceinline__ void pk_lstm_pointwise(const f32x4 s, const float (&e_bi)[4], const float (&e_bh)[4], const bool has_bi,
+                                                  const bool has_bh, const float e_c, const float e_m, const float e_s, const float e_mu,
+                                                  const PkCellOut& o, const int H, const int b, const int u) {
+    float e_b[4];
+#pragma unroll
+    for (int r = 0; r < 4; ++r) e_b[r] = (has_bi ? e_bi[r] : 0.0f) + (has_bh ? e_bh[r] : 0.0f);
+    const float gi = st_sigmoid_fast(s[0] + e_b[0]), gf = st_sigmoid_fast(s[1] + e_b[1]);
+    const float gg = st_tanh_fast(s[2] + e_b[2]), go = st_sigmoid_fast(s[3] + e_b[3]);
+    const float c2 = gf * e_c + gi * gg;
+    const float h2 = go * st_tanh_fast(c2) * e_m;
+    o.c_out[(size_t)b * o.ldc + u] = c2;
+    pk_store(o.h_dst[0], b, u, h2);
+    pk_store(o.h_dst[1], b, u, h2);
+    if (o.ha_dst.base) pk_store(o.ha_dst, b, u, e_s * (h2 - e_mu));
+    if (o.gates_out) {
+        float* gp = o.gates_out + (size_t)b * 4 * H + u;
+        gp[0] = gi; gp[H] = gf; gp[2 * H] = gg; gp[3 * H] = go;
+    }
+}
+
+}
+
+constexpr int ST_SETUP_MAXZERO = 12;
+struct StDecodeSetup {
+    float* zp[ST_SETUP_MAXZERO]; size_t zfloats[ST_SETUP_MAXZERO]; int zn;
+    int skip_buf, skip_kbs, skip_lo, skip_hi;
+    const float* spkr; int S;
+    const float* w_std; const float* b_std; const float* w_mean; const float* b_mean;
+    float* ada_std; float* ada_mean;
+    int B, Q;
+    int cell0;
+    const float* b_ih; const float* b_hh; const float* mask;
+    float* c_out;
+    PkOut h_dst, ha_dst;
+};
+int st_decode_setup_launch(const StDecodeSetup& s, hipStream_t st);
diff --git a/semi_tts_amd/csrc/decoder.hip b/semi_tts_amd/csrc/decoder.hip
--- a/semi_tts_amd/csrc/decoder.hip
+++ b/semi_tts_amd/csrc/decoder.hip
@@ -1,5 +1,6 @@
 #include "st_common.h"
 #include "loop_graph.h"
+#include "decode_setup.h"
 #include <cstdlib>
 
 namespace {
@@ -208,7 +209,21 @@
 
 }
 
+namespace {
+int setup_forms(const st_decoder_dims* d, const st_decoder_io* io, const FwdForms& f) {
+    const bool one = io->setup_spkr && io->setup_S > 0 && io->setup_std_w && io->setup_mean_w && io->setup_ada_std && io->setup_ada_mean &&
+                     io->setup_ada_std == io->ada_std && io->setup_ada_mean == io->ada_mean;
+    const bool cell0 = one && !io->dec_in0 && !io->gates_q_tape && !f.pair_cells && d->Q % 4 == 0 && io->steps > 0;
+    return (one ? 1 : 0) | (cell0 ? 2 : 0);
+}
+}
+
 int pk_attnrng_capacity();
+
+extern "C" int st_decoder_setup_forms(const st_decoder_dims* d, const st_decoder_io* io) {
+    if (!d || !io || (io->steps > 1 && !io->step_src)) return -1;
+    return setup_forms(d, io, fwd_forms(d, io, 1, 1));
+}
 
 extern "C" int st_decoder_fwd_forms(const st_decoder_dims* d, const st_decoder_io* io, int cus, int rng_capacity) {
     if (!d || !io || (io->steps > 1 && !io->step_src)) return -1;
@@ -299,7 +314,30 @@
     const int sp_parts = io->attn_split_parts;
     if (f.attn == ATTN_PQ_FIN || f.attn == ATTN_PQ_RNG) zero(io->pq_granules, (size_t)B * A * sizeof(unsigned long long));
     if (f.attn == ATTN_PQ_RNG) zero(io->attn_xchg, st_attn_rng_xchg_words(B, E, sp_parts) * sizeof(unsigned long long));
-    {
+    ST_CHECK_ARG(!io->setup_spkr || (io->setup_ada_std == io->ada_std && io->setup_ada_mean == io->ada_mean),
+                 "st_decoder_forward: setup_ada_std / setup_ada_mean must be the buffers ada_std / ada_mean point to");
+    const int sf = setup_forms(d, io, f);
+    if (sf & 1) {
+        StDecodeSetup su;
+        memset(&su, 0, sizeof(su));
+        for (int i = 0; i < za.n; ++i) { su.zp[i] = za.p[i]; su.zfloats[i] = za.floats[i]; }
+        su.zn = za.n; su.skip_buf = -1;
+        su.spkr = io->setup_spkr; su.S = io->setup_S;
+        su.w_std = io->setup_std_w; su.b_std = io->setup_std_b; su.w_mean = io->setup_mean_w; su.b_mean = io->setup_mean_b;
+        su.ada_std = io->setup_ada_std; su.ada_mean = io->setup_ada_mean;
+        su.B = B; su.Q = Q;
+        if (sf & 2) {
+            su.cell0 = 1;
+            su.b_ih = w->q_b_ih; su.b_hh = w->q_b_hh; su.mask = io->q_mask;
+            su.c_out = io->cq_tape + BQ;
+            su.h_dst = PkOut{io->xq_tape + sv.q_floats, sv.q_kbs, sv.q_h};
+            su.ha_dst = PkOut{io->xd_tape, sv.d_kbs, sv.d_ha};
+            for (int i = 0; i < za.n; ++i)
+                if (za.p[i] == io->xd_tape) { su.skip_buf = i; su.skip_kbs = sv.d_kbs; su.skip_lo = sv.d_ha; su.skip_hi = sv.d_h; }
+        }
+        int rcs = st_decode_setup_launch(su, st);
+        if (rcs) return rcs;
+    } else {
         size_t most = 0;
         for (int i = 0; i < za.n; ++i) most = za.floats[i] > most ? za.floats[i] : most;
         size_t blocks = (most / 4 + 255) / 256 + 1;
@@ -369,7 +407,7 @@
         pj_d.x = st_t16_view{xd, sv.d_kbs, f.d_k0};
 
         st_t16_view hq_dst = {xq_next, sv.q_kbs, sv.q_h};
-        if (!(f.pair_cells && t > 0) && !ST_SKIPPED(0)) {
+        if (!(f.pair_cells && t > 0) && !(t == 0 && (sf & 2)) && !ST_SKIPPED(0)) {
             const st_lstm_cell_packed_job jq = cell_q(t);
             rc = st_lstm_cell_packed_fwd(&jq, stream);
             if (rc) return rc;
diff --git a/semi_tts_amd/csrc/skinny.hip b/semi_tts_amd/csrc/skinny.hip
--- a/semi_tts_amd/csrc/skinny.hip
+++ b/semi_tts_amd/csrc/skinny.hip
@@ -1,4 +1,5 @@
 #include "st_common.h"
+#include "decode_setup.h"
 
 namespace {
 
@@ -27,14 +28,13 @@
 }
 
 template <int MODE, int NB, int KW, bool VEC>
-__device__ __forceinline__ void sk_body(const SkArgs& a, f32x4* red) {
+__device__ __forceinline__ void sk_body(const SkArgs& a, const int tile, const int by, f32x4* red) {
     const int tid = threadIdx.x;
     const int lane = tid & 63;
     const int wave = tid >> 6;
     const int i = lane & 15;
     const int kq = lane >> 4;
-    const int tile = blockIdx.x;
-    const int bbase = blockIdx.y * (NB * 16);
+    const int bbase = by * (NB * 16);
 
     int wrow;
     if (MODE == 0) wrow = (i & 3) * a.H + tile * 4 + (i >> 2);
@@ -172,14 +172,14 @@
 template <int MODE, int NB, int KW, bool VEC>
 __global__ __launch_bounds__(KW * 64) void sk_kernel(const SkArgs a) {
     __shared__ f32x4 red[KW * NB * 64];
-    sk_body<MODE, NB, KW, VEC>(a, red);
+    sk_body<MODE, NB, KW, VEC>(a, blockIdx.x, blockIdx.y, red);
 }
 
 template <int MODE, int NB, int KW, bool VEC>
 __global__ __launch_bounds__(KW * 64) void sk_pair_kernel(const SkArgs a0, const SkArgs a1) {
     __shared__ f32x4 red[KW * NB * 64];
-    if (blockIdx.z == 0) sk_body<MODE, NB, KW, VEC>(a0, red);
-    else sk_body<MODE, NB, KW, VEC>(a1, red);
+    if (blockIdx.z == 0) sk_body<MODE, NB, KW, VEC>(a0, blockIdx.x, blockIdx.y, red);
+    else sk_body<MODE, NB, KW, VEC>(a1, blockIdx.x, blockIdx.y, red);
 }
 
 template <int MODE, int NB, bool VEC>
@@ -234,6 +234,66 @@
     if (nb == 1) return sk_launch<MODE, 1, false>(a, tiles, st);
     if (nb == 2) return sk_launch<MODE, 2, false>(a, tiles, st);
     return sk_launch<MODE, 4, false>(a, tiles, st);
+}
+
+template <int NB, bool VEC>
+__global__ __launch_bounds__(512) void decode_setup_kernel(const SkArgs a_std, const SkArgs a_mean, const StDecodeSetup s, const int tiles,
+                                                            const int n_lin, const int zblocks) {
+    constexpr int KW = 8;
+    __shared__ f32x4 red[KW * NB * 64];
+    const int tid = threadIdx.x;
+    if ((int)blockIdx.x < n_lin) {
+        const int tile = (int)blockIdx.x % tiles, by = (int)blockIdx.x / tiles;
+        sk_body<1, NB, KW, VEC>(a_std, tile, by, red);
+        __syncthreads();
+        sk_body<1, NB, KW, VEC>(a_mean, tile, by, red);
+        if (!s.cell0) return;
+        __syncthreads();
+        const int H = s.Q;
+        const PkCellOut o = {s.c_out, H, nullptr, {s.h_dst, PkOut{nullptr, 0, 0}}, s.ha_dst};
+        for (int idx = tid; idx < NB * 256; idx += KW * 64) {
+            const int u = tile * 16 + (idx & 15), b = by * (NB * 16) + (idx >> 4);
+            if (u >= H || b >= s.B) continue;
+            float e_bi[4] = {0.f, 0.f, 0.f, 0.f}, e_bh[4] = {0.f, 0.f, 0.f, 0.f};
+#pragma unroll
+            for (int r = 0; r < 4; ++r) {
+                if (s.b_ih) e_bi[r] = s.b_ih[r * H + u];
+                if (s.b_hh) e_bh[r] = s.b_hh[r * H + u];
+            }
+            const float e_m = s.mask ? s.mask[(size_t)b * H + u] : 1.0f;
+            const float e_s = s.ada_std[(size_t)b * H + u], e_mu = s.ada_mean[(size_t)b * H + u];
+            pk_lstm_pointwise(f32x4{0.f, 0.f, 0.f, 0.f}, e_bi, e_bh, s.b_ih != nullptr, s.b_hh != nullptr, 0.0f, e_m, e_s, e_mu, o, H, b, u);
+        }
+        return;
+    }
+    const int zb = (int)blockIdx.x - n_lin, buf = zb / zblocks, bx = zb % zblocks;
+    float* __restrict__ p = s.zp[buf];
+    const size_t n = s.zfloats[buf];
+    const size_t n4 = (((uintptr_t)p & 15u) == 0) ? n / 4 : 0;
+    const bool skip = buf == s.skip_buf;
+    const size_t stride = (size_t)zblocks * (KW * 64);
+    const f32x4 z = {0.f, 0.f, 0.f, 0.f};
+    for (size_t i = (size_t)bx * (KW * 64) + tid; i < n4; i += stride) {
+        if (skip) { const int kb = (int)((i >> 6) % (size_t)s.skip_kbs); if (kb >= s.skip_lo && kb < s.skip_hi) continue; }
+        reinterpret_cast<f32x4*>(p)[i] = z;
+    }
+    for (size_t i = n4 * 4 + (size_t)bx * (KW * 64) + tid; i < n; i += stride) {
+        if (skip) { const int kb = (int)((i >> 8) % (size_t)s.skip_kbs); if (kb >= s.skip_lo && kb < s.skip_hi) continue; }
+        p[i] = 0.0f;
+    }
+}
+
+template <int NB, bool VEC>
+int setup_launch(const SkArgs& a_std, const SkArgs& a_mean, const StDecodeSetup& s, hipStream_t st) {
+    const int tiles = (s.Q + 15) / 16, n_lin = tiles * ((s.B + NB * 16 - 1) / (NB * 16));
+    size_t most = 0;
+    for (int i = 0; i < s.zn; ++i) most = s.zfloats[i] > most ? s.zfloats[i] : most;
+    size_t zblocks = (most / 4 + 511) / 512 + 1;
+    if (zblocks > 128) zblocks = 128;
+    hipLaunchKernelGGL((decode_setup_kernel<NB, VEC>), dim3((unsigned)(n_lin + s.zn * (int)zblocks)), dim3(512), 0, st, a_std, a_mean, s, tiles,
+                       n_lin, (int)zblocks);
+    ST_LAUNCH_CHECK();
+    return 0;
 }
 
 int sk_fill_segs(SkArgs& a, const st_seg* segs, int nseg) {
@@ -321,3 +381,31 @@
     a.y = y; a.ldy = ldy; a.n_split = n_split; a.y2 = y2; a.ldy2 = ldy2; a.rep = rep;
     return sk_dispatch<1>(a, (N + 15) / 16, (hipStream_t)stream);
 }
+
+int st_decode_setup_launch(const StDecodeSetup& s, hipStream_t st) {
+    ST_CHECK_ARG(s.B > 0 && s.Q > 0 && s.S > 0 && s.spkr && s.w_std && s.w_mean && s.ada_std && s.ada_mean, "decode set-up: bad AdaIN arguments");
+    ST_CHECK_ARG(s.zn >= 0 && s.zn <= ST_SETUP_MAXZERO, "decode set-up: %d zero regions", s.zn);
+    ST_CHECK_ARG(!s.cell0 || (s.Q % 4 == 0 && s.c_out && s.h_dst.base), "decode set-up: bad first-cell arguments");
+    ST_CHECK_ARG(s.skip_buf < 0 || (s.skip_buf < s.zn && s.skip_kbs > 0), "decode set-up: bad skip range");
+    SkArgs a[2];
+    bool vec = true;
+    for (int j = 0; j < 2; ++j) {
+        memset(&a[j], 0, sizeof(SkArgs));
+        const st_seg g = {s.spkr, j == 0 ? s.w_std : s.w_mean, s.S, s.S, s.S};
+        int rc = sk_fill_segs(a[j], &g, 1);
+        if (rc) return rc;
+        a[j].B = s.B; a[j].N = s.Q; a[j].H = 0;
+        a[j].bias = j == 0 ? s.b_std : s.b_mean; a[j].act = j == 0 ? ST_ACT_RELU : ST_ACT_NONE;
+        a[j].y = j == 0 ? s.ada_std : s.ada_mean; a[j].ldy = s.Q;
+        vec = vec && st_aligned16(g.x) && st_aligned16(g.w) && (g.ldx % 4 == 0) && (g.ldw % 4 == 0) && (g.k % 4 == 0);
+    }
+    const int nb = s.B <= 16 ? 1 : (s.B <= 32 ? 2 : 4);
+    if (vec) {
+        if (nb == 1) return setup_launch<1, true>(a[0], a[1], s, st);
+        if (nb == 2) return setup_launch<2, true>(a[0], a[1], s, st);
+        return setup_launch<4, true>(a[0], a[1], s, st);
+    }
+    if (nb == 1) return setup_launch<1, false>(a[0], a[1], s, st);
+    if (nb == 2) return setup_launch<2, false>(a[0], a[1], s, st);
+    return setup_launch<4, false>(a[0], a[1], s, st);
+}
diff --git a/semi_tts_amd/csrc/skinny_packed.hip b/semi_tts_amd/csrc/skinny_packed.hip
--- a/semi_tts_amd/csrc/skinny_packed.hip
+++ b/semi_tts_amd/csrc/skinny_packed.hip
@@ -1,4 +1,5 @@
 #include "st_common.h"
+#include "decode_setup.h"
 #include "attention_body.h"
 #include "attention_bwd_body.h"
 #include <cstdlib>
@@ -149,12 +150,6 @@
     }
 }
 
-__device__ __forceinline__ size_t t16_off(int b, int k, int KB) {
-    return (((size_t)(b >> 4) * KB + (k >> 4)) * 64 + ((k >> 2) & 3) * 16 + (b & 15)) * 4 + (k & 3);
-}
-
-struct PkOut { float* base; int kb_stride; int kb0; };
-
 struct PkArgs {
     const f32x4* w; int w_kbs;
     const f32x4* x; int x_kbs;
@@ -184,10 +179,6 @@
     float* dgates; int ldg;
     PkOut dg_t16;
 };
-
-__device__ __forceinline__ void pk_store(const PkOut& d, int b, int k, float v) {
-    if (d.base) d.base[t16_off(b, d.kb0 * 16 + k, d.kb_stride)] = v;
-}
 
 template <int NB, int TRIP>
 struct PkRegs { f32x4 w[TRIP]; f32x4 x[TRIP][NB]; };
@@ -340,25 +331,10 @@
     if (b >= a.B || bt_base + btl < bt0) return;
 
     if (MODE == 0) {
-        const int H = a.H;
         const int u = tile * 4 + (lane >> 4);
-        float e_b[4];
-#pragma unroll
-        for (int r = 0; r < 4; ++r) e_b[r] = (a.b_ih ? e_bi[r] : 0.0f) + (a.b_hh ? e_bh[r] : 0.0f);
-        e_c = a.c_prev ? e_c : 0.0f;
-        e_m = a.mask ? e_m : 1.0f;
-        const float gi = st_sigmoid_fast(s[0] + e_b[0]), gf = st_sigmoid_fast(s[1] + e_b[1]);
-        const float gg = st_tanh_fast(s[2] + e_b[2]), go = st_sigmoid_fast(s[3] + e_b[3]);
-        const float c2 = gf * e_c + gi * gg;
-        const float h2 = go * st_tanh_fast(c2) * e_m;
-        a.c_out[(size_t)b * a.ldc + u] = c2;
-        pk_store(a.h_dst[0], b, u, h2);
-        pk_store(a.h_dst[1], b, u, h2);
-        if (a.ha_dst.base) pk_store(a.ha_dst, b, u, e_s * (h2 - e_mu));
-        if (a.gates_out) {
-            float* gp = a.gates_out + (size_t)b * 4 * H + u;
-            gp[0] = gi; gp[H] = gf; gp[2 * H] = gg; gp[3 * H] = go;
-        }
+        const PkCellOut o = {a.c_out, a.ldc, a.gates_out, {a.h_dst[0], a.h_dst[1]}, a.ha_dst};
+        pk_lstm_pointwise(s, e_bi, e_bh, a.b_ih != nullptr, a.b_hh != nullptr, a.c_prev ? e_c : 0.0f, a.mask ? e_m : 1.0f, e_s, e_mu,
+                          o, a.H, b, u);
         PK_PROF(5);
     } else {
         const int n0 = tile * 16 + 4 * (lane >> 4);
@@ -562,23 +538,9 @@
     }
     if (eb >= B) return;
     if (a.part) { s[0] += e_p[0]; s[1] += e_p[1]; s[2] += e_p[2]; s[3] += e_p[3]; }
-    float e_b[4];
-#pragma unroll
-    for (int r = 0; r < 4; ++r) e_b[r] = (a.b_ih ? e_bi[r] : 0.0f) + (a.b_hh ? e_bh[r] : 0.0f);
-    e_c = a.c_prev ? e_c : 0.0f;
-    e_m = a.mask ? e_m : 1.0f;
-    const float gi = st_sigmoid_fast(s[0] + e_b[0]), gf = st_sigmoid_fast(s[1] + e_b[1]);
-    const float gg = st_tanh_fast(s[2] + e_b[2]), go = st_sigmoid_fast(s[3] + e_b[3]);
-    const float c2 = gf * e_c + gi * gg;
-    const float h2 = go * st_tanh_fast(c2) * e_m;
-    a.c_out[(size_t)eb * a.ldc + u] = c2;
-    pk_store(a.h_dst[0], eb, u, h2);
-    pk_store(a.h_dst[1], eb, u, h2);
-    if (a.ha_dst.base) pk_store(a.ha_dst, eb, u, e_s * (h2 - e_mu));
-    if (a.gates_out) {
-        float* gp = a.gates_out + (size_t)eb * 4 * H + u;
-        gp[0] = gi; gp[H] = gf; gp[2 * H] = gg; gp[3 * H] = go;
-    }
+    const PkCellOut o = {a.c_out, a.ldc, a.gates_out, {a.h_dst[0], a.h_dst[1]}, a.ha_dst};
+    pk_lstm_pointwise(s, e_bi, e_bh, a.b_ih != nullptr, a.b_hh != nullptr, a.c_prev ? e_c : 0.0f, a.mask ? e_m : 1.0f, e_s, e_mu,
+                      o, H, eb, u);
     RT2_PROF(5);
 }
 
diff --git a/semi_tts_amd/module.py b/semi_tts_amd/module.py
--- a/semi_tts_amd/module.py
+++ b/semi_tts_amd/module.py
@@ -329,6 +329,8 @@
         self._last_bwd_forms = None
         self.fwd_pair_cells = True
         self.attn_rng_one_launch = True
+        self.decode_setup = os.environ.get('ST_DECODE_SETUP', '1') != '0'
+        self._last_setup_forms = None
 
     def gate_split_k(self):
         if self.split_cell_k:
@@ -403,7 +405,12 @@
                                        else ops.gemm(x, m.weight, bias=m.bias, act_pre=act)))
         pm = AG.conv(memory, self.attn.memory_layer.linear.weight) if differentiable else self.attn.process_memory(memory)
         ctx_memory = memory
-        if self.spkr_embed_mode == 'adain':
+        setup_spkr = None
+        if self.spkr_embed_mode == 'adain' and self.decode_setup and not differentiable and B <= 64:
+            ada_std = torch.empty(B, Q, device=dev, dtype=torch.float32)
+            ada_mean = torch.empty(B, Q, device=dev, dtype=torch.float32)
+            setup_spkr = spkr_embed
+        elif self.spkr_embed_mode == 'adain':
             ada_std = lin(spkr_embed, self.pseudo_latent_std[0], 'relu')
             ada_mean = lin(spkr_embed, self.pseudo_latent_mean)
         else:
@@ -445,7 +452,7 @@
             if d_mask is None and self.dec_dropout.p > 0:
                 d_mask = _scaled_mask((steps, B, D), self.dec_dropout.p, dev)
         plan = dict(steps=steps, step_src=step_src, Bt=Bt, Tt=Tt, masks=(own_mask, q_mask, d_mask),
-                    teacher_mean=teacher_mean, dec_in0=dec_in0.detach() if dec_in0 is not None else None)
+                    teacher_mean=teacher_mean, dec_in0=dec_in0.detach() if dec_in0 is not None else None, setup_spkr=setup_spkr)
         if differentiable:
             mel, align, stop = AG.decoder_loop(self, plan, ctx_memory.contiguous(), pm, ada_std, ada_mean, teacher_pre, dec_in0)
             return mel, (align * 0.0 if self.pretrain else align), stop
@@ -482,7 +489,9 @@
         sizes = dict(xq=(steps + 1) * slot[0], xd=(steps + 1) * slot[1], xo=steps * slot[2], pre1=n_pre1 * t16(P), melt=t16(in_dim))
         no_pads = B % 16 == 0 and all(k % 16 == 0 for k in (P, E, Q, D, in_dim))
         tf_all = teacher_pre is not None and Bt == B and all(step_src[t] == min(t, Tt - 1) for t in range(steps - 1))
-        tiled = (ops.uninit if (keep_tapes and no_pads and tf_all and self.prenet_norm_type is None) else ops.zeros)(sum(sizes.values()), **f32)
+        no_fill_free = self.decode_setup and not keep_tapes and no_pads and fuse_pre0
+        no_fill = no_fill_free or (keep_tapes and no_pads and tf_all and self.prenet_norm_type is None)
+        tiled = (ops.uninit if no_fill else ops.zeros)(sum(sizes.values()), **f32)
         tapes, off = {}, 0
         for k, n in sizes.items():
             tapes[k] = tiled[off:off + n]
@@ -567,7 +576,14 @@
                 if self.handoff_status is None or self.handoff_status.device != dev:
                     self.handoff_status = torch.zeros(1, device=dev, dtype=torch.int32)
                 io.handoff_status = ops._p(self.handoff_status, torch.int32)
+        if plan.get('setup_spkr') is not None:
+            std_l, mean_l = self.pseudo_latent_std[0], self.pseudo_latent_mean
+            io.setup_spkr, io.setup_S = ops._p(plan['setup_spkr']), int(plan['setup_spkr'].shape[1])
+            io.setup_std_w, io.setup_std_b = ops._p(std_l.weight), ops._p(std_l.bias)
+            io.setup_mean_w, io.setup_mean_b = ops._p(mean_l.weight), ops._p(mean_l.bias)
+            io.setup_ada_std, io.setup_ada_mean = ops._p(ada_std), ops._p(ada_mean)
         self._last_fwd_forms = int(lib.st_decoder_fwd_forms(C.byref(dims), C.byref(io), 0, 0))
+        self._last_setup_forms = int(lib.st_decoder_setup_forms(C.byref(dims), C.byref(io))) | (4 if no_fill_free else 0)
         check(lib.st_decoder_forward(C.byref(w), C.byref(dims), C.byref(io), ops.stream_handle()),
               'st_decoder_forward')
         if io.handoff_status and self.check_handoff and not ops.capturing():
@@ -589,7 +605,7 @@
             tapes['xo_nat'] = xo_nat
         tapes['packed'] = packed
         tapes.update(pm=pm, ada_std=ada_std, ada_mean=ada_mean, teacher_pre=teacher_pre, masks=(own_mask, q_mask, d_mask),
-                     keep=keep, step_src=step_src, slot=slot)
+                     keep=keep, step_src=step_src, slot=slot, setup_spkr=plan.get('setup_spkr'))
         return mel, align, stop, tapes
 
 
```

After: 2.909 million, median of 6. Within noise of the previous version (+0.5%).
